# logannye/streaming-zero-knowledge-proofs

Hardware: AMD Instinct MI355X
Metric: STARK prove field-elements/sec (NTT+FRI+Merkle), 2^24 domain, 1/2/4/8 GPUs (higher is better)
Workload: dtype u64; 1 GPU; stark-v1 prove, T=2^21 rows (N=2^24 LDE domain), b=512, tau=8, trace resident in HBM when the timed region starts, proof bytes on the host (host_to_proof beside it: every proof uploads its own trace over PCIe); T=2097152, N=16777216, tau=8, b=512, proof_bytes=2301655, proofs_in_flight_per_gpu=3, upload_bytes_per_proof=69206016, parallelism=replicas x1, 3 independent proofs in flight per GPU

## Files before the change

### include/sezkp_stark.h

```cpp
#ifndef SEZKP_STARK_H
#define SEZKP_STARK_H

#include <stddef.h>
#include <stdint.h>

#ifdef __cplusplus
extern "C" {
#endif

#define SEZKP_ABI_VERSION 4u

#define SEZKP_OK 0
#define SEZKP_E_INVALID (-1)
#define SEZKP_E_DEVICE (-2)
#define SEZKP_E_NOMEM (-3)
#define SEZKP_E_DECODE (-4)
#define SEZKP_E_VERIFY (-5)

#define SEZKP_FLAG_STREAMING 1u

uint32_t sezkp_abi_version(void);
const char* sezkp_version(void);

typedef struct sezkp_buf {
    uint8_t* data;
    size_t len;
} sezkp_buf;
void sezkp_buf_free(sezkp_buf* b);

typedef struct sezkp_block_view {
    uint32_t n_blocks;
    uint32_t tau;
    const uint16_t* version;
    const uint32_t* block_id;
    const uint64_t* step_lo;
    const uint64_t* step_hi;
    const uint16_t* ctrl_in;
    const uint16_t* ctrl_out;
    const int64_t* in_head_in;
    const int64_t* in_head_out;
    const int64_t* win_left;
    const int64_t* win_right;
    const uint32_t* off_in;
    const uint32_t* off_out;
    const uint64_t* step_start;
    const int8_t* input_mv;
    const int8_t* mv;
    const uint8_t* has_write;
    const uint16_t* wsym;
} sezkp_block_view;

int32_t sezkp_stark_v1_prove(const sezkp_block_view* blocks, const uint8_t manifest_root[32], uint32_t flags,
                             sezkp_buf* proof_bytes, sezkp_buf* meta_json, char* err, size_t err_len);
int32_t sezkp_stark_v1_prove_artifact_cbor(const sezkp_block_view* blocks, const uint8_t manifest_root[32],
                                           uint32_t flags, sezkp_buf* artifact_cbor, char* err, size_t err_len);
int32_t sezkp_stark_v1_verify(const uint8_t* proof_bytes, size_t len, const sezkp_block_view* blocks,
                              const uint8_t manifest_root[32], char* err, size_t err_len);

typedef struct sezkp_ctx sezkp_ctx;
sezkp_ctx* sezkp_ctx_create(int32_t device, char* err, size_t err_len);
void sezkp_ctx_destroy(sezkp_ctx* ctx);
int32_t sezkp_ctx_upload(sezkp_ctx* ctx, const sezkp_block_view* blocks, char* err, size_t err_len);
int32_t sezkp_ctx_upload_rows(sezkp_ctx* ctx, const sezkp_block_view* blocks, uint64_t row0, uint64_t nrows,
                              char* err, size_t err_len);
int32_t sezkp_shard_rows(const uint64_t* step_start, uint32_t n_blocks, int32_t rank, int32_t world, uint64_t* row0,
                         uint64_t* nrows);
int32_t sezkp_ctx_prove(sezkp_ctx* ctx, const uint8_t manifest_root[32], uint32_t flags, sezkp_buf* proof_bytes,
                        char* err, size_t err_len);
int32_t sezkp_ctx_stage(sezkp_ctx* ctx, const sezkp_block_view* blocks, char* err, size_t err_len);
int32_t sezkp_host_register(void* p, size_t bytes);
int32_t sezkp_host_unregister(void* p);
int32_t sezkp_ctx_prove_borrow(sezkp_ctx* ctx, const uint8_t manifest_root[32], uint32_t flags,
                               const uint8_t** data, size_t* len, char* err, size_t err_len);
int32_t sezkp_ctx_stage_times(const sezkp_ctx* ctx, double* out_ms, int32_t max);
int32_t sezkp_ctx_prove_async(sezkp_ctx* ctx, const uint8_t manifest_root[32], uint32_t flags, char* err,
                              size_t err_len);
int32_t sezkp_ctx_wait(sezkp_ctx* ctx, const uint8_t** data, size_t* len, char* err, size_t err_len);
void* sezkp_ctx_stream(const sezkp_ctx* ctx);
typedef struct sezkp_dict_plan_info {
  uint32_t col;
  uint32_t kind;
  uint32_t tape;
  int32_t K;
  uint32_t a;
  uint32_t delta;
  uint32_t R;
  uint32_t dR;
  int64_t min;
} sezkp_dict_plan_info;
int32_t sezkp_ctx_dict_plans(const sezkp_ctx* ctx, sezkp_dict_plan_info* out, int32_t max);
int32_t sezkp_ctx_dict_cache_stats(const sezkp_ctx* ctx, uint32_t* cols_rebuilt, uint32_t* cols_reused,
                                   uint64_t* entries_rebuilt);

#define SEZKP_AIR_FAMILIES 5
typedef struct sezkp_air_family {
  uint64_t cells, rows, first_row;
  uint32_t first_tape, pad;
  uint64_t first_value;
} sezkp_air_family;
typedef struct sezkp_air_audit {
  uint64_t n_rows;
  uint32_t tau, pad;
  uint64_t rows_violating, first_violating, rows_rejectable, first_rejectable;
  sezkp_air_family fam[SEZKP_AIR_FAMILIES];
} sezkp_air_audit;
int32_t sezkp_ctx_air_audit(sezkp_ctx* ctx, sezkp_air_audit* out, uint8_t* violating_bits, uint8_t* rejectable_bits,
                            char* err, size_t err_len);
int32_t sezkp_stark_v1_air_audit(const sezkp_block_view* blocks, sezkp_air_audit* out, sezkp_buf* violating_bits,
                                 sezkp_buf* rejectable_bits, char* err, size_t err_len);

typedef struct sezkp_proof_ref {
  const uint8_t* bytes;
  size_t len;
  const uint8_t* manifest_root;
  uint32_t tau;
  uint32_t pad;
} sezkp_proof_ref;
typedef struct sezkp_verify_result {
  int32_t code;
  uint32_t pad;
  char msg[248];
} sezkp_verify_result;
int32_t sezkp_ctx_verify_batch(sezkp_ctx* ctx, const sezkp_proof_ref* proofs, uint32_t n, sezkp_verify_result* out,
                               char* err, size_t err_len);
int32_t sezkp_stark_v1_verify_batch(const sezkp_proof_ref* proofs, uint32_t n, sezkp_verify_result* out, char* err,
                                    size_t err_len);
enum {
  SEZKP_VT_PARSE, SEZKP_VT_PACK, SEZKP_VT_DEVICE_WALL, SEZKP_VT_H2D, SEZKP_VT_KERNEL, SEZKP_VT_D2H, SEZKP_VT_DECIDE,
  SEZKP_VT_WALL, SEZKP_VT_JOBS, SEZKP_VT_SLICES, SEZKP_VERIFY_TIMES
};
int32_t sezkp_ctx_verify_times(const sezkp_ctx* ctx, double* out_ms, int32_t max);

int32_t sezkp_comm_unique_id(uint8_t out[128], char* err, size_t err_len);
sezkp_ctx* sezkp_ctx_create_sharded(int32_t device, int32_t rank, int32_t world, const uint8_t unique_id[128],
                                    char* err, size_t err_len);
typedef struct sezkp_host_comm {
  void* user;
  int32_t (*allgather)(void* user, const void* send, void* recv, size_t bytes_per_rank);
  int32_t (*alltoall)(void* user, const void* send, void* recv, size_t bytes_per_rank);
  int32_t (*allreduce_sum_u8)(void* user, void* buf, size_t bytes);
} sezkp_host_comm;
sezkp_ctx* sezkp_ctx_create_sharded_host(int32_t device, int32_t rank, int32_t world, const sezkp_host_comm* comm,
                                         char* err, size_t err_len);
sezkp_ctx* sezkp_ctx_create_sharded_solo(int32_t device, int32_t rank, int32_t world, char* err, size_t err_len);
typedef struct sezkp_comm_stat {
  char name[32];
  uint64_t bytes;
  double ms;
} sezkp_comm_stat;
int32_t sezkp_ctx_comm_stats(const sezkp_ctx* ctx, sezkp_comm_stat* out, int32_t max);

int32_t sezkp_ctx_dist_ntt(sezkp_ctx* ctx, uint64_t* local, uint64_t* scratch, uint32_t log_n, int32_t dir,
                           char* err, size_t err_len);

int32_t sezkp_gl_ntt(uint64_t* d, uint64_t* scratch, uint32_t log_n, int32_t dir, void* stream);
int32_t sezkp_gl_coset_lde_deep(uint64_t* evals, uint32_t log_n, uint32_t log_blowup, uint64_t shift, uint64_t z,
                                uint64_t* out, uint8_t* leaves32, void* stream);
int32_t sezkp_fri_fold(const uint64_t* in, uint64_t n_out, uint64_t beta, uint64_t* out, void* stream);
int32_t sezkp_fri_fold_commit(const uint64_t* in, uint64_t n_out, uint64_t beta, uint64_t* out, uint8_t* root32,
                              void* stream);
int32_t sezkp_merkle_root_u64(const uint64_t* vals, uint64_t n, uint8_t* root32, void* stream);
int32_t sezkp_blake3_leaves_u64(const uint64_t* vals, uint64_t n, uint8_t* leaves32, void* stream);
int32_t sezkp_blake3_leaves_labeled(const uint64_t* vals, uint64_t n, const char* label, uint32_t label_len,
                                    uint8_t* leaves32, void* stream);
uint64_t sezkp_merkle_node_count(uint64_t n);
int32_t sezkp_merkle_build(const uint8_t* leaves32, uint64_t n, uint8_t* nodes32, void* stream);
int32_t sezkp_merkle_paths(const uint8_t* nodes32, uint64_t n, const uint64_t* idx, uint32_t q, uint8_t* out32,
                           void* stream);

int32_t sezkp_manifest_root(const sezkp_block_view* blocks, uint8_t out[32]);
int32_t sezkp_manifest_frontier_root(const sezkp_block_view* blocks, uint8_t out[32]);
typedef struct sezkp_blocks sezkp_blocks;
int32_t sezkp_blocks_decode_cbor(const uint8_t* data, size_t len, sezkp_blocks** out, char* err, size_t err_len);
int32_t sezkp_blocks_decode_jsonl(const uint8_t* data, size_t len, sezkp_blocks** out, char* err, size_t err_len);
int32_t sezkp_blocks_encode_jsonl(const sezkp_block_view* blocks, sezkp_buf* out);
const sezkp_block_view* sezkp_blocks_view(const sezkp_blocks* b);
// ... 25 lines not shown
```

### streaming-zero-knowledge-proofs_amd/csrc/dev_common.h

```cpp
#pragma once
#include <hip/hip_runtime.h>
#include <stdint.h>

namespace sezkp {

constexpr uint64_t GL_P = 0xffffffff00000001ULL;
constexpr uint64_t GL_EPS = 0xffffffffULL;

__device__ __forceinline__ uint64_t add64c(uint64_t a, uint64_t b, uint32_t& carry) {
  uint32_t c0;
  const uint32_t lo = __builtin_addc((uint32_t)a, (uint32_t)b, 0u, &c0);
  const uint32_t hi = __builtin_addc((uint32_t)(a >> 32), (uint32_t)(b >> 32), c0, &carry);
  return ((uint64_t)hi << 32) | lo;
}
__device__ __forceinline__ uint64_t sub64b(uint64_t a, uint64_t b, uint32_t& borrow) {
  uint32_t b0;
  const uint32_t lo = __builtin_subc((uint32_t)a, (uint32_t)b, 0u, &b0);
  const uint32_t hi = __builtin_subc((uint32_t)(a >> 32), (uint32_t)(b >> 32), b0, &borrow);
  return ((uint64_t)hi << 32) | lo;
}
__device__ __forceinline__ uint64_t gl_add(uint64_t a, uint64_t b) {
  uint32_t c1, c2;
  const uint64_t s = add64c(a, b, c1);
  const uint64_t t = add64c(s, GL_EPS, c2);
  return (c1 | c2) ? t : s;
}
__device__ __forceinline__ uint64_t gl_sub(uint64_t a, uint64_t b) {
  uint32_t br;
  const uint64_t d = sub64b(a, b, br);
  return br ? d - GL_EPS : d;
}
__device__ __forceinline__ uint64_t gl_canon(uint64_t r) {
  uint32_t c;
  const uint64_t t = add64c(r, GL_EPS, c);
  return c ? t : r;
}
__device__ __forceinline__ uint64_t gl_reduce128_weak(uint64_t lo, uint64_t hi) {
  const uint32_t h0 = (uint32_t)hi, h1 = (uint32_t)(hi >> 32);
  uint32_t br, c;
  uint64_t t0 = sub64b(lo, h1, br);
  if (br) t0 -= GL_EPS;
  const uint64_t t1 = ((uint64_t)h0 << 32) - h0;
  const uint64_t r = add64c(t0, t1, c);
  return c ? r + GL_EPS : r;
}
__device__ __forceinline__ uint64_t gl_reduce128(uint64_t lo, uint64_t hi) {
  return gl_canon(gl_reduce128_weak(lo, hi));
}
__device__ __forceinline__ void gl_mul128(uint64_t a, uint64_t b, uint64_t& lo, uint64_t& hi) {
  const uint32_t a0 = (uint32_t)a, a1 = (uint32_t)(a >> 32), b0 = (uint32_t)b, b1 = (uint32_t)(b >> 32);
  const uint64_t p00 = (uint64_t)a0 * b0;
  const uint64_t t = (uint64_t)a0 * b1 + (p00 >> 32);
  const uint64_t u = (uint64_t)a1 * b0 + (uint32_t)t;
  hi = (uint64_t)a1 * b1 + ((t >> 32) + (u >> 32));
  lo = ((uint64_t)(uint32_t)u << 32) | (uint32_t)p00;
}
__device__ __forceinline__ uint64_t gl_mul(uint64_t a, uint64_t b) {
  uint64_t lo, hi;
  gl_mul128(a, b, lo, hi);
  return gl_reduce128(lo, hi);
}
__device__ __forceinline__ uint64_t gl_sqr(uint64_t a) { return gl_mul(a, a); }
__device__ __forceinline__ uint64_t gl_from_i64(int64_t x) {
  return x >= 0 ? (uint64_t)x : GL_P - (uint64_t)(-x);
}
__device__ __forceinline__ uint64_t gl_pow2k(uint64_t x, int k) {
  for (int i = 0; i < k; i++) x = gl_sqr(x);
  return x;
}
__device__ inline uint64_t gl_inv(uint64_t a) {
  uint64_t t2 = gl_mul(gl_sqr(a), a);
  uint64_t t4 = gl_mul(gl_pow2k(t2, 2), t2);
  uint64_t t8 = gl_mul(gl_pow2k(t4, 4), t4);
  uint64_t t16 = gl_mul(gl_pow2k(t8, 8), t8);
  uint64_t t24 = gl_mul(gl_pow2k(t16, 8), t8);
  uint64_t t28 = gl_mul(gl_pow2k(t24, 4), t4);
  uint64_t t30 = gl_mul(gl_pow2k(t28, 2), t2);
  uint64_t t31 = gl_mul(gl_sqr(t30), a);
  uint64_t t32 = gl_mul(gl_sqr(t31), a);
  uint64_t hi = gl_pow2k(gl_sqr(t31), 32);
  return gl_mul(hi, t32);
}
__device__ __forceinline__ uint64_t gl_pow_dev(uint64_t b, uint64_t e) {
  uint64_t r = 1;
  while (e) {
    if (e & 1) r = gl_mul(r, b);
    b = gl_sqr(b);
    e >>= 1;
  }
  return r;
}

#define B3_IV0 0x6A09E667u
#define B3_IV1 0xBB67AE85u
#define B3_IV2 0x3C6EF372u
#define B3_IV3 0xA54FF53Au
#define B3_IV4 0x510E527Fu
#define B3_IV5 0x9B05688Cu
#define B3_IV6 0x1F83D9ABu
#define B3_IV7 0x5BE0CD19u
#define B3_ROOT_FLAGS 11u

__device__ __forceinline__ uint32_t rotr32(uint32_t x, int n) {
  return __builtin_amdgcn_alignbit(x, x, n);
}

__host__ __device__ constexpr int b3_sigma(int r, int i) {
  constexpr int PERM[16] = {2, 6, 3, 10, 7, 0, 4, 13, 1, 11, 12, 5, 9, 14, 15, 8};
  for (int k = 0; k < r; k++) i = PERM[i];
  return i;
}

#define B3_FENCE(v)                                                                                         \
  asm volatile("" : "+v"(v[0]), "+v"(v[1]), "+v"(v[2]), "+v"(v[3]), "+v"(v[4]), "+v"(v[5]), "+v"(v[6]),   \
               "+v"(v[7]), "+v"(v[8]), "+v"(v[9]), "+v"(v[10]), "+v"(v[11]), "+v"(v[12]), "+v"(v[13]),     \
               "+v"(v[14]), "+v"(v[15]))

template <int R, bool DIAG, bool FENCE>
__device__ __forceinline__ void b3_half_round(uint32_t (&v)[16], const uint32_t (&m)[16]) {
#define B3_STEP(EXPR)                                                                     \
  _Pragma("unroll") for (int g = 0; g < 4; g++) {                                         \
    const int A = g, B = 4 + (DIAG ? (g + 1) & 3 : g), C = 8 + (DIAG ? (g + 2) & 3 : g), \
              D = 12 + (DIAG ? (g + 3) & 3 : g);                                          \
    (void)A; (void)B; (void)C; (void)D;                                                   \
    EXPR;                                                                                 \
  }                                                                                       \
  if (FENCE) B3_FENCE(v);
  B3_STEP(v[A] = v[A] + v[B] + m[b3_sigma(R, 2 * g + 8 * DIAG)])
  B3_STEP(v[D] = v[D] ^ v[A])
  B3_STEP(v[D] = rotr32(v[D], 16))
  B3_STEP(v[C] = v[C] + v[D])
  B3_STEP(v[B] = v[B] ^ v[C])
  B3_STEP(v[B] = rotr32(v[B], 12))
  B3_STEP(v[A] = v[A] + v[B] + m[b3_sigma(R, 2 * g + 1 + 8 * DIAG)])
  B3_STEP(v[D] = v[D] ^ v[A])
  B3_STEP(v[D] = rotr32(v[D], 8))
  B3_STEP(v[C] = v[C] + v[D])
  B3_STEP(v[B] = v[B] ^ v[C])
  B3_STEP(v[B] = rotr32(v[B], 7))
#undef B3_STEP
}
template <int R>
__device__ __forceinline__ void b3_rounds(uint32_t (&v)[16], const uint32_t (&m)[16]) {
  b3_half_round<R, false, (R > 0)>(v, m);
  b3_half_round<R, true, (R > 0)>(v, m);
  if constexpr (R < 6) b3_rounds<R + 1>(v, m);
}
// ... 114 lines not shown
```

### streaming-zero-knowledge-proofs_amd/csrc/ntt.hip

```cpp
#include <stdlib.h>

#include <algorithm>

#include "dev_common.h"
#include "gl_pow2.h"
#include "sezkp_internal.h"
#include "compose.h"

namespace sezkp {

constexpr int NTT_THREADS = 256;
constexpr int NTT_CMAX = 16;
constexpr int NTT_PADC = NTT_CMAX + 1;
constexpr int NTT_MMAX = 8;

__device__ __forceinline__ uint64_t tw_pow(const NttTables& T, uint64_t e, bool inverse) {
  uint64_t mask = (T.K >= 64) ? ~0ULL : ((1ULL << T.K) - 1);
  if (inverse) e = (0 - e) & mask;
  return gl_mul(T.hi[e >> T.S], T.lo[e & ((1ULL << T.S) - 1)]);
}
__device__ __forceinline__ uint64_t pow3(const NttTables& T, uint64_t e) {
  return gl_mul(T.p3_hi[e >> T.S], T.p3_lo[e & ((1ULL << T.S) - 1)]);
}

__device__ __forceinline__ uint64_t src_slot(const NttPassArgs& P, uint64_t k, uint32_t e) {
  if (!P.src_logP) return k;
  const int lm = P.log_src - P.src_logP;
  const uint64_t hi = (uint64_t)e >> P.src_logP;
  return ((uint64_t)(e & ((1u << P.src_logP) - 1)) << lm) | (lm ? (__brev((uint32_t)hi) >> (32 - lm)) : 0);
}

__device__ __forceinline__ uint64_t dp_load(const NttPassArgs& P, const NttTables& T, uint64_t p, int b) {
  const uint64_t e = (uint64_t)(__brev((uint32_t)p) >> (32 - P.dp_logN));
  uint64_t v = gl_mul(P.dp_rhi[e >> 12], P.dp_rlo[e & 4095]);
  if ((p & ((1ULL << b) - 1)) == 0) {
    const uint64_t k = p >> b;
    const uint32_t rk = P.log_src ? (__brev((uint32_t)k) >> (32 - P.log_src)) : 0;
    uint64_t qv = gl_mul(gl_mul(P.src[src_slot(P, k, rk)], P.inv_n), pow3(T, rk));
    if (P.coset_e) qv = gl_mul(qv, tw_pow(T, ((uint64_t)rk * P.coset_e) & ((1ULL << T.K) - 1), false));
    v = gl_sub(gl_add(v, qv), gl_mul(P.dp_rhk[e >> 12], P.dp_rlo[e & 4095]));
  }
  return v;
}

template <bool DIF>
__global__ void __launch_bounds__(NTT_THREADS) k_ntt_pass(NttPassArgs P) {
  __shared__ uint64_t sh[(1 << NTT_MMAX) * NTT_PADC];
  __shared__ uint64_t W[(1 << NTT_MMAX) / 2];
  const int m = P.m, R = 1 << m, sL = P.sL;
  const uint64_t L = 1ULL << sL;
  const int logC = P.logC, C = 1 << logC;
  const int tid = threadIdx.x;
  const uint64_t tile = blockIdx.x;
  const NttTables& T = P.tw;

  for (int x = tid; x < R / 2; x += NTT_THREADS) W[x] = tw_pow(T, (uint64_t)x << (T.K - m), P.inverse);

  const int nel = R << logC;
  const bool wide = L >= (uint64_t)C;
  uint64_t blk_base = 0, low0 = 0;
  if (wide) {
    uint64_t tiles_per_blk = L >> logC;
    blk_base = (tile / tiles_per_blk) * ((uint64_t)R << sL);
    low0 = (tile % tiles_per_blk) << logC;
  }
  const int tw_shift = T.K - m - sL;
  for (int q = tid; q < nel; q += NTT_THREADS) {
    int t, c;
    uint64_t low, pos;
    if (wide) {
      t = q >> logC; c = q & (C - 1); low = low0 + c;
      pos = blk_base + low + ((uint64_t)t << sL);
    } else {
      low = q & (L - 1);
      t = (q >> sL) & (R - 1);
      c = ((q >> (sL + m)) << sL) | (int)low;
      pos = tile * (uint64_t)nel + q;
    }
    uint64_t v;
    if (P.dp_rlo) {
      v = dp_load(P, T, pos, P.dp_logN - P.log_src);
    } else if (P.src) {
      uint64_t k = pos >> P.skip;
      uint32_t rk = P.log_src ? (__brev((uint32_t)k) >> (32 - P.log_src)) : 0;
      v = gl_mul(gl_mul(P.src[src_slot(P, k, rk)], P.inv_n), pow3(T, rk));
      if (P.coset_e) v = gl_mul(v, tw_pow(T, ((uint64_t)rk * P.coset_e) & ((1ULL << T.K) - 1), false));
    } else {
      v = P.a[pos];
    }
    if (!DIF && low != 0) {
      uint32_t bt = __brev((uint32_t)t) >> (32 - m);
      v = gl_mul(v, tw_pow(T, (low * bt) << tw_shift, P.inverse));
    }
    sh[t * NTT_PADC + c] = v;
  }
  __syncthreads();
  const int nbf = (R / 2) << logC;
  for (int it = 0; it < m - P.skip; it++) {
    const int s = DIF ? (m - 1 - it) : (it + P.skip);
    const int h = 1 << s;
    for (int b = tid; b < nbf; b += NTT_THREADS) {
      const int c = b & (C - 1), u = b >> logC;
      const int j = u & (h - 1);
      const int t0 = ((u >> s) << (s + 1)) | j, t1 = t0 + h;
      const uint64_t w = W[j << (m - 1 - s)];
// ... 133 lines not shown
  const int sb = 32 - (logN - m);
#pragma unroll
  for (int j = 0; j < NTT_CMAX * R / NTT_THREADS; j++) {
    const int e = j * NTT_THREADS + threadIdx.x, i = e >> m, row = e & (R - 1);
    const uint64_t B = __brev((uint32_t)(tile * NTT_CMAX + i)) >> sb;
    sh[row * NTT_PADC + i] = a[(B << m) + row];
  }
}
template <int R>
__device__ __forceinline__ void lds_to_transposed(const uint64_t* sh, const NttPassArgs& P, uint64_t tile) {
  constexpr int m = __builtin_ctz(R);
  const int lo = P.nat_logN - m;
#pragma unroll
  for (int j = 0; j < NTT_CMAX * R / NTT_THREADS; j++) {
    const int e = j * NTT_THREADS + threadIdx.x, i = e & (NTT_CMAX - 1), row = e >> 4;
    const uint64_t k = __brev((uint32_t)row) >> (32 - m);
    uint64_t v = sh[row * NTT_PADC + i];
    if (P.out_scale != 1) v = gl_mul(v, P.out_scale);
    P.out[(k << lo) + tile * NTT_CMAX + i] = v;
  }
}

template <int R>
__device__ __forceinline__ void gather_dit_to_lds(uint64_t* sh, const uint64_t* __restrict__ x, uint64_t tile,
                                                  int logN) {
  constexpr int m = __builtin_ctz(R);
#pragma unroll
  for (int j = 0; j < NTT_CMAX * R / NTT_THREADS; j++) {
    const int e = j * NTT_THREADS + threadIdx.x, i = e & (NTT_CMAX - 1), row = e >> 4;
    sh[row * NTT_PADC + i] = x[((uint64_t)(__brev((uint32_t)row) >> (32 - m)) << (logN - m)) + tile * NTT_CMAX + i];
  }
}
template <int R>
__device__ __forceinline__ void lds_to_blocks(const uint64_t* sh, uint64_t* __restrict__ a, uint64_t tile, int logN) {
  constexpr int m = __builtin_ctz(R);
  const int sb = 32 - (logN - m);
#pragma unroll
  for (int j = 0; j < NTT_CMAX * R / NTT_THREADS; j++) {
    const int e = j * NTT_THREADS + threadIdx.x, i = e >> m, row = e & (R - 1);
    const uint64_t B = __brev((uint32_t)(tile * NTT_CMAX + i)) >> sb;
    a[(B << m) + row] = sh[row * NTT_PADC + i];
  }
}

__device__ __forceinline__ uint64_t nat_tile(uint32_t b, uint32_t tiles) {
  if (tiles % 128) return b;
  const uint32_t xcd = b % 8, k = b / 8;
  return (uint64_t)((k / 16) * 8 + xcd) + (uint64_t)(k % 16) * (tiles / 16);
}

template <int R, bool DIF, bool INV>
__device__ __forceinline__ void tile_radix16(uint64_t* sh, const NttTables& T) {
  constexpr int m = __builtin_ctz(R);
  const int row = threadIdx.x;
  if (row >= R) return;
  uint64_t x[16];
#pragma unroll
  for (int t = 0; t < 16; t++) x[t] = sh[row * NTT_PADC + t];
  if constexpr (DIF) fft_dif_regs<4, INV>(x);
  if (row) {
    const uint64_t s1 = tw_pow(T, (uint64_t)row << (T.K - m - 4), INV);
    uint64_t t = s1;
#pragma unroll
    for (int q = 1; q < 16; q++) {
      x[rev<4>(q)] = gl_mul(x[rev<4>(q)], t);
      if (q + 1 < 16) t = gl_mul(t, s1);
    }
  }
  if constexpr (!DIF) fft_dit_regs<4, INV, 0>(x);
#pragma unroll
  for (int t = 0; t < 16; t++) sh[row * NTT_PADC + t] = x[t];
}

template <bool DIF, bool INV, int M1, int M2, int SKIP, bool DEEP = false, bool NARROW = false,
          bool X16 = false>
__global__ void __launch_bounds__(NTT_THREADS, 4) k_ntt4(NttPassArgs P) {
  constexpr int F1 = 1 << M1, F2 = 1 << M2, m = M1 + M2, R = 1 << m;
  static_assert(!(NARROW && DEEP), "the fused DEEP pass is a wide pass");
  static_assert(!X16 || (NARROW && SKIP == 0), "the in-tile radix-16 step extends a plain NARROW pass");
  __shared__ uint64_t sh[R * NTT_PADC];
  __shared__ uint64_t W[R];
  const int tid = threadIdx.x;
  const NttTables& T = P.tw;
  for (int x = tid; x < R; x += NTT_THREADS) W[x] = tw_pow(T, (uint64_t)x << (T.K - m), INV);
  Tile G;
  G.sL = P.sL;
  G.m = m;
  G.tile = (NARROW && P.nat_out) ? nat_tile(blockIdx.x, gridDim.x) : blockIdx.x;
  G.wide = (1ULL << G.sL) >= (uint64_t)NTT_CMAX;
  G.blk_base = 0;
  G.low0 = 0;
  if (G.wide) {
    const uint64_t tiles_per_blk = (1ULL << G.sL) / NTT_CMAX;
    G.blk_base = (G.tile / tiles_per_blk) * ((uint64_t)R << G.sL);
    G.low0 = (G.tile % tiles_per_blk) * NTT_CMAX;
  }
  const int tw_shift = T.K - m - G.sL;
  const int c = tid & (NTT_CMAX - 1), g = tid / NTT_CMAX;
  const bool staged_load = NARROW && !P.dp_rlo && !P.src;
  if constexpr (NARROW && DIF && !X16) {
    if (P.nat_tr) gather_to_lds<R>(sh, P.a, G.tile, P.nat_logN);
    else if (staged_load) narrow_to_lds<R>(sh, P.a, G.tile);
  } else if constexpr (NARROW && !DIF && SKIP == 0 && !X16) {
    if (staged_load && P.nat_tr) gather_dit_to_lds<R>(sh, P.a, G.tile, P.nat_logN);
    else if (staged_load) narrow_to_lds<R>(sh, P.a, G.tile);
  } else if (staged_load) {
    narrow_to_lds<R>(sh, P.a, G.tile);
  }
  __syncthreads();
  if constexpr (X16 && DIF) {
    tile_radix16<R, true, INV>(sh, T);
    __syncthreads();
  }
  if constexpr (!DIF) {
    uint64_t x[F1];
    if (g < F2) {
      const int u = g;
      uint64_t low = 0;
      if (P.dp_rlo) {
        const uint64_t p0 = tile_pos(G, F1 * u, c, low);
        const int b = P.dp_logN - P.log_src;
#pragma unroll
        for (int r = 0; r < F1; r++) x[r] = dp_load(P, T, p0 + r, b);
      } else if (P.src) {
        const uint64_t p0 = tile_pos(G, F1 * u, c, low);
#pragma unroll
        for (int r = 0; r < F1; r += (1 << SKIP)) {
          const uint64_t k = (p0 + r) >> P.skip;
          const uint32_t rk = P.log_src ? (__brev((uint32_t)k) >> (32 - P.log_src)) : 0;
          uint64_t v = gl_mul(gl_mul(P.src[src_slot(P, k, rk)], P.inv_n), pow3(T, rk));
          if (P.coset_e) v = gl_mul(v, tw_pow(T, ((uint64_t)rk * P.coset_e) & ((1ULL << T.K) - 1), false));
#pragma unroll
          for (int s = 0; s < (1 << SKIP); s++) x[r + s] = v;
        }
      } else if (NARROW) {
#pragma unroll
        for (int r = 0; r < F1; r++) x[r] = sh[(F1 * u + r) * NTT_PADC + c];
      } else {
#pragma unroll
        for (int r = 0; r < F1; r++) x[r] = P.a[tile_pos(G, F1 * u + r, c, low)];
        const bool scale = P.out_scale > 1;
        if (scale && low == 0) {
#pragma unroll
          for (int r = 0; r < F1; r++) x[r] = gl_mul(x[r], P.out_scale);
        }
        if (low != 0) {
          const int j1 = rev<M2>(u);
          uint64_t t = tw_pow(T, (low * (uint64_t)j1) << tw_shift, INV);
          if (scale) t = gl_mul(t, P.out_scale);
          const uint64_t s1 = tw_pow(T, (low * (uint64_t)F2) << tw_shift, INV);
#pragma unroll
          for (int q = 0; q < F1; q++) {
            x[rev<M1>(q)] = gl_mul(x[rev<M1>(q)], t);
            if (q + 1 < F1) t = gl_mul(t, s1);
          }
        }
      }
      fft_dit_regs<M1, INV, SKIP>(x);
    }
    if (staged_load) __syncthreads();
    if (g < F2) {
      const int u = g, j1 = rev<M2>(u);
#pragma unroll
      for (int k2 = 0; k2 < F1; k2++) {
        const uint64_t v = k2 && j1 ? gl_mul(x[k2], W[j1 * k2]) : x[k2];
        sh[(u * F1 + k2) * NTT_PADC + c] = v;
      }
    }
    __syncthreads();
    uint64_t y[F2];
    if (g < F1) {
      const int k2 = g;
#pragma unroll
      for (int u = 0; u < F2; u++) y[u] = sh[(u * F1 + k2) * NTT_PADC + c];
      fft_dit_regs<M2, INV, 0>(y);
      uint64_t low;
      if constexpr (DEEP) {
        static_assert(F1 * NTT_CMAX == NTT_THREADS && !INV && !DIF, "fused DEEP needs every thread in step 2");
#pragma unroll
        for (int k1 = 0; k1 < F2; k1++) sh[(k1 * F1 + k2) * NTT_PADC + c] = y[k1];
        const uint64_t pos0 = tile_pos(G, k2, c, low);
        const uint64_t e = ((uint64_t)P.deep_g + (pos0 << P.deep_logP)) << (T.K - P.deep_logN);
        const uint64_t x0 = gl_mul(gl_mul(T.hi[e >> T.S], T.lo[e & ((1ULL << T.S) - 1)]), 3);
        deep_tile<F2>(x0, P.deep_z, [&](int k1, uint64_t inv) {
          P.a[tile_pos(G, k2 + F1 * k1, c, low)] = gl_mul(sh[(k1 * F1 + k2) * NTT_PADC + c], inv);
        });
      } else if (!NARROW) {
        uint64_t* dst = P.out ? P.out : P.a;
#pragma unroll
        for (int k1 = 0; k1 < F2; k1++) dst[tile_pos(G, k2 + F1 * k1, c, low)] = y[k1];
      }
    }
    if constexpr (NARROW) {
      __syncthreads();
      if (g < F1) {
#pragma unroll
        for (int k1 = 0; k1 < F2; k1++) sh[(g + F1 * k1) * NTT_PADC + c] = y[k1];
      }
      __syncthreads();
      if constexpr (X16) {
        tile_radix16<R, false, INV>(sh, T);
        __syncthreads();
      }
      if (!X16 && P.nat_tr) lds_to_blocks<R>(sh, P.out ? P.out : P.a, G.tile, P.nat_logN);
      else lds_to_narrow<R>(sh, P.out ? P.out : P.a, G.tile);
    }
  } else {
    uint64_t x[F2];
    if (g < F1) {
      const int r = g;
      uint64_t low;
#pragma unroll
      for (int u = 0; u < F2; u++)
        x[u] = NARROW ? sh[(F1 * u + r) * NTT_PADC + c] : P.a[tile_pos(G, F1 * u + r, c, low)];
      fft_dif_regs<M2, INV>(x);
    }
    if (NARROW) __syncthreads();
    if (g < F1) {
      const int r = g;
#pragma unroll
      for (int q = 0; q < F2; q++) {
        const int klo = rev<M2>(q);
        const uint64_t v = klo && r ? gl_mul(x[q], W[r * klo]) : x[q];
        sh[(q * F1 + r) * NTT_PADC + c] = v;
      }
    }
    __syncthreads();
    uint64_t y[F1];
    if (g < F2) {
      const int q = g;
#pragma unroll
      for (int r = 0; r < F1; r++) y[r] = sh[(q * F1 + r) * NTT_PADC + c];
      fft_dif_regs<M1, INV>(y);
      uint64_t low;
      (void)tile_pos(G, q * F1, c, low);
      if (low != 0) {
        uint64_t t = tw_pow(T, (low * (uint64_t)rev<M2>(q)) << tw_shift, INV);
        const uint64_t s1 = tw_pow(T, (low * (uint64_t)F2) << tw_shift, INV);
#pragma unroll
        for (int kh = 0; kh < F1; kh++) {
          y[rev<M1>(kh)] = gl_mul(y[rev<M1>(kh)], t);
          if (kh + 1 < F1) t = gl_mul(t, s1);
        }
      }
      if (!NARROW) {
        uint64_t* dst = P.out ? P.out : P.a;
#pragma unroll
        for (int qq = 0; qq < F1; qq++) dst[tile_pos(G, q * F1 + qq, c, low)] = y[qq];
      }
    }
    if constexpr (NARROW) {
      __syncthreads();
      if (g < F2) {
#pragma unroll
        for (int qq = 0; qq < F1; qq++) sh[(g * F1 + qq) * NTT_PADC + c] = y[qq];
      }
      __syncthreads();
      if (!X16 && P.nat_tr) lds_to_transposed<R>(sh, P, G.tile);
      else if (P.nat_out) lds_to_natural<R>(sh, P, G.tile);
      else lds_to_narrow<R>(sh, P.a, G.tile);
    }
  }
}

template <int F1>
__device__ __forceinline__ int dif9_slot(int q, int r, int c) {
  return (q * F1 + r) * NTT_PADC + c + (q << 4);
}
template <bool INV>
__global__ void __launch_bounds__(512, 2) k_ntt_dif9(NttPassArgs P) {
  constexpr int M1 = 5, M2 = 4, F1 = 1 << M1, F2 = 1 << M2, m = M1 + M2, R = 1 << m, NT = 512;
  __shared__ uint64_t sh[R * NTT_PADC + 16 * (1 << M2)];
  __shared__ uint64_t W[R];
  const int tid = threadIdx.x;
  const NttTables& T = P.tw;
  for (int x = tid; x < R; x += NT) W[x] = tw_pow(T, (uint64_t)x << (T.K - m), INV);
  Tile G;
  G.sL = P.sL;
  G.m = m;
  G.tile = blockIdx.x;
  G.wide = true;
  const uint64_t tiles_per_blk = (1ULL << G.sL) / NTT_CMAX;
  G.blk_base = (G.tile / tiles_per_blk) * ((uint64_t)R << G.sL);
  G.low0 = (G.tile % tiles_per_blk) * NTT_CMAX;
  const int tw_shift = T.K - m - G.sL;
  const int c = tid & (NTT_CMAX - 1), g = tid / NTT_CMAX;
  uint64_t low;
  {
    const int r = g;
    uint64_t x[F2];
#pragma unroll
    for (int u = 0; u < F2; u++) x[u] = P.a[tile_pos(G, F1 * u + r, c, low)];
    fft_dif_regs<M2, INV>(x);
    __syncthreads();
#pragma unroll
    for (int q = 0; q < F2; q++) {
      const int klo = rev<M2>(q);
      sh[dif9_slot<F1>(q, r, c)] = klo && r ? gl_mul(x[q], W[r * klo]) : x[q];
    }
  }
  __syncthreads();
  {
    const int q = g & (F2 - 1), h = g >> M2;
    uint64_t y[16];
#pragma unroll
    for (int r = 0; r < 16; r++) {
      const uint64_t a = sh[dif9_slot<F1>(q, r, c)], b = sh[dif9_slot<F1>(q, r + 16, c)];
      if (h == 0) {
        y[r] = gl_add(a, b);
      } else {
        const int e = r ? tw_exp<INV>(r, 16) : 0;
        const bool neg = e >= 96;
        y[r] = gl_mul2e(neg ? gl_sub(b, a) : gl_sub(a, b), neg ? e - 96 : e);
      }
    }
    fft_dif_regs<4, INV>(y);
    (void)tile_pos(G, q * F1, c, low);
    if (low != 0) {
      uint64_t t = tw_pow(T, (low * ((uint64_t)rev<M2>(q) + (uint64_t)F2 * h)) << tw_shift, INV);
// ... 84 lines not shown
      uint64_t t = ta[hh];
#pragma unroll
      for (int k = 0; k < 4; k++) {
        y[rev<2>(k)] = gl_mul(y[rev<2>(k)], t);
        if (k < 3) t = gl_mul(t, tb);
      }
    }
#pragma unroll
    for (int d = 0; d < 4; d++) dst[tile_pos(G, 4 * h + d, c, low)] = y[d];
  }
}

__device__ __forceinline__ int n12_slot(int e) {
  const int b = (e >> 6) & 7, c = (e >> 3) & 7, d = e & 7;
  return (e & ~63) | ((c ^ (b & 3)) << 3) | (d ^ c);
}

template <bool INV>
__global__ void __launch_bounds__(R8_NT, 2) k_ntt_n12r8(NttPassArgs P) {
  __shared__ uint64_t sh[4096];
  const int g = threadIdx.x;
  const NttTables& T = P.tw;
  const uint64_t tile = nat_tile(blockIdx.x, gridDim.x);
  const uint64_t p0 = tile << 12;
  uint64_t x[8];
  const int lo2 = g & 63;
  const uint64_t w1 = tw_pow(T, (uint64_t)g << (T.K - 12), INV);
  const uint64_t w2 = tw_pow(T, (uint64_t)lo2 << (T.K - 9), INV);
#pragma unroll
  for (int d = 0; d < 8; d++) x[d] = P.a[p0 + g + 512 * d];
  fft_dif_regs<3, INV>(x);
  if (g) r8_twiddle(x, w1);
#pragma unroll
  for (int q = 0; q < 8; q++) sh[n12_slot(g + 512 * q)] = x[q];
  __syncthreads();
  {
    const int base = (g >> 6) * 512 + lo2;
#pragma unroll
    for (int d = 0; d < 8; d++) x[d] = sh[n12_slot(base + 64 * d)];
    fft_dif_regs<3, INV>(x);
    if (lo2) r8_twiddle(x, w2);
#pragma unroll
    for (int d = 0; d < 8; d++) sh[n12_slot(base + 64 * d)] = x[d];
  }
  wave_lds_sync();
  {
    const int lo = g & 7, base = (g >> 3) * 64 + lo;
#pragma unroll
    for (int d = 0; d < 8; d++) x[d] = sh[n12_slot(base + 8 * d)];
    fft_dif_regs<3, INV>(x);
    if (lo) {
#pragma unroll
      for (int k = 1; k < 8; k++) x[rev<3>(k)] = gl_mul_pow2(x[rev<3>(k)], tw_exp64<INV>(lo * k));
    }
#pragma unroll
    for (int d = 0; d < 8; d++) sh[n12_slot(base + 8 * d)] = x[d];
  }
  wave_lds_sync();
#pragma unroll
  for (int d = 0; d < 8; d++) x[d] = sh[n12_slot(8 * g + d)];
  fft_dif_regs<3, INV>(x);
  const int sh_r = 32 - P.nat_logN;
  const bool scale = P.out_scale > 1;
#pragma unroll
  for (int q = 0; q < 8; q++)
    P.out[__brev((uint32_t)(p0 + 8 * g + q)) >> sh_r] = scale ? gl_mul(x[q], P.out_scale) : x[q];
}

static bool launch_r8(hipStream_t st, const NttPassArgs& P, bool inverse, unsigned tiles) {
  if (P.src || P.dp_rlo || P.nat_tr) return false;
  if (P.m == 8 && P.logC == 4 && P.sL >= 4 && !P.nat_out) {
    if (inverse) hipLaunchKernelGGL(k_ntt_w8r8<true>, dim3(tiles), dim3(R8_NT), 0, st, P);
    else hipLaunchKernelGGL(k_ntt_w8r8<false>, dim3(tiles), dim3(R8_NT), 0, st, P);
    return true;
  }
  if (P.m == 12 && P.sL == 0 && P.nat_out) {
    if (inverse) hipLaunchKernelGGL(k_ntt_n12r8<true>, dim3(tiles), dim3(R8_NT), 0, st, P);
    else hipLaunchKernelGGL(k_ntt_n12r8<false>, dim3(tiles), dim3(R8_NT), 0, st, P);
    return true;
  }
  return false;
}

template <bool DIF, bool INV>
static bool launch_ntt4(hipStream_t st, const NttPassArgs& P, unsigned tiles) {
  if (P.logC != 4) return false;
  const int skip = P.src ? P.skip : 0;
  if (DIF && skip) return false;
#define SEZKP_NTT4(M1, M2, SK)                                                                                \
  do {                                                                                                         \
    if (P.sL == 0)                                                                                           \
      hipLaunchKernelGGL((k_ntt4<DIF, INV, M1, M2, SK, false, true>), dim3(tiles), dim3(NTT_THREADS), 0, st, P); \
    else                                                                                                       \
      hipLaunchKernelGGL((k_ntt4<DIF, INV, M1, M2, SK>), dim3(tiles), dim3(NTT_THREADS), 0, st, P);           \
  } while (0)
  if (P.m > NTT_MMAX) {
    if (P.sL != 0 || skip || (P.src && !P.dp_rlo)) return false;
#define SEZKP_NTT4X(M1, M2) \
  hipLaunchKernelGGL((k_ntt4<DIF, INV, M1, M2, 0, false, true, true>), dim3(tiles), dim3(NTT_THREADS), 0, st, P)
    switch (P.m) {
      case 12: SEZKP_NTT4X(4, 4); return true;
      case 11: SEZKP_NTT4X(4, 3); return true;
      case 10: SEZKP_NTT4X(3, 3); return true;
      default: return false;
    }
#undef SEZKP_NTT4X
  }
  switch (P.m * 4 + skip) {
    case 8 * 4 + 0: SEZKP_NTT4(4, 4, 0); return true;
    case 7 * 4 + 0: SEZKP_NTT4(4, 3, 0); return true;
    case 6 * 4 + 0: SEZKP_NTT4(3, 3, 0); return true;
    default: break;
  }
  if constexpr (!DIF) {
    switch (P.m * 4 + skip) {
      case 8 * 4 + 1: SEZKP_NTT4(4, 4, 1); return true;
      case 8 * 4 + 2: SEZKP_NTT4(4, 4, 2); return true;
      case 8 * 4 + 3: SEZKP_NTT4(4, 4, 3); return true;
      case 7 * 4 + 1: SEZKP_NTT4(4, 3, 1); return true;
      case 7 * 4 + 2: SEZKP_NTT4(4, 3, 2); return true;
      case 7 * 4 + 3: SEZKP_NTT4(4, 3, 3); return true;
      case 6 * 4 + 1: SEZKP_NTT4(3, 3, 1); return true;
      case 6 * 4 + 2: SEZKP_NTT4(3, 3, 2); return true;
      case 6 * 4 + 3: SEZKP_NTT4(3, 3, 3); return true;
      default: break;
    }
  }
#undef SEZKP_NTT4
  return false;
}

__global__ void __launch_bounds__(256) k_bitrev_permute(const uint64_t* __restrict__ in, uint64_t* __restrict__ out,
                                                         int logN, uint64_t scale, int do_scale) {
  __shared__ uint64_t sh[16 * 17];
  const int a = 4, b = logN - 2 * a;
  const uint32_t y = blockIdx.x;
  const int tid = threadIdx.x;
  const int x = tid >> 4, z = tid & 15;
  uint32_t ry = b ? (__brev(y) >> (32 - b)) : 0;
  uint64_t src = ((uint64_t)x << (a + b)) | ((uint64_t)y << a) | z;
  uint64_t v = in[src];
  if (do_scale) v = gl_mul(v, scale);
  sh[x * 17 + z] = v;
  __syncthreads();
  const int rz = tid >> 4, rx = tid & 15;
  const int zz = __brev((uint32_t)rz) >> 28, xx = __brev((uint32_t)rx) >> 28;
  uint64_t dst = ((uint64_t)rz << (a + b)) | ((uint64_t)ry << a) | rx;
  out[dst] = sh[xx * 17 + zz];
}

template <int A>
__global__ void __launch_bounds__(256) k_bitrev_inplace(uint64_t* __restrict__ a, int logN, uint64_t scale,
                                                        int do_scale) {
  constexpr int S = 1 << A, PER = S * S / 256;
  __shared__ uint64_t sh[2][S * (S + 1)];
  const int b = logN - 2 * A;
  const uint32_t y = blockIdx.x;
  const uint32_t ry = b ? (__brev(y) >> (32 - b)) : 0;
  if (y > ry) return;
  const int tid = threadIdx.x;
  uint64_t v0[PER], v1[PER];
#pragma unroll
  for (int j = 0; j < PER; j++) {
    const int e = j * 256 + tid, x = e >> A, z = e & (S - 1);
    v0[j] = a[((uint64_t)x << (A + b)) | ((uint64_t)y << A) | z];
    v1[j] = a[((uint64_t)x << (A + b)) | ((uint64_t)ry << A) | z];
  }
#pragma unroll
  for (int j = 0; j < PER; j++) {
    const int e = j * 256 + tid, x = e >> A, z = e & (S - 1);
    sh[0][x * (S + 1) + z] = do_scale ? gl_mul(v0[j], scale) : v0[j];
    sh[1][x * (S + 1) + z] = do_scale ? gl_mul(v1[j], scale) : v1[j];
  }
  __syncthreads();
#pragma unroll
  for (int j = 0; j < PER; j++) {
    const int e = j * 256 + tid, rz = e >> A, rx = e & (S - 1);
// ... 281 lines not shown
    int o = 0;
    if (!dif) ms[o++] = f;
    for (int i = 0; i < k; i++) ms[o++] = base + (i < rem ? 1 : 0);
    if (dif) ms[o++] = f;
    *np = o;
    return true;
  }
  return false;
}

hipError_t ntt_dif(hipStream_t st, uint64_t* a, int logN, bool inverse, const NttTables& T) {
  if (logN == 0) return hipSuccess;
  int ms[8], np;
  const bool x16 = plan_passes_x16(logN, true, ms, &np);
  if (!x16) plan_passes(logN, 1, ms, &np);
  if (logN == 21) {
    NttPassArgs P{};
    P.a = a; P.tw = T; P.m = 9; P.sL = 12; P.inverse = inverse ? 1 : 0; P.logC = 4;
    const unsigned tiles = (unsigned)((1ULL << logN) >> (9 + 4));
    if (inverse) hipLaunchKernelGGL(k_ntt_dif9<true>, dim3(tiles), dim3(512), 0, st, P);
    else hipLaunchKernelGGL(k_ntt_dif9<false>, dim3(tiles), dim3(512), 0, st, P);
    P.m = 12; P.sL = 0;
    const bool ok = inverse ? launch_ntt4<true, true>(st, P, (unsigned)((1ULL << logN) >> 12))
                            : launch_ntt4<true, false>(st, P, (unsigned)((1ULL << logN) >> 12));
    if (!ok) return hipErrorInvalidValue;
    return hipGetLastError();
  }
  int sL = logN;
  for (int i = 0; i < np; i++) {
    NttPassArgs P{};
    P.a = a; P.src = nullptr; P.tw = T; P.m = ms[i]; sL -= ms[i]; P.sL = sL;
    P.inverse = inverse ? 1 : 0; P.skip = 0;
    int logC = logN - P.m; if (logC > 4) logC = 4; P.logC = logC;
    uint64_t tiles = (1ULL << logN) >> (P.m + logC);
    if (P.m > NTT_MMAX) {
      P.logC = 4;
      tiles = (1ULL << logN) >> P.m;
      const bool ok = inverse ? launch_ntt4<true, true>(st, P, (unsigned)tiles)
                              : launch_ntt4<true, false>(st, P, (unsigned)tiles);
      if (!ok) return hipErrorInvalidValue;
      continue;
    }
    const bool fast = inverse ? launch_ntt4<true, true>(st, P, (unsigned)tiles)
                              : launch_ntt4<true, false>(st, P, (unsigned)tiles);
    if (!fast) hipLaunchKernelGGL(k_ntt_pass<true>, dim3((unsigned)tiles), dim3(NTT_THREADS), 0, st, P);
  }
  return hipGetLastError();
}

hipError_t ntt_dit(hipStream_t st, uint64_t* a, int logN, bool inverse, const NttTables& T,
                   const uint64_t* src, int log_src, uint64_t inv_n, uint64_t coset_e, const DeepFuse* deep,
                   bool* fused, const DeepPoly* dpoly, int src_logP) {
  if (src_logP < 0 || src_logP > 3 || (src_logP && (!src || log_src < src_logP))) return hipErrorInvalidValue;
  if (fused) *fused = false;
  if (logN == 0) return hipSuccess;
  if (dpoly && (!src || logN > 32 || log_src > logN)) return hipErrorInvalidValue;
  int ms[8], np;
  const bool x16 = (!src || dpoly) && plan_passes_x16(logN, false, ms, &np);
  if (!x16) plan_passes(logN, src ? 3 : 1, ms, &np);
  if (src && ms[0] < logN - log_src) return hipErrorInvalidValue;
  int sL = 0;
  for (int i = 0; i < np; i++) {
    NttPassArgs P{};
    P.a = a; P.tw = T; P.m = ms[i]; P.sL = sL; P.inverse = inverse ? 1 : 0;
    P.src = (i == 0) ? src : nullptr;
    P.log_src = log_src; P.inv_n = inv_n; P.coset_e = (i == 0) ? coset_e : 0;
    P.src_logP = (i == 0) ? src_logP : 0;
    P.skip = (i == 0 && src && !dpoly) ? (logN - log_src) : 0;
    if (i == 0 && dpoly) { P.dp_rlo = dpoly->rlo; P.dp_rhi = dpoly->rhi; P.dp_rhk = dpoly->rhk; P.dp_logN = logN; }
    int logC = logN - P.m; if (logC > 4) logC = 4; P.logC = logC;
    uint64_t tiles = (1ULL << logN) >> (P.m + logC);
    if (P.m > NTT_MMAX) {
      P.logC = 4;
      tiles = (1ULL << logN) >> P.m;
      const bool ok = inverse ? launch_ntt4<false, true>(st, P, (unsigned)tiles)
                              : launch_ntt4<false, false>(st, P, (unsigned)tiles);
      if (!ok) return hipErrorInvalidValue;
      sL += ms[i];
      continue;
    }
    if (deep && fused && i == np - 1 && i > 0 && !inverse &&
        logC == 4 && P.sL >= 4 && (P.m == 8 || P.m == 7)) {
      P.deep_z = deep->z; P.deep_logN = deep->logN; P.deep_logP = deep->logP; P.deep_g = deep->g;
      if (P.m == 8)
        hipLaunchKernelGGL((k_ntt4<false, false, 4, 4, 0, true>), dim3((unsigned)tiles), dim3(NTT_THREADS), 0, st, P);
      else
        hipLaunchKernelGGL((k_ntt4<false, false, 4, 3, 0, true>), dim3((unsigned)tiles), dim3(NTT_THREADS), 0, st, P);
      *fused = true;
      sL += ms[i];
      continue;
    }
    const bool fast = inverse ? launch_ntt4<false, true>(st, P, (unsigned)tiles)
                              : launch_ntt4<false, false>(st, P, (unsigned)tiles);
    if (!fast) hipLaunchKernelGGL(k_ntt_pass<false>, dim3((unsigned)tiles), dim3(NTT_THREADS), 0, st, P);
    sL += ms[i];
  }
  return hipGetLastError();
}

static bool ntt_dif_natural_tr(hipStream_t st, uint64_t* a, uint64_t* scratch, int logN, bool inverse,
                               const NttTables& T, uint64_t scale, hipError_t* err) {
  if (logN < 23 || logN > 26) return false;
  int plan[3];
  plan[2] = 8;
  const int rest = logN - 8;
  plan[0] = (rest + 1) / 2;
  plan[1] = rest - plan[0];
  int sL = logN;
  for (int i = 0; i < 3; i++) {
    NttPassArgs P{};
    P.a = i == 0 ? a : scratch;
    P.out = i == 0 ? scratch : nullptr;
    P.tw = T; P.m = plan[i]; sL -= plan[i]; P.sL = sL;
    P.inverse = inverse ? 1 : 0;
    P.logC = 4;
    const uint64_t tiles = (1ULL << logN) >> (P.m + 4);
    if (i == 2) {
      P.a = scratch; P.out = a; P.nat_tr = 1; P.nat_logN = logN; P.out_scale = scale;
    }
    if (P.m == 9) {
      if (inverse) hipLaunchKernelGGL(k_ntt_dif9<true>, dim3((unsigned)tiles), dim3(512), 0, st, P);
      else hipLaunchKernelGGL(k_ntt_dif9<false>, dim3((unsigned)tiles), dim3(512), 0, st, P);
      continue;
    }
    const bool ok = inverse ? launch_ntt4<true, true>(st, P, (unsigned)tiles)
                            : launch_ntt4<true, false>(st, P, (unsigned)tiles);
    if (!ok) { *err = hipErrorInvalidValue; return true; }
  }
  *err = hipGetLastError();
  return true;
}

static bool ntt_dit_natural(hipStream_t st, uint64_t* a, uint64_t* scratch, int logN, bool inverse,
                            const NttTables& T, uint64_t scale, hipError_t* err) {
  if (logN < 21 || logN > 24) return false;
  int ms[8], np;
  if (plan_passes_x16(logN, false, ms, &np)) return false;
  plan_passes(logN, 1, ms, &np);
  if (np < 2 || ms[0] > NTT_MMAX) return false;
  int sL = 0;
  for (int i = 0; i < np; i++) {
    NttPassArgs P{};
    P.tw = T; P.m = ms[i]; P.sL = sL; P.inverse = inverse ? 1 : 0; P.logC = 4;
    P.a = i == 0 ? a : scratch;
    P.out = i == 0 ? scratch : (i == np - 1 ? a : nullptr);
    if (i == 0) { P.nat_tr = 1; P.nat_logN = logN; }
    if (i == np - 1) P.out_scale = scale;
    const unsigned tiles = (unsigned)(P.m > NTT_MMAX ? (1ULL << logN) >> P.m : (1ULL << logN) >> (P.m + 4));
    const bool ok = inverse ? launch_ntt4<false, true>(st, P, tiles) : launch_ntt4<false, false>(st, P, tiles);
    if (!ok) { *err = hipErrorInvalidValue; return true; }
    sL += ms[i];
  }
  *err = hipGetLastError();
  return true;
}

bool ntt_dif_natural(hipStream_t st, uint64_t* a, uint64_t* scratch, int logN, bool inverse, const NttTables& T,
                     uint64_t scale, hipError_t* err) {
  *err = hipSuccess;
  if (scratch && scratch != a && ntt_dit_natural(st, a, scratch, logN, inverse, T, scale, err)) return true;
  if (scratch && scratch != a && ntt_dif_natural_tr(st, a, scratch, logN, inverse, T, scale, err)) return true;
  if (!scratch || scratch == a || logN < 19 || logN > 22)
    return false;
  int ms[8], np;
  const bool x16 = plan_passes_x16(logN, true, ms, &np);
  if (!x16) plan_passes(logN, 1, ms, &np);
// ... 86 lines not shown
```

### streaming-zero-knowledge-proofs_amd/csrc/prover.cpp

```cpp
#include <hip/hip_runtime.h>
#include <stdio.h>
#include <stdlib.h>
#include <string.h>

#include <algorithm>
#include <chrono>
#include <condition_variable>
#include <map>
#include <memory>
#include <mutex>
#include <string>
#include <thread>
#include <vector>

#include "../../include/sezkp_stark.h"
#include "codec.h"
#include "comm.h"
#include "host_crypto.h"
#include "prove_plan.h"
#include "sezkp_internal.h"
#include "verify_plan.h"

using namespace sezkp;

// ... 71 lines not shown
  bool stop = false;
  uint8_t root[32];
  int32_t rc = 0;
  std::string msg;
  size_t len = 0;
};

static int worker_delay_us() {
  static const int us = [] {
    const char* e = getenv("SEZKP_TEST_WORKER_DELAY_US");
    return e ? atoi(e) : 0;
  }();
  return us;
}

struct sezkp_ctx {
  int device = 0;
  std::unique_ptr<AsyncSlot> async;
  hipStream_t st = nullptr;
  hipStream_t st2 = nullptr;
  hipStream_t stc = nullptr;
  hipEvent_t ev_fold = nullptr, ev_tail = nullptr, ev_expand = nullptr, ev_cols = nullptr;
  hipEvent_t ev_qin = nullptr, ev_qout = nullptr;
  struct TraceSlot {
    int8_t* imv = nullptr;
    int8_t* mv = nullptr;
    uint8_t* wf = nullptr;
    uint16_t* ws = nullptr;
    uint64_t *bw = nullptr, *bi = nullptr, *bo = nullptr;
    uint8_t* raw = nullptr;
    uint64_t* h_tab = nullptr;
    hipEvent_t ready = nullptr;
    bool image_pending = false;
  };
  TraceSlot slot[2];
  int active = 0;
  bool staged = false;
  std::mutex stage_mu;
  std::vector<uint64_t> cur_step_start;
  NttTables tw{};
  std::vector<std::pair<void*, size_t>> dev_allocs, host_allocs, mapped_allocs;
  std::multimap<size_t, void*> spare_dev, spare_host, spare_mapped;
  bool loaded = false;
  uint64_t n = 0, N = 0;
  int logn = 0, logN = 0, ncols = 0, logChunks = 0;
  uint32_t tau = 0, nblk = 0;
  TraceDev T{};
  std::vector<std::string> labels;
  ColTemplate* d_tmpl = nullptr;
  uint32_t* d_tabs = nullptr;
  uint32_t* d_tab_cols = nullptr;
  int n_tab_cols = 0;
  uint64_t tab_units = 0;
  uint32_t* d_work = nullptr;
  int n_work = 0;
  uint32_t* d_pw_cols = nullptr;
  int n_pw_cols = 0;
  uint32_t* d_pw_chunks = nullptr;
  int n_pw_chunks = 0;
  DictCol* d_dcols = nullptr;
  int n_dict = 0;
  int64_t* d_dpart = nullptr;
  DictPlan* d_dplans = nullptr;
  std::vector<sezkp_dict_plan_info> dict_info;
  bool have_plans = false;
  uint32_t* d_dtabs = nullptr;
  DictKey* d_dkeys = nullptr;
  uint64_t* d_dlvl_seq = nullptr;
  uint32_t* d_dreuse = nullptr;
  uint32_t* d_dstatus = nullptr;
  size_t dict_cache_cols = ~(size_t)0;
  uint64_t dict_epoch = 1, dict_seq = 0;
  struct DictHostKey {
    uint64_t n = 0, nrows = 0, row0 = 0, plan_rows = 0;
    uint32_t tab_cap = 0;
    bool operator==(const DictHostKey& o) const {
      return n == o.n && nrows == o.nrows && row0 == o.row0 && plan_rows == o.plan_rows && tab_cap == o.tab_cap;
    }
  } dict_hkey;
  std::vector<uint8_t> dict_shape;
  bool dict_dirty = false;
  uint32_t dstat_rebuilt = 0, dstat_reused = 0;
  uint64_t dstat_entries = 0;
  void free_dict_cache() {
    if (d_dtabs) (void)hipFree(d_dtabs);
    if (d_dkeys) (void)hipFree(d_dkeys);
    d_dtabs = nullptr;
    d_dkeys = nullptr;
    dict_cache_cols = ~(size_t)0;
  }
  uint32_t* d_dlev = nullptr;
  std::vector<uint32_t> dict_of;
  uint32_t* d_outer = nullptr;
  uint32_t* d_err = nullptr;
  uint64_t outer_stride = 0;
  uint32_t* d_colroots = nullptr;
  uint64_t* d_base = nullptr;
  ComposeTerms Tm{};
  uint64_t *d_dq_part = nullptr, *d_dq_rlo = nullptr, *d_dq_rhi = nullptr, *d_dq_rhk = nullptr;
  uint64_t* d_lde = nullptr;
  uint64_t* d_fri = nullptr;
  uint32_t* d_roots = nullptr;
  DevChal* d_chal = nullptr;
  DevChal* h_chal = nullptr;
  uint32_t* d_dict_of = nullptr;
  int rank = 0, world = 1, logP = 0;
  std::unique_ptr<Comm> comm;
  bool sharded() const { return comm != nullptr; }
  int tree_stop() const { return sharded() ? L16_LOG : LSTORE_FRI; }
  int tree_wg_log = L16_LOG;
  int wg_stop() const { return std::min(tree_stop(), tree_wg_log); }
  uint64_t M = 0;
  int logM = 0;
  int rR = -1;
  uint64_t ch_lo = 0, ch_hi = 0;
  uint32_t blk_lo = 0, blk_cnt = 0;
  uint64_t* d_cyc = nullptr;
  bool full_lde = false;
  uint64_t* d_xbuf = nullptr;
  uint64_t* d_rep = nullptr;
  std::vector<uint64_t*> lvals;
  std::vector<TreeDev> ltrees, caps;
  std::vector<uint32_t*> rr_gather;
  std::vector<int> rep16;
  int tail_first = 1;
  FriLayerDev* d_layers = nullptr;
  ForestLayer* d_forest = nullptr;
  uint64_t* d_tailbuf = nullptr;
  int n_forest = 0;
  uint32_t forest_wgs = 0;
  UpperJob* d_jobs = nullptr;
  std::vector<std::pair<size_t, int>> jobs0, jobsF;
  std::vector<std::pair<size_t, int>> jobsL0, jobsLR;
  uint32_t* d_req = nullptr;
  uint32_t* h_req = nullptr;
  ProofLayout PL{};
  size_t hdr_bytes = 0;
  std::vector<size_t> root_pos;
  uint8_t* h_proof = nullptr;
  uint32_t* h_small = nullptr;
  size_t max_fri_req = 0, max_open_req = 0;
  hipEvent_t ev[ST_NSTAGE + 1]{};
  double stage_ms[ST_NSTAGE + 1]{};
  hipEvent_t kev[2]{};
  double kernel_ms = 0;
  hipEvent_t oev[2]{};
  double host_ms[4]{};
  bool have_times = false;
  bool broken = false;
  bool coll_issued = false;
  struct CollStat {
    const char* name;
    uint64_t bytes;
    hipEvent_t a, b;
  };
  std::vector<CollStat> coll_stats;
  std::vector<hipEvent_t> coll_ev;
  size_t coll_used = 0;
  uint32_t* stall_word = nullptr;
  uint64_t* d_audit = nullptr;
  uint64_t* h_audit = nullptr;
  uint64_t audit_n = 0;
  void free_audit() {
    if (d_audit) (void)hipFree(d_audit);
    d_audit = nullptr;
    audit_n = 0;
// ... 270 lines not shown
                                     ", " + std::to_string(v.step_hi[k]) + "] is empty or longer than 2^28"};
    const uint64_t len = v.step_hi[k] - v.step_lo[k] + 1;
    const uint64_t steps = v.step_start[k + 1] - v.step_start[k];
    if (len != steps)
      throw Err{SEZKP_E_INVALID, "block " + std::to_string(k) + ": step_hi-step_lo+1=" + std::to_string(len) +
                                     " but movement_log has " + std::to_string(steps) + " steps"};
  }
  ShapePlan sp;
  ColumnPlan cp;
  FriPlan fp;
  ProofPlan pp;
  try {
    sp = plan_shape(tau, v.step_start, nblk, rank, logP, sharded());
    cp = plan_columns(sp, v.step_start, getenv("SEZKP_NO_DICT") == nullptr);
    fp = plan_fri(sp);
    pp = plan_proof(sp, cp.labels);
  } catch (const PlanError& e) {
    throw Err{SEZKP_E_INVALID, e.msg};
  }
  n = sp.n;
  if (audit_n != n) free_audit();
  logn = sp.logn;
  logN = sp.logN;
  N = sp.N;
  ncols = sp.ncols;
  logChunks = sp.logChunks;
  ch_lo = sp.ch_lo;
  ch_hi = sp.ch_hi;
  blk_lo = sp.blk_lo;
  blk_cnt = sp.blk_cnt;
  full_lde = sp.full_lde;
  M = sp.M;
  logM = sp.logM;
  tree_wg_log = sp.tree_wg_log;
  rR = sp.rR;
  if (nrows == ~0ull) nrows = n - row0;
  {
    const uint64_t need0 = v.step_start[blk_lo], need1 = v.step_start[blk_lo + blk_cnt];
    if (row0 > need0 || row0 + nrows < need1 || row0 + nrows > n)
      throw Err{SEZKP_E_INVALID, "step arrays hold rows [" + std::to_string(row0) + ", " + std::to_string(row0 + nrows) +
                                     ") but this context needs rows [" + std::to_string(need0) + ", " +
                                     std::to_string(need1) + ")"};
  }

  auto up = [&](auto* dst, const auto* src, size_t count) {
    if (count) HIP_OR_THROW(hipMemcpy(dst, src, count * sizeof(*src), hipMemcpyHostToDevice));
  };
  staged = false;
  active = 0;
  {
    hipEvent_t keep = slot[1].ready;
    slot[1] = TraceSlot{};
    slot[1].ready = keep;
  }
  alloc_slot(slot[0]);
  uint64_t* d_bs = dalloc<uint64_t>(nblk + 1);
  up(d_bs, v.step_start, nblk + 1);
  cur_step_start.assign(v.step_start, v.step_start + nblk + 1);
  write_trace(slot[0], v, st, row0, nrows);
  HIP_OR_THROW(hipStreamSynchronize(st));
  TraceSlot& t0 = slot[0];
  T.n = n;
  T.tau = (int)tau;
  T.nblk = nblk;
  T.input_mv = t0.imv;
  T.mv = t0.mv;
  T.wflag = t0.wf;
  T.wsym = t0.ws;
  T.blk_start = d_bs;
  T.blk_winlen = t0.bw;
  T.blk_offin = t0.bi;
  T.blk_offout = t0.bo;
  T.row_blk = dalloc<uint32_t>(n);
  T.row_flags = dalloc<uint8_t>(n);
  T.head = dalloc<int32_t>((size_t)tau * n + 2);
  T.head_rng = dalloc<int64_t>(2 * (size_t)tau * nblk + 2);

  labels = cp.labels;
  const std::vector<ColTemplate>& tm = cp.tmpl;
  const std::vector<DictCol>& dcols = cp.dcols;
  tab_units = cp.tab_units;
  d_tmpl = dalloc<ColTemplate>(ncols);
  up(d_tmpl, tm.data(), tm.size());
  d_colroots = dalloc<uint32_t>((size_t)ncols * 8 + 16 + 2 * dcols.size());
  d_err = d_colroots + (size_t)ncols * 8;
  d_dstatus = d_err + 16;
  HIP_OR_THROW(hipMemset(d_err, 0, 64));
  d_tabs = dalloc<uint32_t>(cp.tab_nodes * 8 + 8);
  n_tab_cols = (int)cp.tab_cols.size();
  d_tab_cols = dalloc<uint32_t>(cp.tab_cols.size() + 1);
  up(d_tab_cols, cp.tab_cols.data(), cp.tab_cols.size());
  n_dict = (int)dcols.size();
  have_plans = false;
  dict_info.assign(dcols.size(), sezkp_dict_plan_info{});
  for (size_t i = 0; i < dcols.size(); i++) {
    dict_info[i].col = dcols[i].col;
    dict_info[i].kind = tm[dcols[i].col].kind;
    dict_info[i].tape = tm[dcols[i].col].tape;
  }
  d_dcols = dalloc<DictCol>(dcols.size() + 1);
  up(d_dcols, dcols.data(), dcols.size());
  d_dpart = dalloc<int64_t>(2 * dcols.size() * ((n + 4095) / 4096) + 2);
  d_dplans = dalloc<DictPlan>(dcols.size() + 1);
  if (dcols.size() != dict_cache_cols) {
    free_dict_cache();
    dict_epoch++;
    const size_t nd = dcols.size();
    const size_t key_bytes = nd * sizeof(DictKey) + DICT_LEVELS * 8, cache_bytes = key_bytes + nd * 4 + 64;
    HIP_OR_THROW(hipMalloc((void**)&d_dtabs, (nd * DICT_LEVELS * DICT_CAP * 8 + 8) * sizeof(uint32_t)));
    HIP_OR_THROW(hipMalloc((void**)&d_dkeys, cache_bytes));
    HIP_OR_THROW(hipMemset(d_dkeys, 0, cache_bytes));
    d_dlvl_seq = reinterpret_cast<uint64_t*>(d_dkeys + nd);
    d_dreuse = reinterpret_cast<uint32_t*>(d_dlvl_seq + DICT_LEVELS);
    dict_cache_cols = nd;
  }
  {
    std::vector<uint8_t> shape(dcols.size() * (sizeof(ColTemplate) + sizeof(DictCol)));
    uint8_t* p = shape.data();
    for (const DictCol& d : dcols) {
      memcpy(p, &tm[d.col], sizeof(ColTemplate));
      memcpy(p + sizeof(ColTemplate), &d, sizeof(DictCol));
      p += sizeof(ColTemplate) + sizeof(DictCol);
    }
    if (shape != dict_shape) {
      dict_shape.swap(shape);
      dict_epoch++;
    }
  }
  d_dlev = dalloc<uint32_t>(dcols.size() * (n >> COL_CHUNK_LOG2) * DLEV_NODES * 8 + 8);
  dict_of = cp.dict_of;
  n_pw_cols = (int)cp.pw_cols.size();
  d_pw_cols = dalloc<uint32_t>(cp.pw_cols.size() + 1);
  up(d_pw_cols, cp.pw_cols.data(), cp.pw_cols.size());
  n_pw_chunks = (int)cp.pw_chunks.size();
  d_pw_chunks = dalloc<uint32_t>(cp.pw_chunks.size() + 1);
  up(d_pw_chunks, cp.pw_chunks.data(), cp.pw_chunks.size());
  n_work = (int)(cp.work.size() / 2);
  d_work = dalloc<uint32_t>(cp.work.size() + 2);
  up(d_work, cp.work.data(), cp.work.size());
  outer_stride = tree_stored_nodes(logChunks, 0);
  d_outer = dalloc<uint32_t>((size_t)ncols * outer_stride * 8);

  const int k = logN;
  d_base = dalloc<uint64_t>(n);
  Tm.hr = dalloc<uint64_t>(n);
  Tm.sl = dalloc<uint64_t>(n);
  Tm.c3 = dalloc<int64_t>(n);
  Tm.c2 = dalloc<int32_t>(n + 2);
  Tm.sy = dalloc<int32_t>(n + 2);
  Tm.bf = dalloc<uint64_t>((size_t)nblk + 1);
  Tm.bl = dalloc<uint64_t>((size_t)nblk + 1);
  Tm.row_flags = T.row_flags;
  Tm.row_blk = T.row_blk;
  {
    const uint64_t Ml = full_lde ? N : N >> logP;
    d_dq_part = dalloc<uint64_t>(n / 1024 + 1);
    d_dq_rlo = dalloc<uint64_t>(4096);
    d_dq_rhi = dalloc<uint64_t>(Ml > 4096 ? Ml >> 12 : 1);
    d_dq_rhk = dalloc<uint64_t>(n > 4096 ? n >> 12 : 1);
  }
  d_lde = dalloc<uint64_t>(fp.lde_vals);
  if (sharded()) {
    d_cyc = dalloc<uint64_t>(full_lde ? N : M);
    if (!full_lde) d_xbuf = dalloc<uint64_t>(M);
  }
  d_fri = dalloc<uint64_t>(fp.run_vals + 1);
  d_rep = dalloc<uint64_t>(fp.rep_vals + 1);
  d_roots = dalloc<uint32_t>((size_t)fp.root_slots * 8);
  uint32_t* d_nodes = dalloc<uint32_t>(fp.total_nodes * 8 + 8);
  lvals.assign(k + 1, nullptr);
  ltrees.assign(k + 1, TreeDev{});
  caps.assign(k + 1, TreeDev{});
  rr_gather.assign(k + 1, nullptr);
  std::vector<FriLayerDev> ly(k + 1);
  uint64_t* const val_buf[3] = {d_lde, d_fri, d_rep};
  for (int r = 0; r <= k; r++) {
    const FriLayerPlan& L = fp.layers[r];
    lvals[r] = val_buf[L.buf] + L.val_off;
    ltrees[r] = TreeDev{d_nodes + L.node_off * 8, d_roots + 8 * L.root_slot, L.logLen, L.lstore};
    caps[r] = TreeDev{d_nodes + L.cap_off * 8, d_roots + 8 * L.cap_root_slot, L.cap_logLen, L.cap_lstore};
    if (L.has_cap) rr_gather[r] = d_nodes + L.gather_off * 8;
    ly[r] = FriLayerDev{lvals[r], ltrees[r], caps[r], (uint32_t)L.has_cap, (uint32_t)logP};
  }
  d_layers = dalloc<FriLayerDev>(k + 1);
  up(d_layers, ly.data(), ly.size());
  rep16 = fp.rep16;
  tail_first = fp.tail_first;
  {
    std::vector<ForestLayer> fl;
    for (const ForestEntryPlan& e : fp.forest) fl.push_back(ForestLayer{lvals[e.layer], ltrees[e.layer], e.wg_start, e.stop});
    n_forest = (int)fl.size();
    forest_wgs = fp.forest_wgs;
    d_forest = dalloc<ForestLayer>(fl.size() + 1);
    if (!fl.empty()) up(d_forest, fl.data(), fl.size());
    d_tailbuf = fp.tailbuf ? dalloc<uint64_t>((size_t)TAIL_MAX << TAIL_MAX) : nullptr;
  }
  {
    std::vector<UpperJob> all = fp.jobs;
    for (size_t i = 0; i < all.size(); i++) {
      const int r = fp.job_layer[i];
      all[i].tree = fp.job_cap[i] ? caps[r] : ltrees[r];
      if (all[i].gath) all[i].gath = rr_gather[r];
    }
    jobs0 = fp.jobs0;
    jobsF = fp.jobsF;
    jobsL0 = fp.jobsL0;
    jobsLR = fp.jobsLR;
    d_jobs = dalloc<UpperJob>(all.size() + 1);
    if (!all.empty()) up(d_jobs, all.data(), all.size());
  }
  max_fri_req = pp.max_fri_req;
  max_open_req = pp.max_open_req;
  h_req = hmapped<uint32_t>(max_fri_req * 3 + max_open_req * OPEN_REQ_WORDS);
  d_req = h_req;
  hdr_bytes = pp.hdr_bytes;
  root_pos = pp.root_pos;
  PL = pp.PL;
  PL.base = dalloc<uint32_t>(PL.total / 4 + 2);
  h_proof = halloc<uint8_t>(hdr_bytes + PL.total);
  memcpy(h_proof, pp.header.data(), hdr_bytes);
  h_small = halloc<uint32_t>((size_t)(ncols + k + 4) * 8 + 2 * (size_t)n_dict);
  d_chal = dalloc<DevChal>(1);
  h_chal = halloc<DevChal>(1);
  d_dict_of = dalloc<uint32_t>((size_t)ncols);
  up(d_dict_of, dict_of.data(), dict_of.size());
  release_spares();
  loaded = true;
}

void sezkp_ctx::alloc_slot(TraceSlot& t) {
  const size_t cells = (size_t)tau * n, nt = (size_t)tau * nblk;
  t.imv = dalloc<int8_t>(n);
  t.mv = dalloc<int8_t>(cells);
  t.wf = dalloc<uint8_t>(cells);
  t.ws = dalloc<uint16_t>(cells);
  t.bw = dalloc<uint64_t>(3 * nt + 1);
  t.bi = t.bw + nt;
  t.bo = t.bi + nt;
  t.raw = dalloc<uint8_t>(4 * cells);
  t.h_tab = halloc<uint64_t>(3 * nt + 1);
  if (!t.ready) HIP_OR_THROW(hipEventCreateWithFlags(&t.ready, hipEventDisableTiming));
}

void sezkp_ctx::wait_copy_stream() {
  if (!stc) return;
  for (;;) {
    const hipError_t q = hipStreamQuery(stc);
    if (q == hipSuccess) return;
    if (q != hipErrorNotReady) HIP_OR_THROW(q);
    std::this_thread::yield();
  }
}

void sezkp_ctx::launch_image(TraceSlot& t, hipStream_t s, uint64_t row0, uint64_t nrows) {
  const size_t cells = (size_t)tau * n;
  HIP_OR_THROW(launch_trace_image(s, reinterpret_cast<int8_t*>(t.raw + 2 * cells), t.raw + 3 * cells,
                                  reinterpret_cast<uint16_t*>(t.raw), n, tau, t.mv, t.wf, t.ws, row0, row0 + nrows));
  HIP_OR_THROW(hipEventRecord(t.ready, s));
  t.image_pending = false;
}

void sezkp_ctx::write_trace(TraceSlot& t, const sezkp_block_view& v, hipStream_t s, uint64_t row0, uint64_t nrows,
                            bool staged_copy) {
  const size_t cells = (size_t)tau * n, nt = (size_t)tau * nblk;
  wait_copy_stream();
  HIP_OR_THROW(hipEventSynchronize(t.ready));
  for (uint32_t k = 0; k < nblk; k++)
    for (uint32_t r = 0; r < tau; r++) {
      const size_t i = (size_t)k * tau + r, o = (size_t)r * nblk + k;
      const int64_t d = v.win_right[i] - v.win_left[i];
      const uint64_t wl = (d < 0 ? 0 - (uint64_t)d : (uint64_t)d) + 1;
      t.h_tab[o] = wl % GL_P_HOST;
      t.h_tab[nt + o] = v.off_in[i];
      t.h_tab[2 * nt + o] = v.off_out[i];
    }
  constexpr size_t chunk = (size_t)4 << 20;
  auto cp = [&](void* dst, const void* src, size_t bytes) {
    for (size_t o = 0; o < bytes;) {
      const size_t b = std::min(chunk, bytes - o);
      HIP_OR_THROW(hipMemcpyAsync((uint8_t*)dst + o, (const uint8_t*)src + o, b, hipMemcpyHostToDevice, s));
      o += b;
    }
  };
  uint16_t* raw_ws = reinterpret_cast<uint16_t*>(t.raw);
  int8_t* raw_mv = reinterpret_cast<int8_t*>(t.raw + 2 * cells);
  uint8_t* raw_hw = t.raw + 3 * cells;
  const size_t c0 = (size_t)row0 * tau, nc = (size_t)nrows * tau;
  cp(raw_ws + c0, v.wsym, nc * 2);
  cp(raw_mv + c0, v.mv, nc);
  cp(raw_hw + c0, v.has_write, nc);
  cp(t.imv + row0, v.input_mv, nrows);
  cp(t.bw, t.h_tab, 3 * nt * 8);
  if (staged_copy) t.image_pending = true;
  else launch_image(t, s, row0, nrows);
}

void sezkp_ctx::check_shape_same(const sezkp_block_view& v) const {
  if (v.tau != tau || v.n_blocks != nblk)
    throw Err{SEZKP_E_INVALID, "staged trace has another shape (tau / block count): call sezkp_ctx_upload"};
  if (nblk && memcmp(v.step_start, cur_step_start.data(), (size_t)(nblk + 1) * 8) != 0)
    throw Err{SEZKP_E_INVALID, "staged trace has other block boundaries: call sezkp_ctx_upload"};
  for (uint32_t k = 0; k < nblk; k++)
    if (v.step_hi[k] < v.step_lo[k] || v.step_hi[k] - v.step_lo[k] + 1 != v.step_start[k + 1] - v.step_start[k])
      throw Err{SEZKP_E_INVALID, "block " + std::to_string(k) + ": step range does not match its steps"};
// ... 331 lines not shown
    if (sharded() && coll_issued) {
      try {
        comm->wait(st, coll_timeout_s());
      } catch (const std::exception& e) {
        throw Err{SEZKP_E_DEVICE, std::string("rank ") + std::to_string(rank) + ": " + e.what()};
      }
    } else {
      HIP_OR_THROW(hipStreamSynchronize(st));
    }
    t_last = std::chrono::duration<double, std::milli>(clk::now() - t0).count();
    t_sync += t_last;
  };
  HIP_OR_THROW(hipSetDevice(device));
  const int k = logN;
  const bool kprobe = opt.kernel_events, stage_ev = opt.stage_events;
  auto rec = [&](int s) {
    if (stage_ev) HIP_OR_THROW(hipEventRecord(ev[s], st));
  };
  bool kdone = false;
  auto krec = [&](bool end) {
    if (!kprobe) return;
    HIP_OR_THROW(hipEventRecord(kev[end ? 1 : 0], st));
    if (end) kdone = true;
  };
  auto ok = [&](hipError_t e, const char* what) {
    if (e == hipSuccess && opt.sync_debug) e = hipStreamSynchronize(st);
    if (e != hipSuccess) throw Err{SEZKP_E_DEVICE, std::string(what) + ": " + hipGetErrorString(e)};
  };
  auto fork = [&](hipStream_t from, hipStream_t to, hipEvent_t e) {
    HIP_OR_THROW(hipEventRecord(e, from));
    HIP_OR_THROW(hipStreamWaitEvent(to, e, 0));
  };

  const bool sharded = this->sharded();
  const uint64_t S = 1ULL << L16_LOG;
  auto coll = [&](const char* name, uint64_t wire, auto&& issue) {
    fail_point(rank, name);
    while (coll_ev.size() < 2 * (coll_used + 1)) {
      hipEvent_t e;
      HIP_OR_THROW(hipEventCreate(&e));
      coll_ev.push_back(e);
    }
    hipEvent_t a = coll_ev[2 * coll_used], b = coll_ev[2 * coll_used + 1];
    coll_used++;
    HIP_OR_THROW(hipEventRecord(a, st));
    coll_issued = true;
    try {
      issue();
    } catch (const Err&) {
      throw;
    } catch (const std::exception& e) {
      throw Err{SEZKP_E_DEVICE, std::string(name) + ": " + e.what()};
    }
    HIP_OR_THROW(hipEventRecord(b, st));
    coll_stats.push_back(CollStat{name, wire, a, b});
    if (hook_match(opt.stall_after, rank, name)) {
      if (!stall_word) {
        HIP_OR_THROW(hipHostMalloc(&stall_word, 64, hipHostMallocMapped | hipHostMallocCoherent));
        *stall_word = 0;
      }
      HIP_OR_THROW(hipStreamWaitValue32(st, stall_word, 1, hipStreamWaitValueGte, 0xFFFFFFFFu));
    }
  };
  const uint64_t P1 = (uint64_t)world - 1;
  const uint64_t row_lo = n >= 1024 ? ch_lo << COL_CHUNK_LOG2 : 0;
  const uint64_t row_hi = n >= 1024 ? ch_hi << COL_CHUNK_LOG2 : n;
  const bool no_deep_poly = opt.no_deep_poly;
  const uint32_t dict_tab_cap = opt.dict_tab_cap;
  const uint64_t dict_plan_rows = opt.dict_plan_rows(row_hi - row_lo);
  {
    const bool cache_off = opt.dict_cache_off;
    DictHostKey hk;
    hk.n = n;
    hk.nrows = row_hi - row_lo;
    hk.row0 = row_lo;
    hk.plan_rows = dict_plan_rows;
    hk.tab_cap = dict_tab_cap;
    if (cache_off || dict_dirty || !(hk == dict_hkey)) dict_epoch++;
    dict_hkey = hk;
    dict_dirty = true;
    dict_seq++;
  }
  const DictCache dcache{d_dkeys, d_dreuse, d_dlvl_seq, d_dstatus, dict_epoch, dict_seq};
  uint32_t st_rebuilt = 0;
  uint64_t st_entries = 0;
  const int nguard = sharded ? comm->world : 1;
  auto check_guards = [&](const uint32_t* g_h, int ng) {
    for (int r = 0; r < ng; r++) {
      const uint32_t g = g_h[r];
      if (g) {
        const hipError_t me = hipMemsetAsync(d_err, 0, 64, st);
        if (me != hipSuccess) {
          broken = true;
          throw Err{SEZKP_E_DEVICE, std::string("guard word tripped (code ") + std::to_string(g) +
                                        ") and clearing it failed: " + hipGetErrorString(me) +
                                        "; the context is unusable"};
        }
      }
      const std::string who = " on rank " + std::to_string(sharded ? r : rank);
      if (g & GUARD_HEAD_RANGE) throw Err{SEZKP_E_INVALID, head_range_msg(who)};
      if (g) throw Err{SEZKP_E_DEVICE, "column commitment guard tripped" + who + " (code " + std::to_string(g) + ")"};
    }
  };
  Transcript tr("sezkp-stark/v1");
  const uint64_t shift_inv = hgl_inv(3);
  uint64_t z = 0, zn = 0;
  bool dq = false;
  const size_t gofs = sharded ? 8 : 0;
  const bool dist_intt = sharded && world > 1 && opt.dist_intt;
  DeepPoly dpoly{d_dq_rlo, d_dq_rhi, d_dq_rhk};
  std::vector<uint8_t> roots((size_t)(k + 1) * 32);
  uint64_t rows[NUM_QUERIES], frows[NUM_QUERIES];
  std::vector<uint64_t> pos((size_t)NUM_QUERIES * (k + 1));
  size_t nf = 0, no = 0;

  auto enqueue_A = [&]() {
    rec(0);
    ok(launch_expand(st, T, blk_lo, blk_cnt, d_err), "expand");
    rec(1);
    fork(st, st2, ev_expand);
    ok(launch_col_tables(st2, T, d_tmpl, d_tab_cols, n_tab_cols, tab_units, d_tabs, blk_lo, blk_cnt), "col_tables");
    ok(launch_col_commit(st2, T, d_tmpl, d_work, n_work, d_tabs, d_outer, outer_stride), "col_commit");
    ok(launch_col_commit_pw(st2, T, d_tmpl, d_pw_cols, n_pw_cols, d_pw_chunks, n_pw_chunks, d_tabs, d_outer,
                            outer_stride, d_err), "col_commit_pw");
    ok(launch_compose_terms(st2, T, Tm, row_lo, row_hi - row_lo), "compose_terms");
    HIP_OR_THROW(hipEventRecord(ev_cols, st2));
    ok(launch_dict_commit(st, T, d_tmpl, d_dcols, n_dict, d_dpart, d_dplans, d_dtabs, d_outer, outer_stride, row_lo,
                          row_hi - row_lo, d_dlev, dcache, dict_tab_cap, dict_plan_rows),
       "col_commit_dict");
    HIP_OR_THROW(hipStreamWaitEvent(st, ev_cols, 0));
    if (opt.trip_guard && opt.trip_guard_rank == rank) HIP_OR_THROW(hipMemsetAsync(d_err, 0x7f, 1, st));
    if (sharded) {
      const size_t bytes = (size_t)(ch_hi - ch_lo) * 32;
      coll("col_chunk_roots", P1 * (bytes * ncols + 4), [&] {
        comm->group_start();
        for (int c = 0; c < ncols; c++) {
          uint32_t* lvl0 = d_outer + (size_t)c * outer_stride * 8;
          comm->allgather(lvl0 + ch_lo * 8, lvl0, bytes, st);
        }
        comm->allgather(d_err, d_err + 8, 4, st);
        comm->group_end();
      });
    }
    rec(2);
    TreeDev outer0{d_outer, d_colroots, logChunks, 0};
    ok(launch_tree_upper(st, &outer0, ncols, outer_stride, 8, 0), "col_outer");
    rec(3);
    HIP_OR_THROW(hipMemcpyAsync(h_small, d_colroots,
                                n_dict ? (size_t)ncols * 32 + 4 * (16 + 2 * (size_t)n_dict)
                                       : (size_t)ncols * 32 + 4 * (gofs + nguard),
                                hipMemcpyDeviceToHost, st));
  };
  auto host_1 = [&]() {
    const uint32_t* colroots_h = h_small;
    check_guards(h_small + 8 * ncols + gofs, nguard);
    for (int c = 0; c < n_dict; c++) {
      st_rebuilt += h_small[8 * ncols + 16 + 2 * c];
      st_entries += h_small[8 * ncols + 16 + 2 * c + 1];
    }
    std::vector<uint8_t> colroots((const uint8_t*)colroots_h, (const uint8_t*)colroots_h + (size_t)ncols * 32);
    for (int c = 0; c < ncols; c++) memcpy(h_proof + root_pos[c], colroots.data() + 32 * c, 32);

    tr.absorb("manifest_root", mroot, 32);
    tr.absorb_u64("n", n);
    tr.absorb_u64("tau", tau);
    tr.absorb_u64("n_cols", (uint64_t)ncols);
    for (int c = 0; c < ncols; c++) tr.absorb("col_root", colroots.data() + 32 * c, 32);
    mark("tr_roots");
    auto ab = tr.challenge("alphas", 64);
    uint64_t a[8];
    for (int i = 0; i < 8; i++) a[i] = rd64(ab.data() + 8 * i) % GL_P_HOST;
    tr.absorb("masks", "masks", 5);
    tr.absorb_u64("n_masks", 1);
    tr.absorb_u64("deg", 4);
    uint64_t mask[4];
    for (int j = 0; j < 4; j++) mask[j] = rd64(tr.challenge("mask_coeff", 8).data()) % GL_P_HOST;
    z = rd64(tr.challenge("ood_point", 8).data()) % GL_P_HOST;
    for (;;) {
      uint64_t t = hgl_mul(z, shift_inv);
      for (int i = 0; i < k; i++) t = hgl_mul(t, t);
      if (t != 1) break;
      z = hgl_add(z, 1);
    }
    for (int i = 0; i < 8; i++) h_chal->alpha[i] = a[i];
    for (int j = 0; j < 4; j++) h_chal->mask[j] = mask[j];
    zn = hgl_pow(z, n);
    mark("z_done");
    mark("compose_issued");
    dq = logn >= 4 && z != 0 && zn != 1 && !no_deep_poly;
    if (dq) {
      const uint64_t K1 = hgl_mul(hgl_sub(1, zn), hgl_inv(n % GL_P_HOST));
      const uint64_t zN = hgl_pow(zn, N / n);
      uint64_t K2 = hgl_mul(hgl_pow(z, N - 1), hgl_inv(hgl_sub(hgl_pow(3, N), zN)));
      const int cP = full_lde ? 0 : logP;
      const uint64_t cg = full_lde ? 0 : (uint64_t)rank;
      const uint64_t M_ = N >> cP;
      const uint64_t rho = hgl_mul(hgl_mul(3, hgl_inv(z)), hgl_pow(hgl_root_2exp((uint32_t)logN), cg));
      const uint64_t rhoM = hgl_pow(rho, M_);
      uint64_t G = 0, pw = 1;
      for (int t = 0; t < (1 << cP); t++) {
        G = hgl_add(G, pw);
        pw = hgl_mul(pw, rhoM);
      }
      K2 = hgl_mul(K2, G);
      h_chal->z = z;
      h_chal->zn = zn;
      h_chal->K1 = K1;
      h_chal->K2 = K2;
      h_chal->rho = rho;
      h_chal->rho4096 = hgl_pow(rho, 4096);
      h_chal->K3 = hgl_mul(hgl_mul(zn, hgl_inv(z)), hgl_inv(n % GL_P_HOST));
    }
  };
  auto enqueue_B = [&]() {
    HIP_OR_THROW(hipMemcpyAsync(d_chal, h_chal, offsetof(DevChal, beta), hipMemcpyHostToDevice, st));
    const uint64_t dq_per = dq_rows_per_part(row_hi - row_lo);
    if (dq) {
      ok(launch_inv_base(st, Tm, d_base, d_dq_part, logn, d_chal, tw, row_lo, row_hi - row_lo, dq_per), "inv_base");
    } else {
      ok(launch_compose_combine(st, Tm, d_chal, tw, logn, d_base, row_lo, row_hi - row_lo), "compose");
      if (sharded && !dist_intt)
        coll("base_values", P1 * (row_hi - row_lo) * 8,
             [&] { comm->allgather(d_base + row_lo, d_base, (size_t)(row_hi - row_lo) * 8, st); });
    }
    rec(4);
    auto gather_fz = [&](uint64_t nrows) {
      if (dq) comm->allgather(d_dq_part + row_lo / dq_per, d_dq_part, (size_t)(nrows / dq_per) * 8, st);
    };
    if (dist_intt) {
      const uint64_t m = n >> logP, Q = m >> logP;
      if (row_lo != (uint64_t)rank * m || row_hi - row_lo != m) throw Err{SEZKP_E_INVALID, "sharded INTT: row split"};
      uint64_t* blk = d_base + row_lo;
      coll("intt_alltoall1", P1 * Q * 8, [&] { comm->alltoall(blk, d_lde, Q * 8, st); });
      ok(bintt_dft_twiddle(st, d_lde, world, Q, (uint32_t)rank, logn, tw), "intt_dft");
      coll("intt_alltoall2", P1 * Q * 8, [&] { comm->alltoall(d_lde, blk, Q * 8, st); });
      ok(ntt_dif(st, blk, logn - logP, true, tw), "intt_local");
      coll("intt_coeffs", P1 * (m * 8 + (dq ? m / dq_per * 8 : 0)), [&] {
        comm->group_start();
        comm->allgather(blk, d_base, m * 8, st);
        gather_fz(m);
        comm->group_end();
// ... 227 lines not shown
    ok(launch_fri_paths(st, d_layers, req, (int)nf_grid, PL), "fri_paths");
    mark("fri_paths_issued");
    if (sharded) {
      HIP_OR_THROW(hipStreamWaitEvent(st, ev_tail, 0));
      coll("proof_allreduce", 2 * P1 * PL.total / (uint64_t)world, [&] { comm->allreduce_sum_u8(PL.base, PL.total, st); });
    }
    rec(ST_PATHS + 1);
    const uint64_t d2h_from = sharded ? 0 : PL.fr_off;
    HIP_OR_THROW(hipMemcpyAsync(h_proof + hdr_bytes + d2h_from, (const uint8_t*)PL.base + d2h_from,
                                PL.total - d2h_from, hipMemcpyDeviceToHost, st));
    mark("proof_d2h_issued");
    HIP_OR_THROW(hipMemcpyAsync(h_small + 8 * (k + 1), lvals[k], 8, hipMemcpyDeviceToHost, st));
    if (!sharded) HIP_OR_THROW(hipStreamWaitEvent(st, ev_tail, 0));
    mark("issued");
  };

  enqueue_A();
  sync();
  mark("sync1");
  host_1();
  enqueue_B();
  sync();
  mark("sync2");
  host_2();
  enqueue_C();
  sync();
  mark("sync3");
  host_3();
  enqueue_D(nf, no);
  sync();
  mark("sync4");
  if (htrace) {
    for (auto& m : hmarks) fprintf(stderr, "%s %.1f ", m.first, m.second);
    fprintf(stderr, "\n");
  }
  for (int s = 0; s <= ST_NSTAGE; s++) stage_ms[s] = 0;
  if (stage_ev) {
    for (int s = 0; s < ST_NSTAGE; s++) {
      float ms = 0;
      if (hipEventElapsedTime(&ms, ev[s], ev[s + 1]) == hipSuccess) stage_ms[s] = ms;
    }
    float oms = 0;
    stage_ms[ST_OPEN] = hipEventElapsedTime(&oms, oev[0], oev[1]) == hipSuccess ? oms : 0.0;
    float tot = 0;
    (void)hipEventElapsedTime(&tot, ev[0], ev[ST_NSTAGE]);
    stage_ms[ST_NSTAGE] = tot;
  }
  {
    float ms = 0;
    kernel_ms = kdone && hipEventElapsedTime(&ms, kev[0], kev[1]) == hipSuccess ? ms : 0.0;
  }
  have_times = true;
  (void)hipGetLastError();
  const auto t_ser = clk::now();
  uint8_t* body = h_proof + hdr_bytes;
  auto put64 = [&](uint64_t at, uint64_t v) { memcpy(body + at, &v, 8); };
  put64(0, NUM_QUERIES);
  for (int q = 0; q < NUM_QUERIES; q++) {
    put64(8 + q * PL.q_bytes, rows[q]);
    put64(8 + q * PL.q_bytes + 8, tau);
  }
  put64(PL.fr_off, (uint64_t)k + 1);
  memcpy(body + PL.fr_off + 8, roots.data(), roots.size());
  put64(PL.fq_off, NUM_QUERIES);
  for (int q = 0; q < NUM_QUERIES; q++) {
    const uint64_t at = PL.fq_off + 8 + q * PL.fq_bytes;
    put64(at, (uint64_t)k + 1);
    for (int r = 0; r <= k; r++) put64(at + 8 + 8 * r, pos[(size_t)q * (k + 1) + r]);
    put64(at + 8 + 8 * (uint64_t)(k + 1), (uint64_t)k);
  }
  memcpy(body + PL.tail_off, h_small + 8 * (k + 1), 8);
  memcpy(body + PL.tail_off + 8, mroot, 32);
  const size_t out = hdr_bytes + PL.total;
  const auto t_end = clk::now();
  host_ms[0] = std::chrono::duration<double, std::milli>(t_end - t_enter).count();
  host_ms[1] = t_sync;
  host_ms[2] = t_last;
  host_ms[3] = std::chrono::duration<double, std::milli>(t_end - t_ser).count();
  have_plans = true;
  dict_dirty = false;
  dstat_rebuilt = st_rebuilt;
  dstat_reused = (uint32_t)n_dict - st_rebuilt;
  dstat_entries = st_entries;
  return out;
}

template <class F>
static int32_t guarded(char* err, size_t err_len, int32_t other, F&& body) {
  try {
    body();
    return SEZKP_OK;
  } catch (const Err& e) {
    set_err(err, err_len, e.msg);
    return e.code;
  } catch (const std::exception& e) {
    set_err(err, err_len, e.what());
    return other;
  }
}
static void require_idle(sezkp_ctx* ctx) {
  if (ctx->busy()) throw Err{SEZKP_E_INVALID, "a proof is in flight on this context (call sezkp_ctx_wait)"};
}

extern "C" {

uint32_t sezkp_abi_version(void) { return SEZKP_ABI_VERSION; }
const char* sezkp_version(void) { return "sezkp-mi355x 0.1.0 (stark-v1, gfx950)"; }

void sezkp_buf_free(sezkp_buf* b) {
  if (b && b->data) {
    free(b->data);
    b->data = nullptr;
    b->len = 0;
  }
}

static void to_buf(const std::vector<uint8_t>& v, sezkp_buf* out) {
  out->data = (uint8_t*)malloc(v.size() ? v.size() : 1);
  if (!out->data) throw Err{SEZKP_E_NOMEM, "out of host memory"};
  memcpy(out->data, v.data(), v.size());
  out->len = v.size();
}
static void to_buf(const std::string& s, sezkp_buf* out) { to_buf(std::vector<uint8_t>(s.begin(), s.end()), out); }

static sezkp_ctx* ctx_create(int32_t device, int32_t rank, int32_t world, const uint8_t* uid,
                             const sezkp_host_comm* hc, char* err, size_t err_len, bool solo = false) {
  try {
    if (world < 1 || world > 8 || (world & (world - 1)) || rank < 0 || rank >= world)
      throw Err{SEZKP_E_INVALID, "world must be a power of two <= 8 and 0 <= rank < world"};
    std::unique_ptr<sezkp_ctx> c(new sezkp_ctx());
    c->device = device;
    c->rank = rank;
    c->world = world;
    c->logP = ilog2((uint64_t)world);
    int cnt = 0;
    HIP_OR_THROW(hipGetDeviceCount(&cnt));
    if (device < 0 || device >= cnt) throw Err{SEZKP_E_DEVICE, "no such HIP device " + std::to_string(device)};
    HIP_OR_THROW(hipSetDevice(device));
    HIP_OR_THROW(hipStreamCreateWithFlags(&c->st, hipStreamNonBlocking));
    for (auto& e : c->ev) HIP_OR_THROW(hipEventCreate(&e));
    for (auto& e : c->kev) HIP_OR_THROW(hipEventCreate(&e));
    for (auto& e : c->oev) HIP_OR_THROW(hipEventCreate(&e));
    HIP_OR_THROW(hipStreamCreateWithFlags(&c->st2, hipStreamNonBlocking));
    HIP_OR_THROW(hipEventCreateWithFlags(&c->ev_fold, hipEventDisableTiming));
    HIP_OR_THROW(hipEventCreateWithFlags(&c->ev_tail, hipEventDisableTiming));
    HIP_OR_THROW(hipEventCreateWithFlags(&c->ev_expand, hipEventDisableTiming));
    HIP_OR_THROW(hipEventCreateWithFlags(&c->ev_cols, hipEventDisableTiming));
    HIP_OR_THROW(hipEventCreateWithFlags(&c->ev_qin, hipEventDisableTiming));
    HIP_OR_THROW(hipEventCreateWithFlags(&c->ev_qout, hipEventDisableTiming));
    c->tw = tables_for_device(device);
    const bool force = uid && getenv("SEZKP_FORCE_SHARDED") != nullptr;
    if (world > 1 || force || solo) {
      try {
        c->comm.reset(solo ? make_solo_comm(rank, world)
                           : hc ? make_host_comm(rank, world, *hc) : make_rccl_comm(rank, world, uid));
      } catch (const std::exception& e) {
        throw Err{SEZKP_E_DEVICE, e.what()};
      }
    }
    return c.release();
  } catch (const Err& e) {
    set_err(err, err_len, e.msg);
  } catch (const std::exception& e) {
    set_err(err, err_len, e.what());
  }
  return nullptr;
// ... 163 lines not shown
    AsyncSlot& a = *ctx->async;
    {
      std::lock_guard<std::mutex> lk(a.mu);
      if (a.state != AsyncSlot::IDLE)
        throw Err{SEZKP_E_INVALID, "a proof is already in flight on this context (call sezkp_ctx_wait)"};
      HIP_OR_THROW(hipSetDevice(ctx->device));
      ctx->take_staged();
      memcpy(a.root, manifest_root, 32);
      a.state = AsyncSlot::RUNNING;
    }
    a.cv.notify_all();
  });
}

int32_t sezkp_ctx_wait(sezkp_ctx* ctx, const uint8_t** data, size_t* len, char* err, size_t err_len) {
  if (!ctx || !data || !len) {
    set_err(err, err_len, "null argument");
    return SEZKP_E_INVALID;
  }
  if (!ctx->async) {
    set_err(err, err_len, "no proof in flight on this context");
    return SEZKP_E_INVALID;
  }
  AsyncSlot& a = *ctx->async;
  std::unique_lock<std::mutex> lk(a.mu);
  if (a.state == AsyncSlot::IDLE) {
    set_err(err, err_len, "no proof in flight on this context");
    return SEZKP_E_INVALID;
  }
  a.cv.wait(lk, [&] { return a.state == AsyncSlot::DONE; });
  a.state = AsyncSlot::IDLE;
  if (a.rc != SEZKP_OK) {
    set_err(err, err_len, a.msg);
    return a.rc;
  }
  *data = ctx->h_proof;
  *len = a.len;
  return SEZKP_OK;
}

int32_t sezkp_ctx_stage_times(const sezkp_ctx* ctx, double* out_ms, int32_t max) {
  if (!ctx || !ctx->have_times) return 0;
  int cnt = 0;
  for (int s = 0; s <= ST_NSTAGE && cnt < max; s++) out_ms[cnt++] = ctx->stage_ms[s];
  for (int s = 0; s < 4 && cnt < max; s++) out_ms[cnt++] = ctx->host_ms[s];
  if (cnt < max) out_ms[cnt++] = ctx->kernel_ms;
  return cnt;
}
void* sezkp_ctx_stream(const sezkp_ctx* ctx) { return ctx ? (void*)ctx->st : nullptr; }
int32_t sezkp_ctx_dict_plans(const sezkp_ctx* cctx, sezkp_dict_plan_info* out, int32_t max) {
  sezkp_ctx* ctx = const_cast<sezkp_ctx*>(cctx);
  if (!ctx || (max > 0 && !out) || max < 0) return SEZKP_E_INVALID;
  if (ctx->busy()) return SEZKP_E_INVALID;
  if (!ctx->loaded || !ctx->have_plans || ctx->n_dict == 0) return 0;
  const int32_t cnt = std::min<int32_t>(max, ctx->n_dict);
  if (cnt == 0) return 0;
  std::vector<DictPlan> pl((size_t)cnt);
  if (hipSetDevice(ctx->device) != hipSuccess ||
      hipMemcpy(pl.data(), ctx->d_dplans, (size_t)cnt * sizeof(DictPlan), hipMemcpyDeviceToHost) != hipSuccess) {
    (void)hipGetLastError();
    return SEZKP_E_DEVICE;
  }
  for (int32_t i = 0; i < cnt; i++) {
    sezkp_dict_plan_info& o = out[i];
    o = ctx->dict_info[(size_t)i];
    o.K = pl[i].K;
    o.a = pl[i].a;
    o.delta = pl[i].delta;
    o.R = pl[i].R;
    o.dR = pl[i].delta ? pl[i].dR : 0;
    o.min = pl[i].min;
  }
  return cnt;
}
int32_t sezkp_ctx_dict_cache_stats(const sezkp_ctx* cctx, uint32_t* cols_rebuilt, uint32_t* cols_reused,
                                   uint64_t* entries_rebuilt) {
  sezkp_ctx* ctx = const_cast<sezkp_ctx*>(cctx);
  if (!ctx || !cols_rebuilt || !cols_reused || !entries_rebuilt) return SEZKP_E_INVALID;
  if (ctx->busy()) return SEZKP_E_INVALID;
  const bool have = ctx->loaded && ctx->have_plans && ctx->n_dict != 0;
  *cols_rebuilt = have ? ctx->dstat_rebuilt : 0;
  *cols_reused = have ? ctx->dstat_reused : 0;
  *entries_rebuilt = have ? ctx->dstat_entries : 0;
  return SEZKP_OK;
}
int32_t sezkp_ctx_comm_stats(const sezkp_ctx* ctx, sezkp_comm_stat* out, int32_t max) {
  if (!ctx || !out || max <= 0) return 0;
  int32_t cnt = 0;
  for (const auto& c : ctx->coll_stats) {
    if (cnt >= max) break;
    sezkp_comm_stat& o = out[cnt++];
    memset(o.name, 0, sizeof o.name);
    strncpy(o.name, c.name, sizeof o.name - 1);
    o.bytes = c.bytes;
    float ms = 0;
    o.ms = hipEventElapsedTime(&ms, c.a, c.b) == hipSuccess ? ms : -1.0;
  }
  (void)hipGetLastError();
  return cnt;
}

int32_t sezkp_ctx_dist_ntt(sezkp_ctx* ctx, uint64_t* local, uint64_t* scratch, uint32_t log_n, int32_t dir,
                           char* err, size_t err_len) {
  return guarded(err, err_len, SEZKP_E_DEVICE, [&] {
    if (!ctx || !local || !scratch) throw Err{SEZKP_E_INVALID, "null argument"};
    require_idle(ctx);
    if (ctx->broken) throw Err{SEZKP_E_DEVICE, "context unusable after an aborted collective"};
    if (dir != 1 && dir != -1) throw Err{SEZKP_E_INVALID, "dir must be +1 or -1"};
    const int P = ctx->world, logP = ctx->logP;
    if (log_n > 32 || (int)log_n < 8 + logP)
      throw Err{SEZKP_E_INVALID, "dist_ntt needs 2^(8 + log P) <= n <= 2^32"};
    HIP_OR_THROW(hipSetDevice(ctx->device));
    hipStream_t st = ctx->st;
    const int logM = (int)log_n - logP;
    const uint64_t M = 1ULL << logM, Q = M >> logP;
    const uint64_t e_step = (uint64_t)ctx->rank << (32 - log_n);
    const bool inv = dir < 0;
    auto ok = [](hipError_t e, const char* what) {
      if (e != hipSuccess) throw Err{SEZKP_E_DEVICE, std::string(what) + ": " + hipGetErrorString(e)};
    };
    const uint64_t inv_n = inv ? hgl_inv((1ULL << log_n) % GL_P_HOST) : 1;
    hipError_t nat_err = hipSuccess;
    if (P == 1 && ntt_dif_natural(st, local, scratch, logM, inv, ctx->tw, inv_n, &nat_err)) {
      ok(nat_err, "dist_ntt local");
    } else if (P == 1) {
      if (!inv) {
        ok(ntt_dif(st, local, logM, false, ctx->tw), "dist_ntt local");
        ok(bitrev_inplace(st, local, logM, 1, false), "dist_ntt bitrev");
      } else {
        ok(bitrev_inplace(st, local, logM, inv_n, true), "dist_ntt bitrev");
        ok(ntt_dit(st, local, logM, true, ctx->tw, nullptr, 0, 1), "dist_ntt local");
      }
    } else if (!inv) {
      ok(ntt_dif(st, local, logM, false, ctx->tw), "dist_ntt local");
      ok(dntt_permute_twiddle(st, local, scratch, logM, ctx->tw, e_step, false, false, 1), "dist_ntt twiddle");
      ctx->comm->alltoall(scratch, local, Q * 8, st);
      ok(dntt_dft(st, local, P, Q, false), "dist_ntt dft");
    } else {
      ok(dntt_dft(st, local, P, Q, true), "dist_ntt dft");
      ctx->comm->alltoall(local, scratch, Q * 8, st);
      ok(dntt_permute_twiddle(st, scratch, local, logM, ctx->tw, e_step, true, true, inv_n), "dist_ntt twiddle");
      ok(ntt_dit(st, local, logM, true, ctx->tw, nullptr, 0, 1), "dist_ntt local");
    }
  });
}

static std::vector<MetaEntry> meta_for(uint64_t domain_n, uint32_t tau, uint32_t flags) {
  std::vector<MetaEntry> m = {{"proto", true, "stark-v1", 0}, {"domain_n", false, "", domain_n}, {"tau", false, "", tau}};
  if (flags & SEZKP_FLAG_STREAMING) m.push_back({"mode", true, "streaming", 0});
  return m;
}

int32_t sezkp_stark_v1_prove(const sezkp_block_view* blocks, const uint8_t manifest_root[32], uint32_t flags,
                             sezkp_buf* proof_bytes, sezkp_buf* meta_json, char* err, size_t err_len) {
  sezkp_ctx* ctx = sezkp_ctx_create(0, err, err_len);
  if (!ctx) return SEZKP_E_DEVICE;
  int32_t rc = sezkp_ctx_upload(ctx, blocks, err, err_len);
  if (rc == SEZKP_OK) rc = sezkp_ctx_prove(ctx, manifest_root, flags, proof_bytes, err, err_len);
  if (rc == SEZKP_OK && meta_json) {
    try {
      to_buf(meta_to_json(meta_for(ctx->N, ctx->tau, flags)), meta_json);
    } catch (const Err& e) {
      set_err(err, err_len, e.msg);
      rc = e.code;
    }
  }
// ... 387 lines not shown
```

### streaming-zero-knowledge-proofs_amd/csrc/sezkp_internal.h

```cpp
#pragma once
#include <hip/hip_runtime.h>
#include <stddef.h>
#include <stdint.h>

#include <vector>

#include "plan_types.h"

namespace sezkp {

struct DevChal;
struct ComposeTerms;

struct NttTables {
  const uint64_t* hi;
  const uint64_t* lo;
  const uint64_t* p3_hi;
  const uint64_t* p3_lo;
  int K;
  int S;
};

struct NttPassArgs {
  uint64_t* a;
  const uint64_t* src;
  NttTables tw;
  uint64_t inv_n;
  uint64_t coset_e;
  int m, sL, logC, inverse, skip, log_src;
  int src_logP;
  uint64_t deep_z;
  int deep_logN, deep_logP;
  uint32_t deep_g;
  const uint64_t* dp_rlo;
  const uint64_t* dp_rhi;
  const uint64_t* dp_rhk;
  int dp_logN;
  uint64_t* out;
  int nat_out, nat_logN;
  uint64_t out_scale;
  int nat_tr;
};
struct DeepFuse {
  uint64_t z;
  int logN, logP;
  uint32_t g;
};
struct DeepPoly {
  const uint64_t* rlo;
  const uint64_t* rhi;
  const uint64_t* rhk;
};
uint64_t dq_rows_per_part(uint64_t nrows);
hipError_t launch_inv_base(hipStream_t st, const ComposeTerms& Tm, uint64_t* D, uint64_t* partial, int logn,
                           const DevChal* ch, const NttTables& T, uint64_t row0, uint64_t nrows, uint64_t per);
hipError_t launch_q_tables(hipStream_t st, const uint64_t* partial, int logn, int logN, const DevChal* ch,
                           uint64_t* rlo, uint64_t* rhi, uint64_t* rhk, uint64_t per);

hipError_t ntt_dif(hipStream_t st, uint64_t* a, int logN, bool inverse, const NttTables& T);
bool ntt_dif_natural(hipStream_t st, uint64_t* a, uint64_t* scratch, int logN, bool inverse, const NttTables& T,
                     uint64_t scale, hipError_t* err);
hipError_t ntt_dit(hipStream_t st, uint64_t* a, int logN, bool inverse, const NttTables& T,
                   const uint64_t* src, int log_src, uint64_t inv_n, uint64_t coset_e = 0,
                   const DeepFuse* deep = nullptr, bool* fused = nullptr, const DeepPoly* dpoly = nullptr,
                   int src_logP = 0);
hipError_t bitrev_permute(hipStream_t st, const uint64_t* in, uint64_t* out, int logN, uint64_t scale,
                          bool do_scale);
hipError_t bitrev_inplace(hipStream_t st, uint64_t* a, int logN, uint64_t scale, bool do_scale);
hipError_t dntt_permute_twiddle(hipStream_t st, const uint64_t* in, uint64_t* out, int logM, const NttTables& T,
                                uint64_t e_step, bool inverse, bool tw_src, uint64_t scale);
hipError_t dntt_dft(hipStream_t st, uint64_t* r, int P, uint64_t Q, bool inverse);
hipError_t bintt_dft_twiddle(hipStream_t st, uint64_t* r, int P, uint64_t Q, uint32_t d, int logn,
                             const NttTables& T);

struct TraceDev {
  uint64_t n;
  int tau;
  uint32_t nblk;
  const int8_t* input_mv;
  const int8_t* mv;
  const uint8_t* wflag;
  const uint16_t* wsym;
  const uint64_t* blk_start;
  const uint64_t* blk_winlen;
  const uint64_t* blk_offin;
  const uint64_t* blk_offout;
  uint32_t* row_blk;
  uint8_t* row_flags;
  int32_t* head;
  int64_t* head_rng;
};

struct ComposeTerms {
  uint64_t* hr;
  uint64_t* sl;
  int64_t* c3;
  int32_t* c2;
  int32_t* sy;
  uint64_t* bf;
  uint64_t* bl;
  const uint8_t* row_flags;
  const uint32_t* row_blk;
};

constexpr int AIR_FAMILIES = 5;
enum AuditWord {
  AUD_CELLS = 0,
  AUD_ROWS = AIR_FAMILIES,
  AUD_NVIOL = 2 * AIR_FAMILIES,
  AUD_NREJ,
  AUD_KEY,
  AUD_FVIOL = AUD_KEY + AIR_FAMILIES,
  AUD_FREJ,
  AUD_VALUE,
  AUD_GUARD = AUD_VALUE + AIR_FAMILIES,
  AUD_WORDS
};
struct AirAuditOut {
  uint64_t* cnt;
  uint64_t* viol;
  uint64_t* rej;
};
hipError_t launch_air_audit(hipStream_t st, const TraceDev& T, const AirAuditOut& O, const uint32_t* d_err);

constexpr uint32_t GUARD_HEAD_RANGE = 0x100u;

struct Alphas {
  uint64_t bool_flag, mv_domain, head_update, head_bits_bool, head_reconstruct, slack_bits_bool,
      slack_reconstruct, sym_bits_bool, sym_reconstruct, boundary_first, boundary_last;
};

struct DictPlan {
  int64_t min;
  uint32_t R;
  int32_t K;
  uint32_t pw[DICT_LEVELS];
  uint32_t delta;
  int64_t dmin;
  uint32_t dR;
  uint32_t a;
};
struct DictKey {
  int64_t lo, hi, mlo, mhi;
  uint64_t epoch;
};
struct DictCache {
  DictKey* keys;
  uint32_t* reuse;
  uint64_t* lvl_seq;
  uint32_t* status;
  uint64_t epoch;
  uint64_t seq;
};
__host__ __device__ inline int dlev_base(int level) { return level == 6 ? 0 : level == 7 ? 16 : level == 8 ? 24 : 28; }
__host__ __device__ inline int dict_extra(int K) { return K >= 3 ? 2 : (K == 2 ? 1 : 0); }
struct DevChal {
  uint64_t alpha[8];
  uint64_t mask[4];
  uint64_t z, zn, K1, K2, rho, rho4096;
  uint64_t K3;
  uint64_t beta[FS_MAX_BETAS];
};

hipError_t launch_trace_image(hipStream_t st, const int8_t* raw_mv, const uint8_t* raw_hw, const uint16_t* raw_ws,
                              uint64_t n, int tau, int8_t* mv, uint8_t* wf, uint16_t* ws, uint64_t r0 = 0,
                              uint64_t r1 = ~0ull);
hipError_t launch_expand(hipStream_t st, const TraceDev& T, uint32_t blk_lo, uint32_t blk_cnt, uint32_t* d_err);
hipError_t launch_col_tables(hipStream_t st, const TraceDev& T, const ColTemplate* d_tmpl, const uint32_t* d_tab_cols,
                             int n_tab_cols, uint64_t tab_entries, uint32_t* tabs, uint32_t blk_lo, uint32_t blk_cnt);
hipError_t launch_col_commit(hipStream_t st, const TraceDev& T, const ColTemplate* d_tmpl, const uint32_t* d_work,
                             int nwork, const uint32_t* tabs, uint32_t* outer_nodes, uint64_t outer_stride_nodes);
hipError_t launch_dict_commit(hipStream_t st, const TraceDev& T, const ColTemplate* d_tmpl, const DictCol* d_dcols,
                              int ndict, int64_t* d_part, DictPlan* d_plans, uint32_t* d_dtabs, uint32_t* outer_nodes,
                              uint64_t outer_stride_nodes, uint64_t row0, uint64_t nrows, uint32_t* d_dlev,
// ... 90 lines not shown
```

### streaming-zero-knowledge-proofs_amd/csrc/trace.hip

```cpp
#include <type_traits>

#include "dev_common.h"
#include "col_leaf.h"
#include "sezkp_internal.h"
#include "compose.h"

namespace sezkp {

constexpr int TR_THREADS = 256;

__global__ void __launch_bounds__(TR_THREADS) k_trace_image(const int8_t* __restrict__ raw_mv,
                                                          const uint8_t* __restrict__ raw_hw,
                                                          const uint16_t* __restrict__ raw_ws, uint64_t n, int tau,
                                                          int8_t* __restrict__ mv, uint8_t* __restrict__ wf,
                                                          uint16_t* __restrict__ ws, uint64_t r0, uint64_t r1) {
  const uint64_t s = r0 + (uint64_t)blockIdx.x * TR_THREADS + threadIdx.x;
  if (s >= r1) return;
  const size_t i0 = (size_t)s * tau;
  for (int r = 0; r < tau; r++) {
    const size_t o = (size_t)r * n + s;
    const bool w = raw_hw[i0 + r] != 0;
    mv[o] = raw_mv[i0 + r];
    wf[o] = w ? 1 : 0;
    ws[o] = w ? raw_ws[i0 + r] : 0;
// ... 184 lines not shown
      for (int j = 0; j < 4; j++) v[j] = gl_from_i64((int8_t)(w >> (8 * j)));
      return;
    }
    case 1:
    case 2: {
      uint32_t w = *reinterpret_cast<const uint32_t*>(T.row_flags + row0);
      const int sh = ct.kind - 1;
#pragma unroll
      for (int j = 0; j < 4; j++) v[j] = (w >> (8 * j + sh)) & 1;
      return;
    }
    case 3: {
      uint32_t w = *reinterpret_cast<const uint32_t*>(T.mv + o);
#pragma unroll
      for (int j = 0; j < 4; j++) v[j] = gl_from_i64((int8_t)(w >> (8 * j)));
      return;
    }
    case 4: {
      uint32_t w = *reinterpret_cast<const uint32_t*>(T.wflag + o);
#pragma unroll
      for (int j = 0; j < 4; j++) v[j] = (w >> (8 * j)) & 0xff;
      return;
    }
    case 5: {
      uint2 w = *reinterpret_cast<const uint2*>(T.wsym + o);
      v[0] = w.x & 0xffff; v[1] = w.x >> 16; v[2] = w.y & 0xffff; v[3] = w.y >> 16;
      return;
    }
    case 6: {
      const int4 a = *reinterpret_cast<const int4*>(T.head + o);
      v[0] = gl_from_i64(a.x); v[1] = gl_from_i64(a.y); v[2] = gl_from_i64(a.z); v[3] = gl_from_i64(a.w);
      return;
    }
    default: {
      const uint64_t* tab = ct.kind == 7 ? T.blk_winlen : (ct.kind == 8 ? T.blk_offin : T.blk_offout);
      tab += (uint64_t)ct.tape * T.nblk;
      uint4 bl = *reinterpret_cast<const uint4*>(T.row_blk + row0);
      v[0] = tab[bl.x]; v[1] = tab[bl.y]; v[2] = tab[bl.z]; v[3] = tab[bl.w];
      return;
    }
  }
}

template <int OFF>
__device__ __forceinline__ void leaf_labeled_t(const ColTemplate& ct, uint64_t v, uint32_t (&out)[8]) {
  uint32_t m[16];
#pragma unroll
  for (int i = 0; i < 16; i++) m[i] = ct.words[i];
  constexpr int W = OFF / 4, B = OFF % 4;
  const uint32_t lo = (uint32_t)v, hi = (uint32_t)(v >> 32);
  if (B == 0) {
    m[W] |= lo;
    m[W + 1] |= hi;
  } else {
    m[W] |= lo << (8 * B);
    m[W + 1] |= (lo >> (32 - 8 * B)) | (hi << (8 * B));
    m[W + 2] |= hi >> (32 - 8 * B);
  }
  b3_hash_block(m, OFF + 8, out);
}
template <int OFF>
__device__ __forceinline__ void leaf_labeled(const ColTemplate& ct, uint64_t v, uint32_t (&out)[8]) {
  if constexpr (OFF == 0) leaf_labeled_rt(ct, v, out);
  else leaf_labeled_t<OFF>(ct, v, out);
}

__device__ __forceinline__ void lds_put8(uint32_t (*lds)[TR_THREADS], int i, const uint32_t (&h)[8]) {
#pragma unroll
  for (int w = 0; w < 8; w++) lds[w][i] = h[w];
}

template <int OFF>
__device__ __forceinline__ void hash4_labeled(const ColTemplate& ct, const uint64_t (&v)[4], uint32_t (&h)[8]) {
  uint32_t a[8], b[8], p0[8], p1[8];
  leaf_labeled<OFF>(ct, v[0], a);
  leaf_labeled<OFF>(ct, v[1], b);
  b3_parent(a, b, p0);
  leaf_labeled<OFF>(ct, v[2], a);
  leaf_labeled<OFF>(ct, v[3], b);
  b3_parent(a, b, p1);
  b3_parent(p0, p1, h);
}

__global__ void __launch_bounds__(TR_THREADS) k_col_tables(TraceDev T, const ColTemplate* __restrict__ tmpl,
                                                           const uint32_t* __restrict__ cols, uint32_t* __restrict__ tabs,
                                                           uint32_t blk_lo, uint32_t blk_cnt) {
  const ColTemplate ct = tmpl[cols[blockIdx.y]];
  uint64_t i = (uint64_t)blockIdx.x * TR_THREADS + threadIdx.x;
  uint32_t h[8];
  if (kind_has_leaf_table(ct.kind)) {
    if (i >= (1ULL << ct.tab_log)) return;
    const uint64_t v = (ct.kind == 0 || ct.kind == 3) ? gl_from_i64((int8_t)(uint8_t)i) : i;
    leaf_labeled_rt(ct, v, h);
    node_store(tabs + 8 * (ct.tab + i), h);
    return;
  }
  const bool flags = ct.kind == 1 || ct.kind == 2;
  if (flags ? i >= 2 : i >= blk_cnt) return;
  if (!flags) i += blk_lo;
  uint64_t v;
  if (ct.kind == 1 || ct.kind == 2) v = i;
  else {
    const uint64_t* tab = ct.kind == 7 ? T.blk_winlen : (ct.kind == 8 ? T.blk_offin : T.blk_offout);
    v = tab[(uint64_t)ct.tape * T.nblk + i];
  }
  leaf_labeled_rt(ct, v, h);
  uint32_t* o = tabs + 8 * (ct.tab + i * U_LEVELS);
  node_store(o, h);
  for (int l = 1; l < U_LEVELS; l++) {
    b3_parent(h, h, h);
    node_store(o + 8 * l, h);
  }
}

__device__ __forceinline__ void col_index4(const TraceDev& T, const ColTemplate& ct, uint64_t row0, uint32_t (&ix)[4]) {
  const uint64_t o = (uint64_t)ct.tape * T.n + row0;
  if (ct.kind == 5) {
    uint2 w = *reinterpret_cast<const uint2*>(T.wsym + o);
    ix[0] = w.x & 0xffff; ix[1] = w.x >> 16; ix[2] = w.y & 0xffff; ix[3] = w.y >> 16;
    return;
  }
  const uint8_t* src = ct.kind == 0 ? reinterpret_cast<const uint8_t*>(T.input_mv) + row0
                     : ct.kind == 3 ? reinterpret_cast<const uint8_t*>(T.mv) + o : T.wflag + o;
  uint32_t w = *reinterpret_cast<const uint32_t*>(src);
#pragma unroll
  for (int j = 0; j < 4; j++) ix[j] = (w >> (8 * j)) & 0xff;
}

template <int OFF>
__device__ __forceinline__ void commit_body(const TraceDev& T, const ColTemplate& ct, uint64_t row0, uint32_t (&h)[8]) {
  uint64_t v[4];
  col_values4(T, ct, row0, v);
  hash4_labeled<OFF>(ct, v, h);
}

__global__ void __launch_bounds__(TR_THREADS) k_col_commit(TraceDev T, const ColTemplate* __restrict__ tmpl,
                                                           const uint32_t* __restrict__ work,
                                                           const uint32_t* __restrict__ tabs,
                                                           uint32_t* __restrict__ outer, uint64_t outer_stride) {
  __shared__ uint32_t lds[8][TR_THREADS];
  const int c = work[2 * blockIdx.x];
  const uint64_t ch = work[2 * blockIdx.x + 1];
  const ColTemplate ct = tmpl[c];
  const int tid = threadIdx.x;
  const uint64_t n = T.n;
  const uint64_t cl = n < 1024 ? n : 1024;
  int logcl = 0;
  while ((1ULL << logcl) < cl) logcl++;
  const int logper = logcl < 2 ? logcl : 2;
  const int nact = (int)(cl >> logper);
  if (tid < nact) {
    const uint64_t row0 = (ch << COL_CHUNK_LOG2) + ((uint64_t)tid << logper);
    uint32_t h[8];
    if (logper == 2 && kind_has_leaf_table(ct.kind)) {
      uint32_t ix[4], a[8], b[8], p0[8], p1[8];
      col_index4(T, ct, row0, ix);
      const uint32_t* tb = tabs + 8 * ct.tab;
      node_load(tb + 8 * ix[0], a);
      node_load(tb + 8 * ix[1], b);
      b3_parent(a, b, p0);
      node_load(tb + 8 * ix[2], a);
      node_load(tb + 8 * ix[3], b);
      b3_parent(a, b, p1);
      b3_parent(p0, p1, h);
    } else if (logper == 2) {
      switch (ct.off) {
        case 16: commit_body<16>(T, ct, row0, h); break;
        case 17: commit_body<17>(T, ct, row0, h); break;
        case 18: commit_body<18>(T, ct, row0, h); break;
        case 19: commit_body<19>(T, ct, row0, h); break;
        case 20: commit_body<20>(T, ct, row0, h); break;
        case 21: commit_body<21>(T, ct, row0, h); break;
        case 22: commit_body<22>(T, ct, row0, h); break;
        case 23: commit_body<23>(T, ct, row0, h); break;
        default: commit_body<0>(T, ct, row0, h); break;
      }
    } else if (logper == 1) {
      uint32_t a[8], b[8];
      leaf_labeled_rt(ct, col_value(T, ct, row0), a);
      leaf_labeled_rt(ct, col_value(T, ct, row0 + 1), b);
      b3_parent(a, b, h);
    } else {
      leaf_labeled_rt(ct, col_value(T, ct, row0), h);
    }
    lds_put8(lds, tid, h);
  }
  __syncthreads();
  int cnt = nact;
  while (cnt > 1) {
    const int half = cnt >> 1;
    uint32_t h[8];
    const bool act = tid < half;
    if (act) {
      uint32_t l[8], r[8];
#pragma unroll
      for (int w = 0; w < 8; w++) {
        uint2 p = *reinterpret_cast<const uint2*>(&lds[w][2 * tid]);
        l[w] = p.x;
        r[w] = p.y;
      }
      b3_parent(l, r, h);
    }
    __syncthreads();
    if (act) lds_put8(lds, tid, h);
    __syncthreads();
    cnt = half;
  }
  if (tid < 8) outer[(uint64_t)c * outer_stride * 8 + ch * 8 + tid] = lds[tid][0];
}

constexpr int PW_THREADS = 64;
constexpr int PW_STACK = 12;
__global__ void __launch_bounds__(PW_THREADS) k_col_commit_pw(TraceDev T, const ColTemplate* __restrict__ tmpl,
                                                              const uint32_t* __restrict__ pw_cols, int n_pw,
                                                              const uint32_t* __restrict__ chunks, int nchunks,
                                                              const uint32_t* __restrict__ tabs,
                                                              uint32_t* __restrict__ outer, uint64_t outer_stride,
                                                              uint32_t* __restrict__ err) {
  __shared__ uint32_t stk[PW_STACK][8][PW_THREADS];
  const int lane = threadIdx.x;
  const uint64_t item = (uint64_t)blockIdx.x * PW_THREADS + lane;
  if (item >= (uint64_t)n_pw * nchunks) return;
  const uint32_t c = pw_cols[item / nchunks];
  const uint64_t ch = chunks[item % nchunks];
  const uint32_t kind = tmpl[c].kind;
  const uint32_t* U = tabs + 8 * tmpl[c].tab;
  const uint64_t n = T.n;
  const uint64_t cl = n < 1024 ? n : 1024;
  const uint64_t c0 = ch << COL_CHUNK_LOG2, c1 = c0 + cl;
  int logcl = 0;
  while ((1ULL << logcl) < cl) logcl++;
  uint64_t lvpack = 0;
  int sp = 0;
  uint32_t k = T.row_blk[c0];
  uint64_t row = c0;
  while (row < c1) {
    if (k >= T.nblk) { atomicOr(err, 4u); return; }
    const uint64_t bs = T.blk_start[k], be = T.blk_start[k + 1];
    if (be <= row) { k++; continue; }
    const uint64_t pe = be < c1 ? be : c1;
    uint64_t cut = pe;
    uint32_t u = k;
    if (kind == 1) { u = row == bs ? 1u : 0u; cut = row == bs ? row + 1 : pe; }
    else if (kind == 2) { u = row + 1 == be ? 1u : 0u; cut = (row + 1 < be && pe == be) ? be - 1 : pe; }
    while (row < cut) {
      const uint64_t off = row - c0, len = cut - row;
      int l = off ? __builtin_ctzll(off) : logcl;
      if (l > logcl) l = logcl;
      while ((1ULL << l) > len) l--;
      const uint64_t step = 1ULL << l;
      uint32_t h[8];
      node_load(U + 8 * ((uint64_t)u * U_LEVELS + l), h);
      while (sp > 0 && (int)((lvpack >> (4 * (sp - 1))) & 15) == l) {
        uint32_t left[8];
#pragma unroll
        for (int w = 0; w < 8; w++) left[w] = stk[sp - 1][w][lane];
        b3_parent(left, h, h);
        sp--;
        l++;
      }
      if (sp >= PW_STACK) { atomicOr(err, 8u); return; }
#pragma unroll
      for (int w = 0; w < 8; w++) stk[sp][w][lane] = h[w];
      lvpack = (lvpack & ~(15ULL << (4 * sp))) | ((uint64_t)l << (4 * sp));
      sp++;
      row += step;
    }
  }
  if (sp != 1) { atomicOr(err, 16u); return; }
#pragma unroll
  for (int w = 0; w < 8; w++) outer[(uint64_t)c * outer_stride * 8 + ch * 8 + w] = stk[0][w][lane];
}

template <int RW>
__global__ void __launch_bounds__(TR_THREADS) k_compose_terms(TraceDev T, ComposeTerms Tm, uint64_t row0,
                                                              uint64_t row_end) {
  static_assert(RW == 1 || RW == 2 || RW == 4, "1, 2 or 4 rows per lane");
  using Narrow = typename std::conditional<RW == 1, uint8_t,
                                           typename std::conditional<RW == 2, uint16_t, uint32_t>::type>::type;
  using Wide = typename std::conditional<RW == 1, uint16_t,
                                         typename std::conditional<RW == 2, uint32_t, uint64_t>::type>::type;
  const uint64_t n = T.n;
  const uint64_t i = row0 + RW * ((uint64_t)blockIdx.x * TR_THREADS + threadIdx.x);
  if (i >= row_end) return;
  const uint64_t inx = (i + RW) & (n - 1);
  const Narrow flw = *reinterpret_cast<const Narrow*>(T.row_flags + i);
  uint32_t blk[RW];
  bool is_first[RW], is_last[RW];
  if constexpr (RW == 1) {
    blk[0] = T.row_blk[i];
  } else {
#pragma unroll
    for (int j = 0; j < RW; j += 2) {
      const uint2 b2 = *reinterpret_cast<const uint2*>(T.row_blk + i + j);
      blk[j] = b2.x;
      blk[j + 1] = b2.y;
    }
  }
#pragma unroll
  for (int j = 0; j < RW; j++) {
    is_first[j] = (flw >> (8 * j)) & 1;
    is_last[j] = (flw >> (8 * j + 1)) & 1;
  }
  int32_t s_c2[RW], s_sy[RW];
  int64_t s_c3[RW];
  uint64_t s_bf[RW], s_bl[RW], hr_lo[RW], sl_lo[RW];
  uint32_t hr_hi[RW], sl_hi[RW];
#pragma unroll
  for (int j = 0; j < RW; j++) {
    s_c2[j] = s_sy[j] = 0;
    s_c3[j] = 0;
    s_bf[j] = s_bl[j] = hr_lo[j] = sl_lo[j] = 0;
    hr_hi[j] = sl_hi[j] = 0;
  }
  for (int r = 0; r < T.tau; r++) {
    const uint64_t o = (uint64_t)r * n;
    const Narrow mvw = *reinterpret_cast<const Narrow*>(T.mv + o + i);
    const Narrow wfw = *reinterpret_cast<const Narrow*>(T.wflag + o + i);
    const Wide wsw = *reinterpret_cast<const Wide*>(T.wsym + o + i);
    int64_t head[RW + 1];
    if constexpr (RW == 1) {
      head[0] = T.head[o + i];
    } else {
#pragma unroll
      for (int j = 0; j < RW; j += 2) {
// ... 422 lines not shown
    } else {
      uint32_t a[8], b[8];
      node_load(t1 + 8 * (uint64_t)(c0 + (int64_t)R * (hp[g + 1] - mn)), a);
      node_load(t1 + 8 * (uint64_t)((hp[g + 2] - mn) + (int64_t)R * (hp[g + 3] - mn)), b);
      b3_parent(a, b, h);
    }
  }
  struct Raw {
    uint32_t f, m;
    int64_t h0;
  };
  __device__ __forceinline__ Raw raw(int j) const {
    const uint64_t g = (uint64_t)j << 2;
    return Raw{*reinterpret_cast<const uint32_t*>(fp + g), *reinterpret_cast<const uint32_t*>(mp + g), hp[g]};
  }
  __device__ __forceinline__ void node(const Raw& r, int j, uint32_t (&h)[8]) const {
    const int64_t c0 = r.h0 - mn;
    if (!(r.f & 0x01010100u)) {
      const int64_t d1 = (int64_t)(int8_t)(r.m >> 8) - dmin, d2 = (int64_t)(int8_t)(r.m >> 16) - dmin,
                    d3 = (int64_t)(int8_t)(r.m >> 24) - dmin;
      node_load(td + 8 * (uint64_t)(c0 + (int64_t)R * (d1 + (int64_t)dR * (d2 + (int64_t)dR * d3))), h);
    } else {
      const uint64_t g = (uint64_t)j << 2;
      uint32_t a[8], b[8];
      node_load(t1 + 8 * (uint64_t)(c0 + (int64_t)R * (hp[g + 1] - mn)), a);
      node_load(t1 + 8 * (uint64_t)((hp[g + 2] - mn) + (int64_t)R * (hp[g + 3] - mn)), b);
      b3_parent(a, b, h);
    }
  }
};
template <typename Key>
struct RawLeaves {
  const Key* p;
  const ColTemplate* ct;
  __device__ __forceinline__ void get(int j, uint32_t (&h)[8]) const {
    leaf_labeled_rt(*ct, gl_from_i64((int64_t)p[j]), h);
  }
};

template <int L, int D>
__device__ __forceinline__ void counter_push(uint32_t (&s)[D > 0 ? D : 1][8], uint32_t (&x)[8], int j,
                                             uint32_t (&h)[8]) {
  if constexpr (L == D) {
#pragma unroll
    for (int w = 0; w < 8; w++) h[w] = x[w];
  } else {
    if ((j >> L) & 1) {
      b3_parent(s[L], x, x);
      counter_push<L + 1, D>(s, x, j, h);
    } else {
#pragma unroll
      for (int w = 0; w < 8; w++) s[L][w] = x[w];
    }
  }
}

template <int D, class Prov>
__device__ __forceinline__ void lane_tree(const Prov& P, uint32_t (&h)[8]) {
  uint32_t s[D > 0 ? D : 1][8];
  for (int j = 0; j < (1 << D); j++) {
    uint32_t x[8];
    P.get(j, x);
    counter_push<0, D>(s, x, j, h);
  }
}
template <int D, class Prov>
__device__ __forceinline__ void lane_tree_pf(const Prov& P, uint32_t (&h)[8]) {
  constexpr int N = 1 << D;
  uint32_t s[D > 0 ? D : 1][8];
  uint32_t nx[8];
  typename Prov::Raw k1 = P.raw(0);
  P.node(k1, 0, nx);
  if (N > 1) k1 = P.raw(1);
  for (int j = 0; j < N; j++) {
    uint32_t x[8];
#pragma unroll
    for (int w = 0; w < 8; w++) x[w] = nx[w];
    if (j + 1 < N) P.node(k1, j + 1, nx);
    if (j + 2 < N) k1 = P.raw(j + 2);
    counter_push<0, D>(s, x, j, h);
  }
}

__device__ __forceinline__ bool pw_range_hash(const TraceDev& T, uint32_t kind, const uint32_t* __restrict__ U,
                                              uint64_t r0, int lw, uint32_t (*stk)[8][64], int slot,
                                              uint32_t (&out)[8]) {
  const uint64_t c1 = r0 + (1ULL << lw);
  uint64_t lvpack = 0;
  int sp = 0;
  uint32_t k = T.row_blk[r0];
  uint64_t row = r0;
  while (row < c1) {
    if (k >= T.nblk) return false;
    const uint64_t bs = T.blk_start[k], be = T.blk_start[k + 1];
    if (be <= row) { k++; continue; }
    const uint64_t pe = be < c1 ? be : c1;
    uint64_t cut = pe;
    uint32_t u = k;
    if (kind == 1) { u = row == bs ? 1u : 0u; cut = row == bs ? row + 1 : pe; }
    else if (kind == 2) { u = row + 1 == be ? 1u : 0u; cut = (row + 1 < be && pe == be) ? be - 1 : pe; }
    while (row < cut) {
      const uint64_t off = row - r0, len = cut - row;
      int l = off ? __builtin_ctzll(off) : lw;
      if (l > lw) l = lw;
      while ((1ULL << l) > len) l--;
      const uint64_t step = 1ULL << l;
      uint32_t h[8];
      node_load(U + 8 * ((uint64_t)u * U_LEVELS + l), h);
      while (sp > 0 && (int)((lvpack >> (4 * (sp - 1))) & 15) == l) {
        uint32_t left[8];
#pragma unroll
        for (int w = 0; w < 8; w++) left[w] = stk[sp - 1][w][slot];
        b3_parent(left, h, h);
        sp--;
        l++;
      }
      if (sp >= PW_STACK) return false;
#pragma unroll
      for (int w = 0; w < 8; w++) stk[sp][w][slot] = h[w];
      lvpack = (lvpack & ~(15ULL << (4 * sp))) | ((uint64_t)l << (4 * sp));
      sp++;
      row += step;
    }
  }
  if (sp != 1) return false;
#pragma unroll
  for (int w = 0; w < 8; w++) out[w] = stk[0][w][slot];
  return true;
}

__device__ __forceinline__ void dict_node_at(const TraceDev& T, const ColTemplate& ct, const DictPlan& P,
                                             const uint32_t* __restrict__ tab, uint64_t row, uint32_t (&h)[8]) {
  if (P.delta) {
    const uint64_t o = (uint64_t)ct.tape * T.n + row;
    DeltaNodes{T.head + o, T.mv + o, T.row_flags + row, tab + 8 * (uint64_t)DICT_CAP, tab + 16 * (uint64_t)DICT_CAP,
               P.min, P.dmin, P.R, P.dR}
        .get(0, h);
    return;
  }
#define SEZKP_DN(KEY)                                                                                           \
  {                                                                                                             \
    const KEY* p = dict_keys<KEY>(T, ct) + row;                                                                 \
    switch (P.K) {                                                                                              \
      case 0: DictNodes<KEY, 0>{p, tab, P.min, P.R}.get(0, h); break;                                           \
      case 1: DictNodes<KEY, 1>{p, tab + 8 * (uint64_t)DICT_CAP, P.min, P.R}.get(0, h); break;                  \
      case 2: DictNodes<KEY, 2>{p, tab + 16 * (uint64_t)DICT_CAP, P.min, P.R}.get(0, h); break;                 \
      case 3: DictNodes<KEY, 3>{p, tab + 24 * (uint64_t)DICT_CAP, P.min, P.R}.get(0, h); break;                 \
      default: DictNodes<KEY, 4>{p, tab + 32 * (uint64_t)DICT_CAP, P.min, P.R}.get(0, h); break;                \
    }                                                                                                           \
  }
  switch (ct.kind) {
    case 0: case 3: SEZKP_DN(int8_t) break;
    case 4: SEZKP_DN(uint8_t) break;
    case 5: SEZKP_DN(uint16_t) break;
    default: SEZKP_DN(int32_t) break;
  }
#undef SEZKP_DN
}

__device__ __forceinline__ void copy_dlev_siblings(const uint32_t* __restrict__ lev, uint64_t in, int glog,
                                                   uint32_t* __restrict__ o) {
  const int lvl = glog + (threadIdx.x >> 3), w = threadIdx.x & 7;
  if (lvl < COL_CHUNK_LOG2) o[18 + 8 * lvl + w] = lev[8 * (dlev_base(lvl) + ((in >> lvl) ^ 1)) + w];
}

__global__ void __launch_bounds__(TR_THREADS) k_col_open(TraceDev T, const ColTemplate* __restrict__ tmpl,
                                                         const uint32_t* __restrict__ outer, uint64_t outer_stride,
                                                         int logChunks, const uint32_t* __restrict__ req,
                                                         ProofLayout P, const uint32_t* __restrict__ tabs,
                                                         const uint32_t* __restrict__ dlev,
                                                         const DictPlan* __restrict__ plans,
                                                         const uint32_t* __restrict__ dtabs,
                                                         const DictCol* __restrict__ dcols) {
  __shared__ uint32_t lds[8][1024];
  const uint32_t* rq = req + OPEN_REQ_WORDS * (uint64_t)blockIdx.x;
  const int c = rq[0];
  const uint64_t row = (uint64_t)rq[1] | ((uint64_t)rq[2] << 32);
  const uint32_t q = rq[3];
  const uint32_t dsel = rq[4];
  const ColTemplate ct = tmpl[c];
  const int tid = threadIdx.x;
  const uint64_t n = T.n;
  const uint64_t ch = row >> COL_CHUNK_LOG2;
  const uint64_t start = ch << COL_CHUNK_LOG2;
  const uint64_t cl = n < 1024 ? n : 1024;
  int logcl = 0;
  while ((1ULL << logcl) < cl) logcl++;
  const uint32_t qi = q / P.open_per_q, s = q % P.open_per_q;
  uint32_t* qb = P.base + (8 + (uint64_t)qi * P.q_bytes) / 4;
  uint32_t* o = qb + (16 + (uint64_t)s * P.open_bytes) / 4;
  const uint64_t in = row - start;
  if (tid == 0) {
    o[2] = (uint32_t)row; o[3] = (uint32_t)(row >> 32);
    o[4] = (uint32_t)ch; o[5] = (uint32_t)(ch >> 32);
    o[6] = (uint32_t)in; o[7] = 0;
    o[16] = (uint32_t)logcl; o[17] = 0;
    o[18 + 8 * logcl] = (uint32_t)logChunks; o[19 + 8 * logcl] = 0;
    const uint64_t v = col_value(T, ct, row);
    o[0] = (uint32_t)v;
    o[1] = (uint32_t)(v >> 32);
  }
  const uint32_t* ob = outer + (uint64_t)c * outer_stride * 8;
  {
    uint32_t* op = o + 20 + 8 * logcl;
    const int lvl = tid >> 3, w = tid & 7;
    if (lvl < logChunks) op[8 * lvl + w] = ob[8 * (tree_level_off(logChunks, 0, lvl) + ((ch >> lvl) ^ 1)) + w];
  }
  const bool pw = kind_piecewise(ct.kind) && ct.tab != NO_TAB;
  const bool dict = dsel != NO_DICT && logcl == COL_CHUNK_LOG2;
  const int K = dict ? plans[dsel].K : -1;
  if (pw) {
    if (tid < logcl) {
      uint32_t h[8];
      const uint64_t rs = start + (((in >> tid) ^ 1) << tid);
      if (pw_range_hash(T, ct.kind, tabs + 8 * (uint64_t)ct.tab, rs, tid,
                        reinterpret_cast<uint32_t(*)[8][64]>(&lds[0][0]), tid, h)) {
#pragma unroll
        for (int w = 0; w < 8; w++) o[18 + 8 * tid + w] = h[w];
      }
    }
    if (tid < 8) o[8 + tid] = ob[8 * ch + tid];
  } else if (dict && K >= 0) {
    const DictPlan Pl = plans[dsel];
    const uint32_t* tab = dtabs + 8 * dcols[dsel].tab;
    const int glog = DICT_LANE_LOG + (int)plans[dsel].a;
    const int D = glog - K;
    const uint64_t gstart = row & ~((1ULL << glog) - 1);
    for (int j = tid; j < (1 << D); j += TR_THREADS) {
      uint32_t h[8];
      dict_node_at(T, ct, Pl, tab, gstart + ((uint64_t)j << K), h);
#pragma unroll
      for (int w = 0; w < 8; w++) lds[w][j] = h[w];
    }
    if (tid < K) {
      const int l = tid;
      const uint64_t rs = ((row >> l) ^ 1) << l;
      uint64_t idx = 0;
      for (int i = (1 << l) - 1; i >= 0; i--) idx = idx * Pl.R + (uint64_t)(dict_key_at(T, ct, rs + i) - Pl.min);
      const uint32_t* e = tab + 8 * ((uint64_t)l * DICT_CAP + idx);
#pragma unroll
      for (int w = 0; w < 8; w++) o[18 + 8 * l + w] = e[w];
    }
    __syncthreads();
    const uint64_t gin = (row - gstart) >> K;
    int cnt = 1 << D;
    for (int lvl = K; lvl < glog; lvl++) {
      const int sib = (int)((gin >> (lvl - K)) ^ 1);
      if (tid < 8) o[18 + 8 * lvl + tid] = lds[tid][sib];
      if (lvl + 1 == glog) break;
      const int half = cnt >> 1;
      const int pq = tid >> 2, qq = tid & 3;
      uint32_t lo = 0, hi = 0;
      if (pq < half) lds_parent_quad(lds, pq, qq, lo, hi);
      __syncthreads();
      if (pq < half) {
        lds[qq][pq] = lo;
        lds[4 + qq][pq] = hi;
      }
      __syncthreads();
      cnt = half;
    }
    const uint32_t* lev = dlev + 8 * ((uint64_t)dsel * (T.n >> COL_CHUNK_LOG2) + ch) * DLEV_NODES;
    copy_dlev_siblings(lev, in, glog, o);
    if (tid < 8) o[8 + tid] = ob[8 * ch + tid];
  } else {
    const int glog = dict ? DICT_LANE_LOG + (int)plans[dsel].a : logcl;
    const uint64_t gstart = dict ? (row & ~((1ULL << glog) - 1)) : start;
    for (uint64_t i = tid; i < (1ULL << glog); i += TR_THREADS) {
      uint32_t h[8];
      leaf_labeled_rt(ct, col_value(T, ct, gstart + i), h);
#pragma unroll
      for (int w = 0; w < 8; w++) lds[w][i] = h[w];
    }
    __syncthreads();
    const uint64_t gin = row - gstart;
    int cnt = 1 << glog;
    for (int lvl = 0; lvl < glog; lvl++) {
      const int sib = (int)((gin >> lvl) ^ 1);
      if (tid < 8) o[18 + 8 * lvl + tid] = lds[tid][sib];
      const int half = cnt >> 1;
      uint32_t hh[2][8];
      int k = 0;
      for (int p = tid; p < half; p += TR_THREADS, k++) {
        uint32_t a[8], b[8];
#pragma unroll
        for (int w = 0; w < 8; w++) { a[w] = lds[w][2 * p]; b[w] = lds[w][2 * p + 1]; }
        b3_parent(a, b, hh[k]);
      }
      __syncthreads();
      k = 0;
      for (int p = tid; p < half; p += TR_THREADS, k++)
#pragma unroll
        for (int w = 0; w < 8; w++) lds[w][p] = hh[k][w];
      __syncthreads();
      cnt = half;
    }
    if (dict) {
      const uint32_t* lev = dlev + 8 * ((uint64_t)dsel * (T.n >> COL_CHUNK_LOG2) + ch) * DLEV_NODES;
// ... 286 lines not shown
    switch (ct.kind) {
      case 0: case 3: dict_lane<int8_t>(dict_keys<int8_t>(T, ct) + lrow, P, tab, ctp, h); break;
      case 4: dict_lane<uint8_t>(dict_keys<uint8_t>(T, ct) + lrow, P, tab, ctp, h); break;
      case 5: dict_lane<uint16_t>(dict_keys<uint16_t>(T, ct) + lrow, P, tab, ctp, h); break;
      default:
        if (P.delta) {
          const uint64_t o = (uint64_t)ct.tape * T.n + lrow;
          const DeltaNodes dn{T.head + o, T.mv + o, T.row_flags + lrow, tab + 8 * (uint64_t)DICT_CAP,
                              tab + 16 * (uint64_t)DICT_CAP, P.min, P.dmin, P.R, P.dR};
          if (a == 1) lane_tree_pf<5>(dn, h);
          else lane_tree_pf<4>(dn, h);
        } else {
          dict_lane<int32_t>(dict_keys<int32_t>(T, ct) + lrow, P, tab, ctp, h);
        }
        break;
    }
#pragma unroll
    for (int w = 0; w < 8; w++) lds[0][w][lane] = h[w];
    node_store(dl + 8 * ((lrow >> COL_CHUNK_LOG2) * DLEV_NODES + dlev_base(llog) +
                         ((lrow >> llog) & ((1u << (COL_CHUNK_LOG2 - llog)) - 1))),
               h);
  }
  __syncthreads();
  int cnt = DICT_WG_LANES, cur = 0;
  for (int lv = llog + 1; lv <= COL_CHUNK_LOG2; lv++) {
    const int half = cnt >> 1;
    const uint64_t prow = wg_row + ((uint64_t)lane << lv);
    if (lane < half && prow < row_end) {
      uint32_t l[8], r[8], h[8];
#pragma unroll
      for (int w = 0; w < 8; w++) {
        const uint2 pr = *reinterpret_cast<const uint2*>(&lds[cur][w][2 * lane]);
        l[w] = pr.x;
        r[w] = pr.y;
      }
      b3_parent(l, r, h);
#pragma unroll
      for (int w = 0; w < 8; w++) lds[cur ^ 1][w][lane] = h[w];
      if (lv < COL_CHUNK_LOG2)
        node_store(dl + 8 * ((prow >> COL_CHUNK_LOG2) * DLEV_NODES + dlev_base(lv) +
                             ((prow >> lv) & ((1u << (COL_CHUNK_LOG2 - lv)) - 1))),
                   h);
    }
    __syncthreads();
    cur ^= 1;
    cnt = half;
  }
  for (int i = lane; i < cnt * 8; i += DICT_WG_LANES) {
    const uint64_t ch = (wg_row >> COL_CHUNK_LOG2) + (i >> 3);
    if (ch < nch_all && (ch << COL_CHUNK_LOG2) < row_end)
      outer[(uint64_t)dc.col * outer_stride * 8 + ch * 8 + (i & 7)] = lds[cur][i & 7][i >> 3];
  }
}

hipError_t launch_trace_image(hipStream_t st, const int8_t* raw_mv, const uint8_t* raw_hw, const uint16_t* raw_ws,
                              uint64_t n, int tau, int8_t* mv, uint8_t* wf, uint16_t* ws, uint64_t r0, uint64_t r1) {
  if (r1 > n) r1 = n;
  if (r0 >= r1 || tau <= 0) return hipSuccess;
  if (tau == 8) {
    r0 &= ~7ull;
    const uint64_t g8 = ((r1 - r0 + 7) / 8 + TR_THREADS - 1) / TR_THREADS;
    if (g8 > 0x7FFFFFFFull) return hipErrorInvalidValue;
    hipLaunchKernelGGL(k_trace_image8, dim3((unsigned)g8), dim3(TR_THREADS), 0, st, raw_mv, raw_hw, raw_ws, n, mv, wf,
                       ws, r0, r1);
    return hipGetLastError();
  }
  const uint64_t g = (r1 - r0 + TR_THREADS - 1) / TR_THREADS;
  if (g > 0x7FFFFFFFull) return hipErrorInvalidValue;
  hipLaunchKernelGGL(k_trace_image, dim3((unsigned)g), dim3(TR_THREADS), 0, st, raw_mv, raw_hw, raw_ws, n, tau, mv,
                     wf, ws, r0, r1);
  return hipGetLastError();
}
hipError_t launch_expand(hipStream_t st, const TraceDev& T, uint32_t blk_lo, uint32_t blk_cnt, uint32_t* d_err) {
  if (blk_cnt == 0) return hipSuccess;
  if ((uint64_t)blk_lo + blk_cnt > T.nblk) return hipErrorInvalidValue;
  hipLaunchKernelGGL(k_expand, dim3(blk_cnt), dim3(TR_THREADS), 0, st, T, blk_lo, d_err);
  return hipGetLastError();
}
hipError_t launch_col_tables(hipStream_t st, const TraceDev& T, const ColTemplate* d_tmpl, const uint32_t* d_tab_cols,
                             int n_tab_cols, uint64_t max_units, uint32_t* tabs, uint32_t blk_lo, uint32_t blk_cnt) {
  if (n_tab_cols == 0) return hipSuccess;
  if ((uint64_t)blk_lo + blk_cnt > T.nblk) return hipErrorInvalidValue;
  const unsigned gx = (unsigned)((max_units + TR_THREADS - 1) / TR_THREADS);
  hipLaunchKernelGGL(k_col_tables, dim3(gx, n_tab_cols), dim3(TR_THREADS), 0, st, T, d_tmpl, d_tab_cols, tabs, blk_lo,
                     blk_cnt);
  return hipGetLastError();
}
static hipError_t dict_shape_ok(const TraceDev& T, uint64_t row0, uint64_t nrows) {
  if (T.n < (1ULL << COL_CHUNK_LOG2)) return hipErrorInvalidValue;
  if (row0 + nrows > T.n || (nrows != T.n && (row0 % DICT_WG_ROWS || nrows % DICT_WG_ROWS))) return hipErrorInvalidValue;
  return hipSuccess;
}
hipError_t launch_dict_commit(hipStream_t st, const TraceDev& T, const ColTemplate* d_tmpl, const DictCol* d_dcols,
                              int ndict, int64_t* d_part, DictPlan* d_plans, uint32_t* d_dtabs, uint32_t* outer_nodes,
                              uint64_t outer_stride_nodes, uint64_t row0, uint64_t nrows, uint32_t* d_dlev,
                              const DictCache& dc, uint32_t tab_cap, uint64_t plan_rows) {
  if (ndict == 0) return hipSuccess;
  hipError_t e = dict_shape_ok(T, row0, nrows);
  if (e != hipSuccess) return e;
  if (tab_cap == 0 || tab_cap > DICT_CAP) return hipErrorInvalidValue;
  const int sweeps = (int)std::max<uint64_t>(1, std::min<uint64_t>(8, nrows / (64ull * DICT_RANGE_STEP)));
  const uint64_t prow = (uint64_t)sweeps * DICT_RANGE_STEP;
  const uint32_t nparts = (uint32_t)((nrows + prow - 1) / prow);
  hipLaunchKernelGGL(k_dict_range, dim3(nparts, ndict), dim3(TR_THREADS), 0, st, T, d_tmpl, d_dcols, d_part, nparts,
                     row0, row0 + nrows, sweeps);
  if ((e = hipGetLastError()) != hipSuccess) return e;
  hipLaunchKernelGGL(k_dict_plan, dim3(ndict), dim3(TR_THREADS), 0, st, d_part, nparts, T.n,
                     plan_rows ? plan_rows : nrows, d_dcols, d_plans, tab_cap, dc);
  if ((e = hipGetLastError()) != hipSuccess) return e;
  for (int l = 0; l < DICT_LEVELS; l++) {
    for (int c0 = 0; c0 < ndict; c0 += DICT_FLAT_MAX) {
      const int nc = ndict - c0 < DICT_FLAT_MAX ? ndict - c0 : DICT_FLAT_MAX;
      hipLaunchKernelGGL(k_dict_level, dim3(DICT_FLAT_WGS), dim3(TR_THREADS), 0, st, d_tmpl, d_dcols + c0,
                         d_plans + c0, dc.reuse + c0, dc.lvl_seq, dc.seq, d_dtabs, nc, l);
      if ((e = hipGetLastError()) != hipSuccess) return e;
    }
  }
  const uint64_t wg_rows = (uint64_t)DICT_WG_LANES << DICT_LANE_LOG;
  const unsigned gx = (unsigned)((nrows + wg_rows - 1) / wg_rows);
  hipLaunchKernelGGL(k_col_commit_dict, dim3(gx, ndict), dim3(DICT_WG_LANES), 0, st, T, d_tmpl, d_dcols, d_plans, d_dtabs,
                     outer_nodes, outer_stride_nodes, row0, row0 + nrows, d_dlev);
  return hipGetLastError();
}

hipError_t launch_col_commit(hipStream_t st, const TraceDev& T, const ColTemplate* d_tmpl, const uint32_t* d_work,
                             int nwork, const uint32_t* tabs, uint32_t* outer_nodes, uint64_t outer_stride_nodes) {
  if (nwork == 0) return hipSuccess;
  hipLaunchKernelGGL(k_col_commit, dim3(nwork), dim3(TR_THREADS), 0, st, T, d_tmpl, d_work, tabs, outer_nodes,
                     outer_stride_nodes);
  return hipGetLastError();
}
hipError_t launch_col_commit_pw(hipStream_t st, const TraceDev& T, const ColTemplate* d_tmpl, const uint32_t* d_pw_cols,
                                int n_pw_cols, const uint32_t* d_chunks, int nchunks, const uint32_t* tabs,
                                uint32_t* outer_nodes, uint64_t outer_stride_nodes, uint32_t* d_err) {
  if (nchunks == 0 || n_pw_cols == 0) return hipSuccess;
  const uint64_t items = (uint64_t)n_pw_cols * nchunks;
  hipLaunchKernelGGL(k_col_commit_pw, dim3((unsigned)((items + PW_THREADS - 1) / PW_THREADS)), dim3(PW_THREADS), 0, st,
                     T, d_tmpl, d_pw_cols, n_pw_cols, d_chunks, nchunks, tabs, outer_nodes, outer_stride_nodes, d_err);
  return hipGetLastError();
}
hipError_t launch_compose_terms(hipStream_t st, const TraceDev& T, const ComposeTerms& Tm, uint64_t row0,
                                uint64_t nrows) {
  if (row0 + nrows > T.n) return hipErrorInvalidValue;
  if (nrows == 0) return hipSuccess;
  const char* rw_s = getenv("SEZKP_COMPOSE_ROWS");
  int rw = rw_s ? atoi(rw_s) : 2;
  if (rw != 1 && rw != 2 && rw != 4) rw = 2;
  while (rw > 1 && (T.n < (uint64_t)rw || (row0 | nrows) % rw)) rw >>= 1;
  const unsigned g = (unsigned)((nrows / rw + TR_THREADS - 1) / TR_THREADS);
  if (rw == 4) hipLaunchKernelGGL(k_compose_terms<4>, dim3(g), dim3(TR_THREADS), 0, st, T, Tm, row0, row0 + nrows);
  else if (rw == 2) hipLaunchKernelGGL(k_compose_terms<2>, dim3(g), dim3(TR_THREADS), 0, st, T, Tm, row0, row0 + nrows);
  else hipLaunchKernelGGL(k_compose_terms<1>, dim3(g), dim3(TR_THREADS), 0, st, T, Tm, row0, row0 + nrows);
  return hipGetLastError();
}
hipError_t launch_compose_combine(hipStream_t st, const ComposeTerms& Tm, const DevChal* ch, const NttTables& tw,
                                  int logn, uint64_t* out, uint64_t row0, uint64_t nrows) {
  const unsigned grid = (unsigned)((nrows + TR_THREADS - 1) / TR_THREADS);
  if (grid == 0) return hipSuccess;
  hipLaunchKernelGGL(k_compose_combine, dim3(grid), dim3(TR_THREADS), 0, st, Tm, ch, tw, logn, out, row0,
                     row0 + nrows);
  return hipGetLastError();
}
hipError_t launch_air_audit(hipStream_t st, const TraceDev& T, const AirAuditOut& O, const uint32_t* d_err) {
  if (T.n == 0 || T.tau < 0 || T.tau > 256 || !O.cnt || !O.viol || !O.rej) return hipErrorInvalidValue;
  hipError_t e = hipMemsetAsync(O.cnt, 0, AUD_WORDS * 8, st);
  if (e != hipSuccess) return e;
  const char* rw_s = getenv("SEZKP_AUDIT_ROWS");
  int rw = rw_s ? atoi(rw_s) : AUD_ROWS_PER_LANE;
// ... 24 lines not shown
```

### streaming-zero-knowledge-proofs_amd/sezkp_amd/_lib.py

```python
from __future__ import annotations

import ctypes as C
import os

PKG_ROOT = os.path.dirname(os.path.dirname(os.path.abspath(__file__)))
LIB_PATH = os.path.join(PKG_ROOT, "lib", "libsezkp_stark.so")

SEZKP_OK = 0
SEZKP_E_INVALID = -1
SEZKP_E_DEVICE = -2
SEZKP_E_NOMEM = -3
SEZKP_E_DECODE = -4
SEZKP_E_VERIFY = -5
SEZKP_FLAG_STREAMING = 1
ABI_VERSION = 4

EXPORTS = [
    "sezkp_abi_version", "sezkp_version", "sezkp_buf_free", "sezkp_stark_v1_prove",
    "sezkp_stark_v1_prove_artifact_cbor", "sezkp_stark_v1_verify", "sezkp_ctx_create", "sezkp_ctx_destroy",
    "sezkp_ctx_upload", "sezkp_ctx_prove", "sezkp_ctx_stage_times", "sezkp_ctx_stream", "sezkp_gl_ntt",
    "sezkp_gl_coset_lde_deep", "sezkp_fri_fold_commit", "sezkp_merkle_root_u64", "sezkp_manifest_root",
    "sezkp_blocks_decode_cbor", "sezkp_blocks_view", "sezkp_blocks_free", "sezkp_blake3",
    "sezkp_comm_unique_id", "sezkp_ctx_create_sharded", "sezkp_ctx_create_sharded_host", "sezkp_ctx_prove_borrow",
    "sezkp_blocks_decode_jsonl", "sezkp_blocks_encode_jsonl", "sezkp_manifest_decode", "sezkp_ctx_dist_ntt",
    "sezkp_blocks_encode_cbor", "sezkp_simulate_trace", "sezkp_simulate_blocks",
    "sezkp_ctx_prove_async", "sezkp_ctx_wait", "sezkp_ctx_stage", "sezkp_host_register", "sezkp_host_unregister",
    "sezkp_fri_fold", "sezkp_blake3_leaves_u64", "sezkp_blake3_leaves_labeled", "sezkp_merkle_node_count",
    "sezkp_merkle_build", "sezkp_merkle_paths", "sezkp_manifest_frontier_root", "sezkp_ctx_comm_stats",
    "sezkp_fs_xof", "sezkp_ctx_upload_rows", "sezkp_shard_rows", "sezkp_blocks_decode_jsonl_meta",
    "sezkp_blocks_line_offsets", "sezkp_manifest_leaf_hashes", "sezkp_merkle_root_of_leaves",
    "sezkp_ctx_create_sharded_solo", "sezkp_blocks_decode_jsonl_lines", "sezkp_ctx_dict_plans",
    "sezkp_ctx_air_audit", "sezkp_stark_v1_air_audit", "sezkp_ctx_dict_cache_stats",
    "sezkp_ctx_verify_batch", "sezkp_stark_v1_verify_batch", "sezkp_ctx_verify_times",
]

AIR_FAMILIES = ("mv_domain", "head_range", "slack_range", "sym_range", "boundary")


class AirFamilyC(C.Structure):
    _fields_ = [("cells", C.c_uint64), ("rows", C.c_uint64), ("first_row", C.c_uint64), ("first_tape", C.c_uint32),
                ("pad", C.c_uint32), ("first_value", C.c_uint64)]


class AirAuditC(C.Structure):
    _fields_ = [("n_rows", C.c_uint64), ("tau", C.c_uint32), ("pad", C.c_uint32), ("rows_violating", C.c_uint64),
                ("first_violating", C.c_uint64), ("rows_rejectable", C.c_uint64), ("first_rejectable", C.c_uint64),
                ("fam", AirFamilyC * len(AIR_FAMILIES))]


class ProofRef(C.Structure):
    _fields_ = [("bytes", C.c_void_p), ("len", C.c_size_t), ("manifest_root", C.c_void_p), ("tau", C.c_uint32),
                ("pad", C.c_uint32)]


class VerifyResultC(C.Structure):
    _fields_ = [("code", C.c_int32), ("pad", C.c_uint32), ("msg", C.c_char * 248)]


VERIFY_TIMES = ("parse_ms", "pack_ms", "device_wall_ms", "h2d_ms", "kernel_ms", "d2h_ms", "decide_ms", "wall_ms",
                "jobs", "slices")


class CommStat(C.Structure):
    _fields_ = [("name", C.c_char * 32), ("bytes", C.c_uint64), ("ms", C.c_double)]


class DictPlanInfo(C.Structure):
    _fields_ = [("col", C.c_uint32), ("kind", C.c_uint32), ("tape", C.c_uint32), ("K", C.c_int32),
                ("a", C.c_uint32), ("delta", C.c_uint32), ("R", C.c_uint32), ("dR", C.c_uint32),
                ("min", C.c_int64)]


class SezkpError(RuntimeError):
    def __init__(self, code: int, msg: str):
        super().__init__(f"[{code}] {msg}")
        self.code = code


class Buf(C.Structure):
    _fields_ = [("data", C.POINTER(C.c_uint8)), ("len", C.c_size_t)]


VIEW_FIELDS = [
    ("version", C.c_uint16), ("block_id", C.c_uint32), ("step_lo", C.c_uint64), ("step_hi", C.c_uint64),
    ("ctrl_in", C.c_uint16), ("ctrl_out", C.c_uint16), ("in_head_in", C.c_int64), ("in_head_out", C.c_int64),
    ("win_left", C.c_int64), ("win_right", C.c_int64), ("off_in", C.c_uint32), ("off_out", C.c_uint32),
    ("step_start", C.c_uint64), ("input_mv", C.c_int8), ("mv", C.c_int8), ("has_write", C.c_uint8),
    ("wsym", C.c_uint16),
]


ALLGATHER_FN = C.CFUNCTYPE(C.c_int32, C.c_void_p, C.c_void_p, C.c_void_p, C.c_size_t)
ALLTOALL_FN = C.CFUNCTYPE(C.c_int32, C.c_void_p, C.c_void_p, C.c_void_p, C.c_size_t)
ALLREDUCE_FN = C.CFUNCTYPE(C.c_int32, C.c_void_p, C.c_void_p, C.c_size_t)


class HostComm(C.Structure):
    _fields_ = [("user", C.c_void_p), ("allgather", ALLGATHER_FN), ("alltoall", ALLTOALL_FN),
                ("allreduce_sum_u8", ALLREDUCE_FN)]


class BlockView(C.Structure):
    _fields_ = [("n_blocks", C.c_uint32), ("tau", C.c_uint32)] + [(f, C.POINTER(t)) for f, t in VIEW_FIELDS]


def _one_hip_runtime() -> None:
    try:
        import torch
    except ImportError:
        pass


def _load():
    _one_hip_runtime()
    if not os.path.exists(LIB_PATH):
        raise ImportError(f"{LIB_PATH} not built: run `make -C {PKG_ROOT}` (or __graft_entry__.build())")
    L = C.CDLL(LIB_PATH)
    L.sezkp_abi_version.restype = C.c_uint32
    if L.sezkp_abi_version() != ABI_VERSION:
        raise ImportError(f"{LIB_PATH} has C ABI {L.sezkp_abi_version()}, this module binds ABI {ABI_VERSION}: "
                          f"rebuild it (make -C {PKG_ROOT})")
    L.sezkp_version.restype = C.c_char_p
    L.sezkp_buf_free.argtypes = [C.POINTER(Buf)]
    E = [C.c_char_p, C.c_size_t]
    L.sezkp_stark_v1_prove.argtypes = [C.POINTER(BlockView), C.c_char_p, C.c_uint32, C.POINTER(Buf), C.POINTER(Buf)] + E
    L.sezkp_stark_v1_prove_artifact_cbor.argtypes = [C.POINTER(BlockView), C.c_char_p, C.c_uint32, C.POINTER(Buf)] + E
    L.sezkp_stark_v1_verify.argtypes = [C.c_char_p, C.c_size_t, C.POINTER(BlockView), C.c_char_p] + E
    L.sezkp_ctx_create.restype = C.c_void_p
    L.sezkp_ctx_create.argtypes = [C.c_int32] + E
    L.sezkp_ctx_destroy.argtypes = [C.c_void_p]
    L.sezkp_ctx_upload.argtypes = [C.c_void_p, C.POINTER(BlockView)] + E
    L.sezkp_ctx_prove.argtypes = [C.c_void_p, C.c_char_p, C.c_uint32, C.POINTER(Buf)] + E
    L.sezkp_ctx_prove_borrow.argtypes = [C.c_void_p, C.c_char_p, C.c_uint32, C.POINTER(C.POINTER(C.c_uint8)),
                                         C.POINTER(C.c_size_t)] + E
    L.sezkp_ctx_stage_times.argtypes = [C.c_void_p, C.POINTER(C.c_double), C.c_int32]
    L.sezkp_ctx_stream.restype = C.c_void_p
    L.sezkp_ctx_comm_stats.argtypes = [C.c_void_p, C.POINTER(CommStat), C.c_int32]
    L.sezkp_ctx_stream.argtypes = [C.c_void_p]
    L.sezkp_ctx_dict_plans.argtypes = [C.c_void_p, C.POINTER(DictPlanInfo), C.c_int32]
    L.sezkp_ctx_dict_cache_stats.argtypes = [C.c_void_p, C.POINTER(C.c_uint32), C.POINTER(C.c_uint32),
                                             C.POINTER(C.c_uint64)]
    L.sezkp_gl_ntt.argtypes = [C.c_void_p, C.c_void_p, C.c_uint32, C.c_int32, C.c_void_p]
    L.sezkp_gl_coset_lde_deep.argtypes = [C.c_void_p, C.c_uint32, C.c_uint32, C.c_uint64, C.c_uint64, C.c_void_p,
                                          C.c_void_p, C.c_void_p]
    L.sezkp_fri_fold.argtypes = [C.c_void_p, C.c_uint64, C.c_uint64, C.c_void_p, C.c_void_p]
    L.sezkp_blake3_leaves_u64.argtypes = [C.c_void_p, C.c_uint64, C.c_void_p, C.c_void_p]
    L.sezkp_blake3_leaves_labeled.argtypes = [C.c_void_p, C.c_uint64, C.c_char_p, C.c_uint32, C.c_void_p, C.c_void_p]
    L.sezkp_merkle_node_count.restype = C.c_uint64
    L.sezkp_merkle_node_count.argtypes = [C.c_uint64]
    L.sezkp_merkle_build.argtypes = [C.c_void_p, C.c_uint64, C.c_void_p, C.c_void_p]
    L.sezkp_merkle_paths.argtypes = [C.c_void_p, C.c_uint64, C.c_void_p, C.c_uint32, C.c_void_p, C.c_void_p]
    L.sezkp_fri_fold_commit.argtypes = [C.c_void_p, C.c_uint64, C.c_uint64, C.c_void_p, C.c_char_p, C.c_void_p]
    L.sezkp_merkle_root_u64.argtypes = [C.c_void_p, C.c_uint64, C.c_char_p, C.c_void_p]
    L.sezkp_manifest_root.argtypes = [C.POINTER(BlockView), C.c_char_p]
    L.sezkp_manifest_frontier_root.argtypes = [C.POINTER(BlockView), C.c_char_p]
    L.sezkp_blocks_decode_cbor.argtypes = [C.c_char_p, C.c_size_t, C.POINTER(C.c_void_p)] + E
    L.sezkp_blocks_decode_jsonl.argtypes = [C.c_char_p, C.c_size_t, C.POINTER(C.c_void_p)] + E
    L.sezkp_blocks_encode_jsonl.argtypes = [C.POINTER(BlockView), C.POINTER(Buf)]
    L.sezkp_manifest_decode.argtypes = [C.c_char_p, C.c_size_t, C.c_int32, C.c_char_p, C.POINTER(C.c_uint32)] + E
    L.sezkp_blocks_view.restype = C.POINTER(BlockView)
    L.sezkp_blocks_view.argtypes = [C.c_void_p]
    L.sezkp_blocks_free.argtypes = [C.c_void_p]
    L.sezkp_blake3.argtypes = [C.c_char_p, C.c_size_t, C.c_char_p, C.c_size_t]
    L.sezkp_comm_unique_id.argtypes = [C.c_char_p] + E
    L.sezkp_ctx_create_sharded.restype = C.c_void_p
    L.sezkp_ctx_create_sharded.argtypes = [C.c_int32, C.c_int32, C.c_int32, C.c_char_p] + E
    L.sezkp_ctx_create_sharded_host.restype = C.c_void_p
    L.sezkp_ctx_create_sharded_host.argtypes = [C.c_int32, C.c_int32, C.c_int32, C.POINTER(HostComm)] + E
    L.sezkp_blocks_encode_cbor.argtypes = [C.POINTER(BlockView), C.POINTER(Buf)]
    L.sezkp_simulate_trace.argtypes = [C.c_uint64, C.c_uint32, C.c_uint64] + [C.c_void_p] * 4
    L.sezkp_simulate_blocks.argtypes = [C.c_uint64, C.c_uint32, C.c_uint32, C.c_uint64, C.POINTER(C.c_void_p)] + E
    L.sezkp_ctx_prove_async.argtypes = [C.c_void_p, C.c_char_p, C.c_uint32] + E
    L.sezkp_ctx_wait.argtypes = [C.c_void_p, C.POINTER(C.POINTER(C.c_uint8)), C.POINTER(C.c_size_t)] + E
    L.sezkp_ctx_stage.argtypes = [C.c_void_p, C.POINTER(BlockView)] + E
    L.sezkp_host_register.argtypes = [C.c_void_p, C.c_size_t]
    L.sezkp_host_unregister.argtypes = [C.c_void_p]
    L.sezkp_ctx_dist_ntt.argtypes = [C.c_void_p, C.c_void_p, C.c_void_p, C.c_uint32, C.c_int32] + E
    L.sezkp_fs_xof.argtypes = [C.c_char_p, C.c_size_t, C.POINTER(C.c_uint32), C.c_char_p, C.POINTER(C.c_uint32),
                               C.POINTER(C.c_uint32), C.c_uint32, C.c_char_p, C.c_void_p]
    L.sezkp_ctx_upload_rows.argtypes = [C.c_void_p, C.POINTER(BlockView), C.c_uint64, C.c_uint64] + E
    L.sezkp_shard_rows.argtypes = [C.c_void_p, C.c_uint32, C.c_int32, C.c_int32, C.POINTER(C.c_uint64),
                                   C.POINTER(C.c_uint64)]
    L.sezkp_blocks_decode_jsonl_meta.argtypes = [C.c_void_p, C.c_size_t, C.c_uint64, C.c_uint64,
                                                 C.POINTER(C.c_void_p)] + E
    L.sezkp_blocks_decode_jsonl_lines.argtypes = [C.c_void_p, C.c_size_t, C.c_uint64, C.c_uint64, C.c_int32,
                                                  C.POINTER(C.c_void_p)] + E
    L.sezkp_blocks_line_offsets.argtypes = [C.c_void_p, C.POINTER(C.POINTER(C.c_uint64)), C.POINTER(C.c_size_t)]
    L.sezkp_manifest_leaf_hashes.argtypes = [C.POINTER(BlockView), C.c_void_p]
    L.sezkp_merkle_root_of_leaves.argtypes = [C.c_char_p, C.c_size_t, C.c_int32, C.c_char_p]
    L.sezkp_ctx_create_sharded_solo.restype = C.c_void_p
    L.sezkp_ctx_create_sharded_solo.argtypes = [C.c_int32, C.c_int32, C.c_int32] + E
    L.sezkp_ctx_air_audit.argtypes = [C.c_void_p, C.POINTER(AirAuditC), C.c_void_p, C.c_void_p] + E
    L.sezkp_stark_v1_air_audit.argtypes = [C.POINTER(BlockView), C.POINTER(AirAuditC), C.POINTER(Buf),
                                           C.POINTER(Buf)] + E
    L.sezkp_ctx_verify_batch.argtypes = [C.c_void_p, C.POINTER(ProofRef), C.c_uint32, C.POINTER(VerifyResultC)] + E
    L.sezkp_stark_v1_verify_batch.argtypes = [C.POINTER(ProofRef), C.c_uint32, C.POINTER(VerifyResultC)] + E
    L.sezkp_ctx_verify_times.argtypes = [C.c_void_p, C.POINTER(C.c_double), C.c_int32]
    return L


lib = _load()


def take_buf(b: Buf) -> bytes:
    out = C.string_at(b.data, b.len) if b.len else b""
    lib.sezkp_buf_free(C.byref(b))
    return out


def check(rc: int, err) -> None:
    if rc != SEZKP_OK:
        raise SezkpError(rc, err.value.decode(errors="replace"))
```

### streaming-zero-knowledge-proofs_amd/sezkp_amd/backend.py

```python
from __future__ import annotations

import ctypes as C
import json
import struct
from dataclasses import dataclass, field

from ._lib import (AIR_FAMILIES, SEZKP_FLAG_STREAMING, VERIFY_TIMES, AirAuditC, Buf, ProofRef, SezkpError,
                   VerifyResultC, check, lib, take_buf)
from .blocks import BlockSoA

STAGES = ["expand", "col_commit", "col_outer", "compose", "intt", "lde_ntt", "deep", "layer0_tree",
          "layer0_upper", "fri_fold_trees", "col_openings", "fri_paths", "total",
          "host_wall", "host_sync_wait", "host_final_wait", "host_serialize",
          "k_forest16"]


@dataclass
class ProofArtifact:
    backend: str
    manifest_root: bytes
    proof_bytes: bytes
    meta: dict = field(default_factory=dict)

    def to_cbor(self) -> bytes:
# ... 208 lines not shown
        proof = take_buf(pb)
        return ProofArtifact("stark", bytes(manifest_root), proof, _meta(proof, self.tau, streaming))

    def air_audit(self, bitmaps: bool = False) -> AirAudit:
        a = AirAuditC()
        nbytes = (self.n_rows + 7) // 8
        vb = C.create_string_buffer(nbytes) if bitmaps else None
        rb = C.create_string_buffer(nbytes) if bitmaps else None
        err = C.create_string_buffer(1024)
        check(lib.sezkp_ctx_air_audit(self._h, C.byref(a), vb, rb, err, 1024), err)
        return AirAudit._from_c(a, vb.raw if bitmaps else None, rb.raw if bitmaps else None)

    def verify_batch(self, proofs, manifest_roots=None, taus=None) -> list:
        return _verify_batch(lambda *a: lib.sezkp_ctx_verify_batch(self._h, *a), proofs, manifest_roots, taus)

    def verify(self, artifact: ProofArtifact, blocks: BlockSoA, manifest_root: bytes) -> None:
        if artifact.backend != "stark":
            raise SezkpError(-5, "backend kind mismatch: expected STARK")
        if bytes(artifact.manifest_root) != bytes(manifest_root):
            raise SezkpError(-5, "manifest root mismatch")
        blocks.check_shape()
        if blocks.n_blocks and blocks.tau == 0:
            return StarkV1.verify(artifact, blocks, manifest_root)
        r = self.verify_batch([artifact.proof_bytes], [bytes(manifest_root)], [blocks.tau if blocks.n_blocks else 0])[0]
        if not r.ok:
            raise SezkpError(r.code, r.message)

    def verify_times(self) -> dict:
        buf = (C.c_double * len(VERIFY_TIMES))()
        n = lib.sezkp_ctx_verify_times(self._h, buf, len(VERIFY_TIMES))
        return {VERIFY_TIMES[i]: buf[i] for i in range(n)}

    def prove_view(self, manifest_root: bytes) -> memoryview:
        ptr = C.POINTER(C.c_uint8)()
        n = C.c_size_t()
        err = C.create_string_buffer(1024)
        check(lib.sezkp_ctx_prove_borrow(self._h, bytes(manifest_root), 0, C.byref(ptr), C.byref(n), err, 1024), err)
        return memoryview((C.c_uint8 * n.value).from_address(C.addressof(ptr.contents))).cast("B").toreadonly()

    def prove_async(self, manifest_root: bytes) -> None:
        err = C.create_string_buffer(1024)
        check(lib.sezkp_ctx_prove_async(self._h, bytes(manifest_root), 0, err, 1024), err)

    def wait_view(self) -> memoryview:
        ptr = C.POINTER(C.c_uint8)()
        n = C.c_size_t()
        err = C.create_string_buffer(1024)
        check(lib.sezkp_ctx_wait(self._h, C.byref(ptr), C.byref(n), err, 1024), err)
        return memoryview((C.c_uint8 * n.value).from_address(C.addressof(ptr.contents))).cast("B").toreadonly()

    def stage_times_ms(self) -> dict:
        buf = (C.c_double * 32)()
        n = lib.sezkp_ctx_stage_times(self._h, buf, 32)
        return {STAGES[i]: buf[i] for i in range(min(n, len(STAGES)))}

    def comm_stats(self) -> list:
        from ._lib import CommStat
        buf = (CommStat * 64)()
        n = lib.sezkp_ctx_comm_stats(self._h, buf, 64)
        out = []
        for i in range(n):
            b, ms = int(buf[i].bytes), float(buf[i].ms)
            out.append({"name": buf[i].name.decode(), "bytes": b, "ms": ms,
                        "GBs": (b / ms / 1e6) if ms > 0 else None})
        return out

    def dict_plans(self) -> list:
        from ._lib import DictPlanInfo
        cap = 1 + 4 * self.tau
        buf = (DictPlanInfo * cap)()
        n = lib.sezkp_ctx_dict_plans(self._h, buf, cap)
        if n < 0:
            why = {-1: "a proof is in flight on this context (or the context is closed)",
                   -2: "copying the plans from the device failed"}.get(n, "unexpected return code")
            raise SezkpError(n, f"dict_plans: {why}")
        return [{f: int(getattr(buf[i], f)) for f, _ in DictPlanInfo._fields_} for i in range(n)]

    def dict_cache_stats(self) -> dict:
        rebuilt, reused, entries = C.c_uint32(0), C.c_uint32(0), C.c_uint64(0)
        rc = lib.sezkp_ctx_dict_cache_stats(self._h, C.byref(rebuilt), C.byref(reused), C.byref(entries))
        if rc < 0:
            raise SezkpError(rc, "dict_cache_stats: a proof is in flight on this context (or the context is closed)")
        return {"cols_rebuilt": rebuilt.value, "cols_reused": reused.value, "entries_rebuilt": entries.value}

    def dist_ntt(self, local, scratch=None, inverse: bool = False, sync: bool = True):
        import torch
        if local.dtype not in (torch.int64, torch.uint64) or not local.is_cuda or not local.is_contiguous():
            raise SezkpError(-1, "local must be a contiguous 64-bit device tensor")
        m = local.numel()
        if m & (m - 1):
            raise SezkpError(-1, "local length must be a power of two")
        if scratch is None:
            scratch = torch.empty_like(local)
        log_n = (m * self.world).bit_length() - 1
        if sync:
            torch.cuda.current_stream(local.device).synchronize()
        err = C.create_string_buffer(1024)
        check(lib.sezkp_ctx_dist_ntt(self._h, local.data_ptr(), scratch.data_ptr(), log_n, -1 if inverse else 1,
                                     err, 1024), err)
        if sync:
            torch.cuda.ExternalStream(self.stream, device=local.device).synchronize()
        return local

    @property
    def stream(self) -> int:
        return lib.sezkp_ctx_stream(self._h) or 0

    def close(self):
        if self._h:
            lib.sezkp_ctx_destroy(self._h)
            self._h = None

    def __del__(self):
        try:
            self.close()
        except Exception:
            pass


class ShardedProverContext(ProverContext):

    def __init__(self, rank: int, world: int, device: int = 0, comm: str = "rccl", group=None):
        import torch.distributed as dist
        err = C.create_string_buffer(1024)
        self.tau = 0
        self.n_rows = 0
        self.rank, self.world = rank, world
        self._hc = None
        if comm == "rccl":
            uid = C.create_string_buffer(128)
            if rank == 0:
                check(lib.sezkp_comm_unique_id(uid, err, 1024), err)
            obj = [bytes(uid.raw)]
            if world > 1:
                dist.broadcast_object_list(obj, src=0, group=group)
            self._h = lib.sezkp_ctx_create_sharded(device, rank, world, obj[0], err, 1024)
        elif comm == "solo":
            self._h = lib.sezkp_ctx_create_sharded_solo(device, rank, world, err, 1024)
        elif comm == "host":
            from .dist import HostCollectives
            self._coll = HostCollectives(group)
            self._hc = self._coll.c_struct()
            self._h = lib.sezkp_ctx_create_sharded_host(device, rank, world, C.byref(self._hc), err, 1024)
        else:
            raise ValueError(f"unknown comm {comm!r}")
        if not self._h:
            raise SezkpError(-2, err.value.decode())
```

Before: 9.960 billion field-elements/s.

## Precompute per-pass NTT twiddle tables and build per-block leaf tables by value

Each wide NTT pass now reads its twiddle factors from a cached, precomputed device table keyed by pass shape, rather than recomputing them with two table lookups and a field multiply plus incremental products. Separately, per-block column leaf tables (winlen/offin/offout) are built over the distinct value range when that range is smaller than the block count, so fewer leaf hashes are computed, and lookups map block values to units. The twiddle tables add global-memory reads per butterfly, and the first call per shape does a synchronous allocate-and-fill. The by-value path adds a min/max reduction in every table block, a bounds check with an error flag, and new stats plumbing.

```diff
diff --git a/include/sezkp_stark.h b/include/sezkp_stark.h
--- a/include/sezkp_stark.h
+++ b/include/sezkp_stark.h
@@ -92,6 +92,9 @@
 int32_t sezkp_ctx_dict_cache_stats(const sezkp_ctx* ctx, uint32_t* cols_rebuilt, uint32_t* cols_reused,
                                    uint64_t* entries_rebuilt);
 
+int32_t sezkp_ctx_pw_table_stats(const sezkp_ctx* ctx, uint32_t* cols_by_value, uint32_t* cols_by_block,
+                                 uint64_t* units_built);
+
 #define SEZKP_AIR_FAMILIES 5
 typedef struct sezkp_air_family {
   uint64_t cells, rows, first_row;
diff --git a/streaming-zero-knowledge-proofs_amd/csrc/dev_common.h b/streaming-zero-knowledge-proofs_amd/csrc/dev_common.h
--- a/streaming-zero-knowledge-proofs_amd/csrc/dev_common.h
+++ b/streaming-zero-knowledge-proofs_amd/csrc/dev_common.h
@@ -63,6 +63,9 @@
 __device__ __forceinline__ uint64_t gl_sqr(uint64_t a) { return gl_mul(a, a); }
 __device__ __forceinline__ uint64_t gl_from_i64(int64_t x) {
   return x >= 0 ? (uint64_t)x : GL_P - (uint64_t)(-x);
+}
+__device__ __forceinline__ int64_t gl_to_i64(uint64_t x) {
+  return x > GL_P / 2 ? -(int64_t)(GL_P - x) : (int64_t)x;
 }
 __device__ __forceinline__ uint64_t gl_pow2k(uint64_t x, int k) {
   for (int i = 0; i < k; i++) x = gl_sqr(x);
diff --git a/streaming-zero-knowledge-proofs_amd/csrc/ntt.hip b/streaming-zero-knowledge-proofs_amd/csrc/ntt.hip
--- a/streaming-zero-knowledge-proofs_amd/csrc/ntt.hip
+++ b/streaming-zero-knowledge-proofs_amd/csrc/ntt.hip
@@ -1,6 +1,9 @@
 #include <stdlib.h>
 
 #include <algorithm>
+#include <map>
+#include <mutex>
+#include <tuple>
 
 #include "dev_common.h"
 #include "gl_pow2.h"
@@ -21,6 +24,10 @@
 }
 __device__ __forceinline__ uint64_t pow3(const NttTables& T, uint64_t e) {
   return gl_mul(T.p3_hi[e >> T.S], T.p3_lo[e & ((1ULL << T.S) - 1)]);
+}
+__device__ __forceinline__ uint64_t tw_hi(const NttTables& T, uint64_t i, bool inverse) {
+  const uint64_t mask = (1ULL << (T.K - T.S)) - 1;
+  return T.hi[(inverse ? 0 - i : i) & mask];
 }
 
 __device__ __forceinline__ uint64_t src_slot(const NttPassArgs& P, uint64_t k, uint32_t e) {
@@ -320,7 +327,8 @@
   __shared__ uint64_t W[R];
   const int tid = threadIdx.x;
   const NttTables& T = P.tw;
-  for (int x = tid; x < R; x += NTT_THREADS) W[x] = tw_pow(T, (uint64_t)x << (T.K - m), INV);
+  for (int x = tid; x < R; x += NTT_THREADS)
+    W[x] = P.tw_tab ? tw_hi(T, (uint64_t)x << (T.K - T.S - m), INV) : tw_pow(T, (uint64_t)x << (T.K - m), INV);
   Tile G;
   G.sL = P.sL;
   G.m = m;
@@ -334,6 +342,7 @@
     G.low0 = (G.tile % tiles_per_blk) * NTT_CMAX;
   }
   const int tw_shift = T.K - m - G.sL;
+  const bool pass_tab = !NARROW && P.tw_pass != nullptr;
   const int c = tid & (NTT_CMAX - 1), g = tid / NTT_CMAX;
   const bool staged_load = NARROW && !P.dp_rlo && !P.src;
   if constexpr (NARROW && DIF && !X16) {
@@ -382,7 +391,15 @@
 #pragma unroll
           for (int r = 0; r < F1; r++) x[r] = gl_mul(x[r], P.out_scale);
         }
-        if (low != 0) {
+        if (low != 0 && pass_tab) {
+          const int j1 = rev<M2>(u);
+#pragma unroll
+          for (int q = 0; q < F1; q++) {
+            uint64_t f = P.tw_pass[((uint64_t)(j1 + F2 * q) << G.sL) + low];
+            if (scale) f = gl_mul(f, P.out_scale);
+            x[rev<M1>(q)] = gl_mul(x[rev<M1>(q)], f);
+          }
+        } else if (low != 0) {
           const int j1 = rev<M2>(u);
           uint64_t t = tw_pow(T, (low * (uint64_t)j1) << tw_shift, INV);
           if (scale) t = gl_mul(t, P.out_scale);
@@ -472,7 +489,12 @@
       fft_dif_regs<M1, INV>(y);
       uint64_t low;
       (void)tile_pos(G, q * F1, c, low);
-      if (low != 0) {
+      if (low != 0 && pass_tab) {
+        const int klo = rev<M2>(q);
+#pragma unroll
+        for (int kh = 0; kh < F1; kh++)
+          y[rev<M1>(kh)] = gl_mul(y[rev<M1>(kh)], P.tw_pass[((uint64_t)(klo + F2 * kh) << G.sL) + low]);
+      } else if (low != 0) {
         uint64_t t = tw_pow(T, (low * (uint64_t)rev<M2>(q)) << tw_shift, INV);
         const uint64_t s1 = tw_pow(T, (low * (uint64_t)F2) << tw_shift, INV);
 #pragma unroll
@@ -723,17 +745,56 @@
   return false;
 }
 
+static int ntt_tw_table_on() {
+  const char* e = getenv("SEZKP_NTT_TW_TABLE");
+  return !(e && e[0] == '0' && !e[1]);
+}
+
+__global__ void __launch_bounds__(NTT_THREADS) k_pass_twiddles(NttTables T, uint64_t* __restrict__ tab, int sL, int m,
+                                                               int inverse) {
+  const uint64_t i = (uint64_t)blockIdx.x * NTT_THREADS + threadIdx.x;
+  if (i >> (sL + m)) return;
+  const uint64_t low = i & ((1ULL << sL) - 1), j = i >> sL;
+  tab[i] = tw_hi(T, (low * j) << (T.K - T.S - m - sL), inverse != 0);
+}
+static const uint64_t* pass_twiddles(hipStream_t st, const NttTables& T, int sL, int m, bool inverse) {
+  static std::mutex mu;
+  static std::map<std::tuple<int, const uint64_t*, int, int, int, int, bool>, uint64_t*> tabs;
+  if (sL < 4 || m + sL > T.K - T.S) return nullptr;
+  int dev = 0;
+  if (hipGetDevice(&dev) != hipSuccess) return nullptr;
+  std::lock_guard<std::mutex> lk(mu);
+  const auto key = std::make_tuple(dev, T.hi, T.K, T.S, sL, m, inverse);
+  auto it = tabs.find(key);
+  if (it != tabs.end()) return it->second;
+  uint64_t* d = nullptr;
+  const uint64_t cnt = 1ULL << (sL + m);
+  if (hipMalloc((void**)&d, cnt * 8) != hipSuccess) return nullptr;
+  hipLaunchKernelGGL(k_pass_twiddles, dim3((unsigned)((cnt + NTT_THREADS - 1) / NTT_THREADS)), dim3(NTT_THREADS), 0, st,
+                     T, d, sL, m, inverse ? 1 : 0);
+  if (hipPeekAtLastError() != hipSuccess || hipStreamSynchronize(st) != hipSuccess) {
+    (void)hipFree(d);
+    return nullptr;
+  }
+  tabs.emplace(key, d);
+  return d;
+}
+
 template <bool DIF, bool INV>
-static bool launch_ntt4(hipStream_t st, const NttPassArgs& P, unsigned tiles) {
-  if (P.logC != 4) return false;
+static bool launch_ntt4(hipStream_t st, const NttPassArgs& P0, unsigned tiles) {
+  if (P0.logC != 4) return false;
+  NttPassArgs P = P0;
+  P.tw_tab = ntt_tw_table_on();
   const int skip = P.src ? P.skip : 0;
   if (DIF && skip) return false;
 #define SEZKP_NTT4(M1, M2, SK)                                                                                \
   do {                                                                                                         \
     if (P.sL == 0)                                                                                           \
       hipLaunchKernelGGL((k_ntt4<DIF, INV, M1, M2, SK, false, true>), dim3(tiles), dim3(NTT_THREADS), 0, st, P); \
-    else                                                                                                       \
+    else {              \
+      P.tw_pass = P.tw_tab ? pass_twiddles(st, P.tw, P.sL, P.m, INV) : nullptr;                               \
       hipLaunchKernelGGL((k_ntt4<DIF, INV, M1, M2, SK>), dim3(tiles), dim3(NTT_THREADS), 0, st, P);           \
+    }                                                                                                          \
   } while (0)
   if (P.m > NTT_MMAX) {
     if (P.sL != 0 || skip || (P.src && !P.dp_rlo)) return false;
@@ -1181,6 +1242,8 @@
     if (deep && fused && i == np - 1 && i > 0 && !inverse &&
         logC == 4 && P.sL >= 4 && (P.m == 8 || P.m == 7)) {
       P.deep_z = deep->z; P.deep_logN = deep->logN; P.deep_logP = deep->logP; P.deep_g = deep->g;
+      P.tw_tab = ntt_tw_table_on();
+      P.tw_pass = P.tw_tab ? pass_twiddles(st, T, P.sL, P.m, false) : nullptr;
       if (P.m == 8)
         hipLaunchKernelGGL((k_ntt4<false, false, 4, 4, 0, true>), dim3((unsigned)tiles), dim3(NTT_THREADS), 0, st, P);
       else
diff --git a/streaming-zero-knowledge-proofs_amd/csrc/prover.cpp b/streaming-zero-knowledge-proofs_amd/csrc/prover.cpp
--- a/streaming-zero-knowledge-proofs_amd/csrc/prover.cpp
+++ b/streaming-zero-knowledge-proofs_amd/csrc/prover.cpp
@@ -177,6 +177,10 @@
   bool dict_dirty = false;
   uint32_t dstat_rebuilt = 0, dstat_reused = 0;
   uint64_t dstat_entries = 0;
+  std::vector<uint32_t> pw_blk_cols;
+  uint32_t* d_pwstat = nullptr;
+  uint32_t pwstat_by_value = 0;
+  uint64_t pwstat_units = 0;
   void free_dict_cache() {
     if (d_dtabs) (void)hipFree(d_dtabs);
     if (d_dkeys) (void)hipFree(d_dkeys);
@@ -613,10 +617,17 @@
   tab_units = cp.tab_units;
   d_tmpl = dalloc<ColTemplate>(ncols);
   up(d_tmpl, tm.data(), tm.size());
-  d_colroots = dalloc<uint32_t>((size_t)ncols * 8 + 16 + 2 * dcols.size());
+  T.pw_lo = dalloc<int64_t>(2 * (size_t)ncols + 2);
+  pw_blk_cols.clear();
+  for (int c = 0; c < ncols; c++)
+    if (tm[c].kind >= 7) pw_blk_cols.push_back((uint32_t)c);
+  d_colroots = dalloc<uint32_t>((size_t)ncols * 8 + 16 + 2 * dcols.size() + ncols);
   d_err = d_colroots + (size_t)ncols * 8;
   d_dstatus = d_err + 16;
+  d_pwstat = d_dstatus + 2 * dcols.size();
+  T.pw_stat = d_pwstat;
   HIP_OR_THROW(hipMemset(d_err, 0, 64));
+  HIP_OR_THROW(hipMemset(d_pwstat, 0, (size_t)ncols * 4));
   d_tabs = dalloc<uint32_t>(cp.tab_nodes * 8 + 8);
   n_tab_cols = (int)cp.tab_cols.size();
   d_tab_cols = dalloc<uint32_t>(cp.tab_cols.size() + 1);
@@ -750,7 +761,7 @@
   PL.base = dalloc<uint32_t>(PL.total / 4 + 2);
   h_proof = halloc<uint8_t>(hdr_bytes + PL.total);
   memcpy(h_proof, pp.header.data(), hdr_bytes);
-  h_small = halloc<uint32_t>((size_t)(ncols + k + 4) * 8 + 2 * (size_t)n_dict);
+  h_small = halloc<uint32_t>((size_t)(ncols + k + 4) * 8 + 2 * (size_t)n_dict + (size_t)ncols);
   d_chal = dalloc<DevChal>(1);
   h_chal = halloc<DevChal>(1);
   d_dict_of = dalloc<uint32_t>((size_t)ncols);
@@ -1248,8 +1259,8 @@
     dict_seq++;
   }
   const DictCache dcache{d_dkeys, d_dreuse, d_dlvl_seq, d_dstatus, dict_epoch, dict_seq};
-  uint32_t st_rebuilt = 0;
-  uint64_t st_entries = 0;
+  uint32_t st_rebuilt = 0, st_pw_by_value = 0;
+  uint64_t st_entries = 0, st_pw_units = 0;
   const int nguard = sharded ? comm->world : 1;
   auto check_guards = [&](const uint32_t* g_h, int ng) {
     for (int r = 0; r < ng; r++) {
@@ -1312,9 +1323,7 @@
     TreeDev outer0{d_outer, d_colroots, logChunks, 0};
     ok(launch_tree_upper(st, &outer0, ncols, outer_stride, 8, 0), "col_outer");
     rec(3);
-    HIP_OR_THROW(hipMemcpyAsync(h_small, d_colroots,
-                                n_dict ? (size_t)ncols * 32 + 4 * (16 + 2 * (size_t)n_dict)
-                                       : (size_t)ncols * 32 + 4 * (gofs + nguard),
+    HIP_OR_THROW(hipMemcpyAsync(h_small, d_colroots, (size_t)ncols * 32 + 4 * (16 + 2 * (size_t)n_dict + (size_t)ncols),
                                 hipMemcpyDeviceToHost, st));
   };
   auto host_1 = [&]() {
@@ -1323,6 +1332,11 @@
     for (int c = 0; c < n_dict; c++) {
       st_rebuilt += h_small[8 * ncols + 16 + 2 * c];
       st_entries += h_small[8 * ncols + 16 + 2 * c + 1];
+    }
+    for (uint32_t c : pw_blk_cols) {
+      const uint32_t units = h_small[8 * ncols + 16 + 2 * n_dict + c];
+      st_pw_by_value += units != 0;
+      st_pw_units += units;
     }
     std::vector<uint8_t> colroots((const uint8_t*)colroots_h, (const uint8_t*)colroots_h + (size_t)ncols * 32);
     for (int c = 0; c < ncols; c++) memcpy(h_proof + root_pos[c], colroots.data() + 32 * c, 32);
@@ -1716,6 +1730,8 @@
   dstat_rebuilt = st_rebuilt;
   dstat_reused = (uint32_t)n_dict - st_rebuilt;
   dstat_entries = st_entries;
+  pwstat_by_value = st_pw_by_value;
+  pwstat_units = st_pw_units;
   return out;
 }
 
@@ -2045,6 +2061,17 @@
   *cols_rebuilt = have ? ctx->dstat_rebuilt : 0;
   *cols_reused = have ? ctx->dstat_reused : 0;
   *entries_rebuilt = have ? ctx->dstat_entries : 0;
+  return SEZKP_OK;
+}
+int32_t sezkp_ctx_pw_table_stats(const sezkp_ctx* cctx, uint32_t* cols_by_value, uint32_t* cols_by_block,
+                                 uint64_t* units_built) {
+  sezkp_ctx* ctx = const_cast<sezkp_ctx*>(cctx);
+  if (!ctx || !cols_by_value || !cols_by_block || !units_built) return SEZKP_E_INVALID;
+  if (ctx->busy()) return SEZKP_E_INVALID;
+  const bool have = ctx->loaded && ctx->have_plans;
+  *cols_by_value = have ? ctx->pwstat_by_value : 0;
+  *cols_by_block = have ? (uint32_t)ctx->pw_blk_cols.size() - ctx->pwstat_by_value : 0;
+  *units_built = have ? ctx->pwstat_units : 0;
   return SEZKP_OK;
 }
 int32_t sezkp_ctx_comm_stats(const sezkp_ctx* ctx, sezkp_comm_stat* out, int32_t max) {
diff --git a/streaming-zero-knowledge-proofs_amd/csrc/sezkp_internal.h b/streaming-zero-knowledge-proofs_amd/csrc/sezkp_internal.h
--- a/streaming-zero-knowledge-proofs_amd/csrc/sezkp_internal.h
+++ b/streaming-zero-knowledge-proofs_amd/csrc/sezkp_internal.h
@@ -40,6 +40,8 @@
   int nat_out, nat_logN;
   uint64_t out_scale;
   int nat_tr;
+  int tw_tab;
+  const uint64_t* tw_pass;
 };
 struct DeepFuse {
   uint64_t z;
@@ -89,7 +91,10 @@
   uint8_t* row_flags;
   int32_t* head;
   int64_t* head_rng;
-};
+  int64_t* pw_lo;
+  uint32_t* pw_stat;
+};
+constexpr int64_t PW_BY_BLOCK = INT64_MIN;
 
 struct ComposeTerms {
   uint64_t* hr;
diff --git a/streaming-zero-knowledge-proofs_amd/csrc/trace.hip b/streaming-zero-knowledge-proofs_amd/csrc/trace.hip
--- a/streaming-zero-knowledge-proofs_amd/csrc/trace.hip
+++ b/streaming-zero-knowledge-proofs_amd/csrc/trace.hip
@@ -290,10 +290,21 @@
   b3_parent(p0, p1, h);
 }
 
+__device__ __forceinline__ const uint64_t* pw_block_values(const TraceDev& T, const ColTemplate& ct) {
+  const uint64_t* tab = ct.kind == 7 ? T.blk_winlen : (ct.kind == 8 ? T.blk_offin : T.blk_offout);
+  return tab + (uint64_t)ct.tape * T.nblk;
+}
+__device__ __forceinline__ uint32_t pw_unit(const uint64_t* __restrict__ bv, int64_t lo, uint32_t k) {
+  if (lo == PW_BY_BLOCK) return k;
+  const uint64_t u = (uint64_t)gl_to_i64(bv[k]) - (uint64_t)lo;
+  return u > 0xffffffffull ? 0xffffffffu : (uint32_t)u;
+}
 __global__ void __launch_bounds__(TR_THREADS) k_col_tables(TraceDev T, const ColTemplate* __restrict__ tmpl,
                                                            const uint32_t* __restrict__ cols, uint32_t* __restrict__ tabs,
-                                                           uint32_t blk_lo, uint32_t blk_cnt) {
-  const ColTemplate ct = tmpl[cols[blockIdx.y]];
+                                                           uint32_t blk_lo, uint32_t blk_cnt, int by_value_ok) {
+  __shared__ int64_t s_rng[2][TR_THREADS / 64];
+  const uint32_t col = cols[blockIdx.y];
+  const ColTemplate ct = tmpl[col];
   uint64_t i = (uint64_t)blockIdx.x * TR_THREADS + threadIdx.x;
   uint32_t h[8];
   if (kind_has_leaf_table(ct.kind)) {
@@ -303,14 +314,50 @@
     node_store(tabs + 8 * (ct.tab + i), h);
     return;
   }
-  const bool flags = ct.kind == 1 || ct.kind == 2;
-  if (flags ? i >= 2 : i >= blk_cnt) return;
-  if (!flags) i += blk_lo;
   uint64_t v;
-  if (ct.kind == 1 || ct.kind == 2) v = i;
-  else {
-    const uint64_t* tab = ct.kind == 7 ? T.blk_winlen : (ct.kind == 8 ? T.blk_offin : T.blk_offout);
-    v = tab[(uint64_t)ct.tape * T.nblk + i];
+  if (ct.kind == 1 || ct.kind == 2) {
+    if (i >= 2) return;
+    v = i;
+  } else {
+    if (blockIdx.x && (uint64_t)blockIdx.x * TR_THREADS >= blk_cnt) return;
+    const uint64_t* bv = pw_block_values(T, ct) + blk_lo;
+    int64_t mn = INT64_MAX, mx = INT64_MIN;
+    for (uint32_t j = threadIdx.x; j < blk_cnt; j += TR_THREADS) {
+      const int64_t s = gl_to_i64(bv[j]);
+      mn = s < mn ? s : mn;
+      mx = s > mx ? s : mx;
+    }
+#pragma unroll
+    for (int o = 32; o >= 1; o >>= 1) {
+      const int64_t a = __shfl_xor(mn, o, 64), b = __shfl_xor(mx, o, 64);
+      mn = a < mn ? a : mn;
+      mx = b > mx ? b : mx;
+    }
+    if ((threadIdx.x & 63) == 0) {
+      s_rng[0][threadIdx.x >> 6] = mn;
+      s_rng[1][threadIdx.x >> 6] = mx;
+    }
+    __syncthreads();
+#pragma unroll
+    for (int w = 0; w < TR_THREADS / 64; w++) {
+      mn = s_rng[0][w] < mn ? s_rng[0][w] : mn;
+      mx = s_rng[1][w] > mx ? s_rng[1][w] : mx;
+    }
+    const uint64_t span = (uint64_t)mx - (uint64_t)mn;
+    const bool by_value = by_value_ok && blk_cnt && span < blk_cnt;
+    if (i == 0) {
+      T.pw_lo[2 * col] = by_value ? mn : PW_BY_BLOCK;
+      T.pw_lo[2 * col + 1] = by_value ? (int64_t)span : (int64_t)T.nblk - 1;
+      T.pw_stat[col] = by_value ? (uint32_t)span + 1 : 0;
+    }
+    if (by_value) {
+      if (i > span) return;
+      v = gl_from_i64(mn + (int64_t)i);
+    } else {
+      if (i >= blk_cnt) return;
+      v = bv[i];
+      i += blk_lo;
+    }
   }
   leaf_labeled_rt(ct, v, h);
   uint32_t* o = tabs + 8 * (ct.tab + i * U_LEVELS);
@@ -433,6 +480,10 @@
   const uint64_t ch = chunks[item % nchunks];
   const uint32_t kind = tmpl[c].kind;
   const uint32_t* U = tabs + 8 * tmpl[c].tab;
+  const bool per_blk = kind >= 7;
+  const uint64_t* bv = per_blk ? pw_block_values(T, tmpl[c]) : nullptr;
+  const int64_t vlo = per_blk ? T.pw_lo[2 * c] : PW_BY_BLOCK;
+  const uint32_t ulast = per_blk ? (uint32_t)T.pw_lo[2 * c + 1] : T.nblk - 1;
   const uint64_t n = T.n;
   const uint64_t cl = n < 1024 ? n : 1024;
   const uint64_t c0 = ch << COL_CHUNK_LOG2, c1 = c0 + cl;
@@ -448,7 +499,8 @@
     if (be <= row) { k++; continue; }
     const uint64_t pe = be < c1 ? be : c1;
     uint64_t cut = pe;
-    uint32_t u = k;
+    uint32_t u = per_blk ? pw_unit(bv, vlo, k) : k;
+    if (u > ulast) { atomicOr(err, 4u); return; }
     if (kind == 1) { u = row == bs ? 1u : 0u; cut = row == bs ? row + 1 : pe; }
     else if (kind == 2) { u = row + 1 == be ? 1u : 0u; cut = (row + 1 < be && pe == be) ? be - 1 : pe; }
     while (row < cut) {
@@ -1037,9 +1089,12 @@
   }
 }
 
-__device__ __forceinline__ bool pw_range_hash(const TraceDev& T, uint32_t kind, const uint32_t* __restrict__ U,
-                                              uint64_t r0, int lw, uint32_t (*stk)[8][64], int slot,
-                                              uint32_t (&out)[8]) {
+__device__ __forceinline__ bool pw_range_hash(const TraceDev& T, const ColTemplate& ct, int64_t vlo, uint32_t ulast,
+                                              const uint32_t* __restrict__ U, uint64_t r0, int lw,
+                                              uint32_t (*stk)[8][64], int slot, uint32_t (&out)[8]) {
+  const uint32_t kind = ct.kind;
+  const bool per_blk = kind >= 7;
+  const uint64_t* bv = per_blk ? pw_block_values(T, ct) : nullptr;
   const uint64_t c1 = r0 + (1ULL << lw);
   uint64_t lvpack = 0;
   int sp = 0;
@@ -1051,7 +1106,8 @@
     if (be <= row) { k++; continue; }
     const uint64_t pe = be < c1 ? be : c1;
     uint64_t cut = pe;
-    uint32_t u = k;
+    uint32_t u = per_blk ? pw_unit(bv, vlo, k) : k;
+    if (u > ulast) return false;
     if (kind == 1) { u = row == bs ? 1u : 0u; cut = row == bs ? row + 1 : pe; }
     else if (kind == 2) { u = row + 1 == be ? 1u : 0u; cut = (row + 1 < be && pe == be) ? be - 1 : pe; }
     while (row < cut) {
@@ -1168,7 +1224,8 @@
     if (tid < logcl) {
       uint32_t h[8];
       const uint64_t rs = start + (((in >> tid) ^ 1) << tid);
-      if (pw_range_hash(T, ct.kind, tabs + 8 * (uint64_t)ct.tab, rs, tid,
+      if (pw_range_hash(T, ct, ct.kind >= 7 ? T.pw_lo[2 * c] : PW_BY_BLOCK,
+                        ct.kind >= 7 ? (uint32_t)T.pw_lo[2 * c + 1] : T.nblk - 1, tabs + 8 * (uint64_t)ct.tab, rs, tid,
                         reinterpret_cast<uint32_t(*)[8][64]>(&lds[0][0]), tid, h)) {
 #pragma unroll
         for (int w = 0; w < 8; w++) o[18 + 8 * tid + w] = h[w];
@@ -1621,8 +1678,10 @@
   if (n_tab_cols == 0) return hipSuccess;
   if ((uint64_t)blk_lo + blk_cnt > T.nblk) return hipErrorInvalidValue;
   const unsigned gx = (unsigned)((max_units + TR_THREADS - 1) / TR_THREADS);
+  const char* bv = getenv("SEZKP_PW_BY_VALUE");
+  const int by_value_ok = !(bv && bv[0] == '0' && !bv[1]);
   hipLaunchKernelGGL(k_col_tables, dim3(gx, n_tab_cols), dim3(TR_THREADS), 0, st, T, d_tmpl, d_tab_cols, tabs, blk_lo,
-                     blk_cnt);
+                     blk_cnt, by_value_ok);
   return hipGetLastError();
 }
 static hipError_t dict_shape_ok(const TraceDev& T, uint64_t row0, uint64_t nrows) {
diff --git a/streaming-zero-knowledge-proofs_amd/sezkp_amd/_lib.py b/streaming-zero-knowledge-proofs_amd/sezkp_amd/_lib.py
--- a/streaming-zero-knowledge-proofs_amd/sezkp_amd/_lib.py
+++ b/streaming-zero-knowledge-proofs_amd/sezkp_amd/_lib.py
@@ -30,7 +30,7 @@
     "sezkp_fs_xof", "sezkp_ctx_upload_rows", "sezkp_shard_rows", "sezkp_blocks_decode_jsonl_meta",
     "sezkp_blocks_line_offsets", "sezkp_manifest_leaf_hashes", "sezkp_merkle_root_of_leaves",
     "sezkp_ctx_create_sharded_solo", "sezkp_blocks_decode_jsonl_lines", "sezkp_ctx_dict_plans",
-    "sezkp_ctx_air_audit", "sezkp_stark_v1_air_audit", "sezkp_ctx_dict_cache_stats",
+    "sezkp_ctx_air_audit", "sezkp_stark_v1_air_audit", "sezkp_ctx_dict_cache_stats", "sezkp_ctx_pw_table_stats",
     "sezkp_ctx_verify_batch", "sezkp_stark_v1_verify_batch", "sezkp_ctx_verify_times",
 ]
 
@@ -140,6 +140,8 @@
     L.sezkp_ctx_dict_plans.argtypes = [C.c_void_p, C.POINTER(DictPlanInfo), C.c_int32]
     L.sezkp_ctx_dict_cache_stats.argtypes = [C.c_void_p, C.POINTER(C.c_uint32), C.POINTER(C.c_uint32),
                                              C.POINTER(C.c_uint64)]
+    L.sezkp_ctx_pw_table_stats.argtypes = [C.c_void_p, C.POINTER(C.c_uint32), C.POINTER(C.c_uint32),
+                                           C.POINTER(C.c_uint64)]
     L.sezkp_gl_ntt.argtypes = [C.c_void_p, C.c_void_p, C.c_uint32, C.c_int32, C.c_void_p]
     L.sezkp_gl_coset_lde_deep.argtypes = [C.c_void_p, C.c_uint32, C.c_uint32, C.c_uint64, C.c_uint64, C.c_void_p,
                                           C.c_void_p, C.c_void_p]
diff --git a/streaming-zero-knowledge-proofs_amd/sezkp_amd/backend.py b/streaming-zero-knowledge-proofs_amd/sezkp_amd/backend.py
--- a/streaming-zero-knowledge-proofs_amd/sezkp_amd/backend.py
+++ b/streaming-zero-knowledge-proofs_amd/sezkp_amd/backend.py
@@ -314,6 +314,13 @@
         if rc < 0:
             raise SezkpError(rc, "dict_cache_stats: a proof is in flight on this context (or the context is closed)")
         return {"cols_rebuilt": rebuilt.value, "cols_reused": reused.value, "entries_rebuilt": entries.value}
+
+    def pw_table_stats(self) -> dict:
+        by_value, by_block, units = C.c_uint32(0), C.c_uint32(0), C.c_uint64(0)
+        rc = lib.sezkp_ctx_pw_table_stats(self._h, C.byref(by_value), C.byref(by_block), C.byref(units))
+        if rc < 0:
+            raise SezkpError(rc, "pw_table_stats: a proof is in flight on this context (or the context is closed)")
+        return {"cols_by_value": by_value.value, "cols_by_block": by_block.value, "units_built": units.value}
 
     def dist_ntt(self, local, scratch=None, inverse: bool = False, sync: bool = True):
         import torch
```

Measured after the change: 10.09 billion field-elements/s (median of 6 runs). 1.01x the previous value.
